# XiYe20/NPVP

Measured on AMD Instinct MI355X. Metric: predictor train frames/sec, higher is better.
Workload: dtype f32 (two-term fp16 split of amax-scaled operands, 3 MFMAs per product, fp32 accumulate: fp32-grade; small GEMMs: three-term bf16 split)

## Files before the change

### include/npvp_hip.h

```cpp
#ifndef NPVP_HIP_H
#define NPVP_HIP_H
#include <stddef.h>
#ifdef __cplusplus
extern "C" {
#endif

typedef struct ihipStream_t* npvp_stream_t;

int npvp_version(void);
const char* npvp_last_error(void);
long long npvp_launch_count(void);
void* npvp_stream_create_low_priority(int* least, int* greatest);
int npvp_stream_destroy(void* stream);
void* npvp_event_create(void);
int npvp_event_record(void* event, void* stream);
float npvp_event_elapsed_ms(void* event0, void* event1);
int npvp_event_destroy(void* event);

long long npvp_graph_node_counts(void* graph, long long* counts, long long* memset_bytes, int max_memsets);

long long npvp_gemm_workspace_bytes(int M, int N, int K);
int npvp_gemm_kernel_id(int a_kc, int b_kc, int M, int N, int K, int precision, int has_planes);
int npvp_gemm_route(int a_kc, int b_kc, int M, int N, int K, int precision, int has_planes, int plain_epilogue, int* out4);
int npvp_gemm_f32(int a_kc, int b_kc, int M, int N, int K, const float* A, long long lda, const float* B, long long ldb,
                  float* C, long long ldc, const float* bias, int act, const float* aux_in, float* aux_out,
                  const float* residual, long long ldr, float drop_p, int drop_mode, int drop_g1, int drop_g2,
                  const unsigned long long* seed, unsigned int salt, float alpha, int precision, float* colsum_a,
                  const void* b_pre, int accumulate, float* rowstats, const float* a_amax, const float* b_amax,
                  float* c_amax, unsigned int* range_flag, float adrop_p, int adrop_g1, int adrop_g2, unsigned int adrop_salt,
                  void* workspace, long long ws_bytes, npvp_stream_t stream);
int npvp_gemm_f32_skip(int a_kc, int b_kc, int M, int N, int K, const float* A, long long lda, const float* B, long long ldb,
                       float* C, long long ldc, const float* bias, int act, const float* aux_in, float* aux_out,
                       const float* residual, long long ldr, float drop_p, int drop_mode, int drop_g1, int drop_g2,
                       const unsigned long long* seed, unsigned int salt, float alpha, int precision, float* colsum_a,
                       const void* b_pre, int accumulate, float* rowstats, const float* a_amax, const float* b_amax,
                       float* c_amax, unsigned int* range_flag, float adrop_p, int adrop_g1, int adrop_g2, unsigned int adrop_salt,
                       float skip_p, int skip_g1, int skip_g2, unsigned int skip_salt, void* workspace, long long ws_bytes,
                       npvp_stream_t stream);
int npvp_frame_stats_finalize(const float* part, int parts_per_frame, float values_per_part, float* mean, float* rstd,
                              int frames, float eps, npvp_stream_t stream);
int npvp_split_weight(const float* w, long long ld, int N, int K, void* F, void* D, npvp_stream_t stream);
int npvp_split_weights_batched(const void* desc, int count, npvp_stream_t stream);
int npvp_amax(const float* x, long long rows, long long cols, long long ld, float* slot, npvp_stream_t stream);

typedef struct npvp_reduce_job {
  const float* ws; float* out; long long ldc; int M, N, splits, accum; float alpha; int blocks; const float* cs_part; float* cs_out;
} npvp_reduce_job_t;
int npvp_wgrad_f16_chainable(int M, int N, int K);
long long npvp_wgrad_f16_chain_workspace_bytes(int M, int N, int K);
int npvp_wgrad_f16_chained(int M, int N, int K, const float* dy, long long lda, const float* x, long long ldb, float* dw,
                           long long ldc, float* db, int accumulate, const float* a_amax, const float* b_amax,
                           unsigned int* range_flag, float adrop_p, int adrop_g1, int adrop_g2, unsigned int adrop_salt,
                           const unsigned long long* seed, const void* prev_job, void* my_job, void* workspace,
                           long long ws_bytes, npvp_stream_t stream);
int npvp_wgrad_f16_chained_skip(int M, int N, int K, const float* dy, long long lda, const float* x, long long ldb, float* dw,
                                long long ldc, float* db, int accumulate, const float* a_amax, const float* b_amax,
                                unsigned int* range_flag, float adrop_p, int adrop_g1, int adrop_g2, unsigned int adrop_salt,
                                float skip_p, int skip_g1, int skip_g2, unsigned int skip_salt,
                                const unsigned long long* seed, const void* prev_job, void* my_job, void* workspace,
                                long long ws_bytes, npvp_stream_t stream);
int npvp_splitk_reduce_job(const void* job, npvp_stream_t stream);
int npvp_splitk_reduce_multi(const void* jobs, int n, npvp_stream_t stream);
int npvp_linear_bwd_f16_takes(int R, int N, int K);
int npvp_linear_bwd_f16(int R, int N, int K, const float* dy, long long ldy, const float* dy_amax, const void* w_planes_d,
                        const float* w_amax, float* dx, long long ldx, int act, const float* aux_in, const float* residual,
                        long long ldr, float drop_p, int drop_mode, int drop_g1, int drop_g2, unsigned int drop_salt, float* dx_amax,
                        const float* x, long long ldxx, const float* x_amax, float* dw, long long ldw, float* db,
                        unsigned int* range_flag, float adrop_p, int adrop_g1, int adrop_g2, unsigned int adrop_salt,
                        const unsigned long long* seed, const void* prev_job, void* my_job, void* workspace, long long ws_bytes,
                        npvp_stream_t stream);
int npvp_linear_bwd_f16_skip(int R, int N, int K, const float* dy, long long ldy, const float* dy_amax, const void* w_planes_d,
                             const float* w_amax, float* dx, long long ldx, int act, const float* aux_in, const float* residual,
                             long long ldr, float drop_p, int drop_mode, int drop_g1, int drop_g2, unsigned int drop_salt,
                             float* dx_amax, const float* x, long long ldxx, const float* x_amax, float* dw, long long ldw, float* db,
                             unsigned int* range_flag, float adrop_p, int adrop_g1, int adrop_g2, unsigned int adrop_salt,
                             float skip_p, int skip_g1, int skip_g2, unsigned int skip_salt, const unsigned long long* seed,
                             const void* prev_job, void* my_job, void* workspace, long long ws_bytes, npvp_stream_t stream);
int npvp_split_weight_f16(const float* w, long long ld, int N, int K, void* F, void* D, float* amax_slot, npvp_stream_t stream);
int npvp_split_weights_f16(const void* desc, int count, void* amax_table, long long amax_bytes, npvp_stream_t stream);

int npvp_layernorm_fwd(const float* x, const float* w, const float* b, float* y, float* mean, float* rstd, long long rows,
                       int C, float eps, int relu, float* y_amax, npvp_stream_t stream);
long long npvp_layernorm_bwd_workspace_bytes(long long rows, int C);
int npvp_layernorm_bwd(const float* dy, const float* x, const float* w, const float* b, const float* mean,
                       const float* rstd, float* dx, float* dw, float* db, long long rows, int C, int relu,
                       const float* dres ,
                       int accumulate , float* dx_amax,
                       void* workspace, long long ws_bytes, npvp_stream_t stream);
int npvp_layernorm_bwd_reduce(const void* workspace, float* dw, float* db, long long rows, int C, int accumulate,
                              npvp_stream_t stream);

int npvp_layernorm_bwd_reduce_job(const void* workspace, float* dw, float* db, long long rows, int C, int accumulate, void* job);
int npvp_frameln_act_bwd_reduce_job(const void* workspace, float* dw, float* db, int frames, int per_frame, int accumulate, void* job);
int npvp_mlpdw_mid_bwd_reduce_job(const void* workspace, float* gw, float* gb, int frames, int Ch, void* job);
int npvp_sum_rows_multi(const void* jobs, int n, npvp_stream_t stream);

int npvp_layernorm_nchw_fwd(const float* x, const float* w, const float* b, float* out_nchw, float* mean, float* rstd, int frames,
                            int P, int C, float eps, int relu, npvp_stream_t stream);

int npvp_frame_stats(const float* x, const float* add, float* mean, float* rstd, int frames, int T, int per_frame,
                     float eps, npvp_stream_t stream);
int npvp_posfuse_fwd(const float* x, const float* add, const float* beta, const float* gamma, float* y, float* mean,
                     float* rstd, int N, int T, int per_frame, float eps, float* y_amax, npvp_stream_t stream);
int npvp_ln_posfuse_fwd(const float* x, const float* lw, const float* lb, float ln_eps, float* y1, float* ln_mean, float* ln_rstd,
                        const float* add, const float* beta, const float* gamma, float* fused, float* pf_mean, float* pf_rstd,
                        int N, int T, int P, int C, float pf_eps, float* y1_amax, float* fused_amax, npvp_stream_t stream);
int npvp_posfuse_bwd_fused(int N, int T, int per_frame);
int npvp_posfuse_bwd(const float* dy, const float* x, const float* add, const float* gamma, const float* mean,
                     const float* rstd, float* du, float* dyxh, float* dbeta, float* dgamma, int N, int T, int per_frame,
                     int accumulate, void* workspace, long long ws_bytes , npvp_stream_t stream);

int npvp_posfuse_instance_fwd(const float* x, const float* add, const float* beta, const float* gamma, float* y, float* mean,
                              float* rstd, int N, int T, int P, int C, float eps, float* y_amax, npvp_stream_t stream);
int npvp_posfuse_instance_bwd(const float* dy, const float* x, const float* add, const float* gamma, const float* mean,
                              const float* rstd, float* du, float* dyxh, int N, int T, int P, int C, npvp_stream_t stream);

int npvp_frameln_act_fwd(const float* h, const float* mean, const float* rstd, const float* w, const float* b,
                         const float* res, float* out, int frames, int per_frame, float drop_p, unsigned int salt,
                         float dp_p, unsigned int dp_salt, int frames_per_sample, const unsigned long long* seed,
                         float* out_amax, npvp_stream_t stream);
long long npvp_frameln_act_bwd_workspace_bytes(int frames, int per_frame);
int npvp_frameln_act_bwd(const float* dout, const float* h, const float* mean, const float* rstd, const float* w,
                         const float* b, float* dh, float* dw, float* db, int frames, int per_frame, float drop_p,
                         unsigned int salt, float dp_p, unsigned int dp_salt, int frames_per_sample,
                         const unsigned long long* seed, int accumulate ,
                         float* dh_amax, void* workspace, long long ws_bytes, npvp_stream_t stream);
int npvp_frameln_act_bwd_reduce(const void* workspace, float* dw, float* db, int frames, int per_frame, int accumulate,
                                npvp_stream_t stream);
int npvp_dwconv3x3(const float* a, const float* wt, const float* bias, float* out, int frames, int H, int W, int Ch,
                   int flip, npvp_stream_t stream);
int npvp_dwconv3x3_stats(const float* a, const float* wt, const float* bias, float* out, float* mean, float* rstd, int frames,
                         int H, int W, int Ch, float eps, void* workspace, long long ws_bytes, npvp_stream_t stream);
int npvp_mlpdw_mid_fwd(const float* h1, const float* mean1, const float* rstd1, const float* w1n, const float* b1n,
                       const float* wt, const float* bias, float* h2, float* mean2, float* rstd2, int frames, int H, int W,
                       int Ch, float eps, void* workspace, long long ws_bytes, npvp_stream_t stream);
int npvp_mlpdw_mid_fwd_parts(const float* h1, const float* part1, int J1, float nb1, float* mean1, float* rstd1, const float* w1n,
                             const float* b1n, const float* wt, const float* bias, float* h2, float* part2, int frames, int H,
                             int W, int Ch, float eps, npvp_stream_t stream);
int npvp_frameln_act_fwd_parts(const float* h, const float* part, int J, float nb, float eps, float* mean, float* rstd,
                               const float* w, const float* b, const float* res, float* out, int frames, int per_frame,
                               float drop_p, unsigned int salt, float dp_p, unsigned int dp_salt, int frames_per_sample,
                               const unsigned long long* seed, float* out_amax, npvp_stream_t stream);
long long npvp_mlpdw_mid_bwd_workspace_bytes(int frames, int Ch);
int npvp_mlpdw_mid_bwd(const float* dh2, const float* h1, const float* mean1, const float* rstd1, const float* w1n,
                       const float* b1n, const float* wt, float* da1, float* dwt_db, float* psum, int frames, int H, int W,
                       int Ch, int accumulate, void* workspace, long long ws_bytes, npvp_stream_t stream);
int npvp_mlpdw_mid_bwd_reduce(const void* workspace, float* dwt_db, int frames, int Ch, int accumulate, npvp_stream_t stream);
int npvp_mlpdw_mid_bwd_reduce_into(const void* workspace, float* gw, float* gb, int frames, int Ch, npvp_stream_t stream);
int npvp_mlpdw_mid_bwd_n2(const float* da2, const float* h2, const float* mean2, const float* rstd2, const float* w2n,
                          const float* b2n, const float* psum2, int nparts2, float drop_p, unsigned int salt,
                          const unsigned long long* seed, const float* h1, const float* mean1, const float* rstd1,
                          const float* w1n, const float* b1n, const float* wt, float* da1, float* dwt_db, float* psum, int frames,
                          int H, int W, int Ch, int accumulate, void* workspace, long long ws_bytes, npvp_stream_t stream);
int npvp_frameln_act_bwd_pgrad(const float* dout, const float* h, const float* mean, const float* rstd, const float* w,
                               const float* b, float* psum, float* dw, float* db, int frames, int per_frame, float drop_p,
                               unsigned int salt, float dp_p, unsigned int dp_salt, int frames_per_sample,
                               const unsigned long long* seed, int accumulate, void* workspace, long long ws_bytes,
                               npvp_stream_t stream);
int npvp_frameln_act_bwd_apply(const float* dout, const float* h, const float* mean, const float* rstd, const float* w,
                               const float* b, const float* psum, int nparts, float* dh, float* dw, float* db, int frames,
                               int per_frame, int accumulate, float* dh_amax, void* workspace, long long ws_bytes,
                               npvp_stream_t stream);
int npvp_mlpdw_mid_fwd_parts_skip(const float* h1, const float* part1, int J1, float nb1, float* mean1, float* rstd1,
                                  const float* w1n, const float* b1n, const float* wt, const float* bias, float* h2, float* part2,
                                  int frames, int H, int W, int Ch, float eps, float skip_p, unsigned int skip_salt, int skip_fps,
                                  const unsigned long long* seed, npvp_stream_t stream);
int npvp_frameln_act_fwd_parts_skip(const float* h, const float* part, int J, float nb, float eps, float* mean, float* rstd,
                                    const float* w, const float* b, const float* res, float* out, int frames, int per_frame,
                                    float drop_p, unsigned int salt, float dp_p, unsigned int dp_salt, int frames_per_sample,
                                    const unsigned long long* seed, float* out_amax, float skip_p, unsigned int skip_salt,
                                    int skip_fps, npvp_stream_t stream);
int npvp_frameln_act_bwd_apply_skip(const float* dout, const float* h, const float* mean, const float* rstd, const float* w,
                                    const float* b, const float* psum, int nparts, float* dh, float* dw, float* db, int frames,
                                    int per_frame, int accumulate, float* dh_amax, void* workspace, long long ws_bytes,
                                    float skip_p, unsigned int skip_salt, int skip_fps, const unsigned long long* seed,
                                    npvp_stream_t stream);

int npvp_im2col3x3(const float* in, float* out, int frames, int H, int W, int C, int col2im, npvp_stream_t stream);
long long npvp_dwconv3x3_wgrad_workspace_bytes(int frames, int Ch);
int npvp_dwconv3x3_wgrad(const float* a, const float* dout, float* dwt_db, int frames, int H, int W, int Ch,
                         void* workspace, long long ws_bytes, npvp_stream_t stream);

int npvp_attn_fwd(const float* q, long long ld_q, const float* k, long long ld_k, const float* v, long long ld_v, float* o,
                  long long ld_o, int mode, int dim0, int P, int W, int ws, int Tq, int Tk, int heads, int head_dim,
                  int mask_mode, float drop_p, const unsigned long long* seed, unsigned int salt, float* o_amax,
                  npvp_stream_t stream);
int npvp_attn_bwd(const float* q, long long ld_q, const float* k, long long ld_k, const float* v, long long ld_v,
                  const float* go, long long ld_o, float* dq, long long ld_dq, float* dk, long long ld_dk, float* dv,
                  long long ld_dv, int mode, int dim0, int P, int W, int ws, int Tq, int Tk, int heads, int head_dim,
                  int mask_mode, float drop_p, const unsigned long long* seed, unsigned int salt, float* dq_amax,
                  float* dk_amax , float* dv_amax,
                  npvp_stream_t stream);
int npvp_attn_long_fwd(const float* q, long long ld_q, const float* k, long long ld_k, const float* v, long long ld_v, float* o,
                       long long ld_o, int mode, int dim0, int P, int W, int ws, int Tq, int Tk, int heads, int head_dim,
                       int mask_mode, float drop_p, const unsigned long long* seed, unsigned int salt, float* o_amax,
                       npvp_stream_t stream);
long long npvp_attn_long_bwd_workspace_bytes(int mode, int dim0, int P, int W, int ws, int Tq, int Tk, int heads);
int npvp_attn_long_bwd(const float* q, long long ld_q, const float* k, long long ld_k, const float* v, long long ld_v,
                       const float* go, long long ld_o, float* dq, long long ld_dq, float* dk, long long ld_dk, float* dv,
                       long long ld_dv, int mode, int dim0, int P, int W, int ws, int Tq, int Tk, int heads, int head_dim,
                       int mask_mode, float drop_p, const unsigned long long* seed, unsigned int salt, float* dq_amax,
                       float* dk_amax , float* dv_amax, void* workspace, long long ws_bytes,
                       npvp_stream_t stream);

int npvp_reparam_samples(const float* mu, const float* logvar, float* z, float* eps_out, long long numel, int S,
                         long long sample_base, const unsigned long long* seed, unsigned int salt, npvp_stream_t stream);
int npvp_attn_samples_fwd(const float* q, long long ld_q, const float* k, long long ld_k, const float* v, long long ld_v, float* o,
                          long long ld_o, int S, int N, int P, int Tq, int Tk, int heads, int head_dim, int sample_chunk,
                          float* o_amax, npvp_stream_t stream);

int npvp_drop_apply(const float* x, float* out, long long rows, int ncols, float p, int mode, int g1, int g2,
                    const unsigned long long* seed, unsigned int salt, float* out_amax, npvp_stream_t stream);
int npvp_transpose(const float* in, float* out, int batch, int R, int C, npvp_stream_t stream);
int npvp_dwtb_accumulate(const float* dwtb, float* gw, float* gb, int C, npvp_stream_t stream);
int npvp_dwtb_build(const float* w, const float* b, float* wtb, int C, npvp_stream_t stream);
int npvp_reduce_mid(const float* in, float* out, int A, int B, long long Cc, float scale, int accumulate, npvp_stream_t stream);
int npvp_broadcast_mid(const float* in, float* out, int A, int B, long long Cc, float scale, npvp_stream_t stream);
int npvp_grid_center_pad(const float* src, long long ld_src, float* dst, long long ld_dst, int F, int H, int W, int Hp, int Wp, int top,
                         int left, int C, long long rows_out, float* dst_amax, npvp_stream_t stream);
int npvp_grid_center_cut(const float* src, long long ld_src, const float* addend, long long ld_add, float* dst, long long ld_dst, int F,
                         int H, int W, int Hp, int Wp, int top, int left, int C, float* dst_amax, npvp_stream_t stream);
int npvp_evt_token_join(const float* x, long long ld_x, const float* token, long long ld_token, long long token_clip_stride, float* y,
                        long long ld_y, int N, int T, int P, int C, float* y_amax, npvp_stream_t stream);
int npvp_evt_token_split(const float* y, long long ld_y, float* x, long long ld_x, float* last, long long ld_last, int N, int T, int P,
                         int C, float* x_amax, float* last_amax, npvp_stream_t stream);

long long npvp_colsum_workspace_bytes(long long rows, int N);
int npvp_colsum(const float* x, long long rows, int N, long long ld, float* out, int accumulate ,
                void* workspace, long long ws_bytes, npvp_stream_t stream);

int npvp_l1_mean(const float* a, const float* b, long long n, float lam, float* out, void* workspace, long long ws_bytes,
                 npvp_stream_t stream);
int npvp_l1_mean_bwd(const float* a, const float* b, long long n, const float* gout, float lam, float* da, npvp_stream_t stream);
int npvp_sum_all(const float* x, long long n, float* out, void* workspace, long long ws_bytes, npvp_stream_t stream);

int npvp_grad_norm_clip(const float* g, long long n, float max_norm, float* out2, void* workspace, long long ws_bytes,
                        npvp_stream_t stream);
int npvp_adamw_step(float* p, float* g, float* m, float* v, long long n, const float* hyper, float beta1, float beta2,
                    float eps, float weight_decay, const float* clip, long long clip_begin, long long clip_end,
                    int write_back_grad, npvp_stream_t stream);

long long npvp_sqdiff_workspace_bytes(int N, long long per_image);
int npvp_sqdiff_per_image(const float* x, const float* y, int N, long long per_image, float data_range, float scale, float* out,
                          void* workspace, long long ws_bytes, npvp_stream_t stream);
long long npvp_ssim_workspace_bytes(int N, int C, int H, int W);
int npvp_ssim_per_image(const float* img1, const float* img2, int N, int C, int H, int W, const float* taps ,
                        int window_size, float* out, void* workspace, long long ws_bytes, npvp_stream_t stream);

int npvp_u8hwc_to_f32chw(const void* src_u8, float* dst, long long frames, int H, int W, int C, const float* mean,
                         const float* std, npvp_stream_t stream);

int npvp_bias_act(const float* x, const float* bias, const float* residual, float* out, long long outer, long long inner, int C,
                  int layout, int act, npvp_stream_t stream);
int npvp_act_bwd(const float* g, const float* y, float* dx, long long n, int act, npvp_stream_t stream);

int npvp_bn_workspace_bytes(int C);
int npvp_bn_stats(const float* x, long long outer, long long inner, int C, int layout, double* sums, void* workspace, long long ws_bytes,
                  npvp_stream_t stream);
int npvp_bn_act_apply(const float* x, const float* w, const float* b, const float* residual, const double* sums, long long count,
                      float eps, float momentum, float* running_mean, float* running_var, long long outer, long long inner, int C,
                      int layout, int act, float* y, float* mean, float* rstd, npvp_stream_t stream);
int npvp_bn_act_bwd(const float* g, const float* x, const float* mean, const float* rstd, const float* w, const float* b, long long outer,
                    long long inner, int C, int layout, int act, int train, float* dx, float* dw, float* db, void* workspace,
                    long long ws_bytes, npvp_stream_t stream);
int npvp_bn_act_apply_sync(const float* x, const float* w, const float* b, const float* residual, const double* stat, float eps,
                           float momentum, float* running_mean, float* running_var, long long outer, long long inner, int C, int layout,
                           int act, float* y, float* mean, float* rstd, npvp_stream_t stream);
int npvp_bn_bwd_sums(const float* g, const float* x, const float* mean, const float* rstd, const float* w, const float* b, long long outer,
                     long long inner, int C, int layout, int act, double* sums, float* dw, float* db, void* workspace, long long ws_bytes,
                     npvp_stream_t stream);
int npvp_bn_act_bwd_apply(const float* g, const float* x, const float* mean, const float* rstd, const float* w, const float* b,
                          const double* sums, const double* count, long long outer, long long inner, int C, int layout, int act, float* dx,
                          npvp_stream_t stream);
int npvp_reflect_pad(const float* x, float* y, int planes, int H, int W, int C, int P, int layout, int backward, npvp_stream_t stream);
int npvp_nonlocal_attn_fwd(const float* q, long long ldq, const float* k, long long ldk, const float* v, long long ldv, float* o,
                           long long ldo, float* lse, int F, int H, int W, int A, int V, npvp_stream_t stream);
int npvp_nonlocal_attn_bwd(const float* q, long long ldq, const float* k, long long ldk, const float* v, long long ldv, const float* go,
                           long long ldgo, const float* lse, float* D, float* dq, long long lddq,
                           float* dk, long long lddk, float* dv, long long lddv, int F, int H, int W, int A, int V, npvp_stream_t stream);
int npvp_nonlocal_attn_grid_fwd(const float* q, long long ldq, const float* k, long long ldk, const float* v, long long ldv, float* o,
                                long long ldo, float* lse, int F, int H, int W, int A, int V, npvp_stream_t stream);
int npvp_nonlocal_attn_grid_bwd(const float* q, long long ldq, const float* k, long long ldk, const float* v, long long ldv,
                                const float* go, long long ldgo, const float* lse, float* D, float* dq, long long lddq,
                                float* dk, long long lddk, float* dv, long long lddv, int F, int H, int W, int A, int V,
                                npvp_stream_t stream);
int npvp_temporal_attn_fwd(const float* q, long long ldq, const float* k, long long ldk, const float* v, long long ldv, float* o,
                           long long ldo, float* lse, int N, int T, int HW, int A, int V, npvp_stream_t stream);
int npvp_temporal_attn_bwd(const float* q, long long ldq, const float* k, long long ldk, const float* v, long long ldv, const float* go,
                           long long ldgo, const float* lse, float* dq, long long lddq, float* dk, long long lddk, float* dv,
                           long long lddv, int N, int T, int HW, int A, int V, npvp_stream_t stream);
int npvp_temporal_attn_long_fwd(const float* q, long long ldq, const float* k, long long ldk, const float* v, long long ldv, float* o,
                                long long ldo, float* lse, int N, int T, int HW, int A, int V, npvp_stream_t stream);
int npvp_temporal_attn_long_bwd(const float* q, long long ldq, const float* k, long long ldk, const float* v, long long ldv,
                                const float* go, long long ldgo, const float* lse, float* D, float* dq, long long lddq, float* dk,
                                long long lddk, float* dv, long long lddv, int N, int T, int HW, int A, int V, npvp_stream_t stream);

int npvp_dp_unique_id(void* id_out_128_bytes);
int npvp_dp_init(int rank, int world, const void* unique_id_128_bytes);
int npvp_dp_world(void);
int npvp_dp_rank(void);
int npvp_dp_allreduce_async(float* bucket, size_t n, npvp_stream_t side);
int npvp_dp_wait(npvp_stream_t compute);
int npvp_dp_finalize(void);

#ifdef __cplusplus
}
#endif
#endif
```

### npvp_amd/csrc/common.h

```cpp
#pragma once
#include <hip/hip_runtime.h>
#include <stdint.h>
#include "npvp_hip.h"

#define NPVP_OK 0
#define NPVP_ERR_ARG (-1)
#define NPVP_ERR_LAUNCH (-2)
#define NPVP_ERR_WORKSPACE (-3)

void npvp_set_error(const char* msg);

namespace npvp { extern long long g_launches; }
#define NPVP_LAUNCH(...)                                                    \
  do {                                                                      \
    __atomic_fetch_add(&npvp::g_launches, 1ll, __ATOMIC_RELAXED);           \
    hipLaunchKernelGGL(__VA_ARGS__);                                        \
  } while (0)

#define NPVP_CHECK_ARG(cond, msg)                    \
  do {                                               \
    if (!(cond)) {                                   \
      npvp_set_error(msg);                           \
      return NPVP_ERR_ARG;                           \
    }                                                \
  } while (0)

#define NPVP_CHECK_LAUNCH()                          \
  do {                                               \
    hipError_t e__ = hipGetLastError();              \
    if (e__ != hipSuccess) {                         \
      npvp_set_error(hipGetErrorString(e__));        \
      return NPVP_ERR_LAUNCH;                        \
    }                                                \
  } while (0)

namespace npvp {

constexpr int WAVE = 64;

__device__ __forceinline__ float wave_sum(float v) {
#pragma unroll
  for (int o = 32; o > 0; o >>= 1) v += __shfl_xor(v, o, 64);
  return v;
}
__device__ __forceinline__ float wave_max(float v) {
#pragma unroll
  for (int o = 32; o > 0; o >>= 1) v = fmaxf(v, __shfl_xor(v, o, 64));
  return v;
}

constexpr int AMAX_WORDS = 32, AMAX_STRIDE = 16;
__device__ __forceinline__ float amax_slot_read(const float* slot) {
  const float v = wave_max(slot[(threadIdx.x & (AMAX_WORDS - 1)) * AMAX_STRIDE]);
  return __builtin_bit_cast(float, __builtin_amdgcn_readfirstlane(__builtin_bit_cast(int, v)));
}
__device__ __forceinline__ unsigned int amax_peek(const float* slot, unsigned int idx) {
  if (!slot) return 0xffffffffu;
  return __hip_atomic_load(reinterpret_cast<const unsigned int*>(slot) + (idx & (AMAX_WORDS - 1)) * AMAX_STRIDE, __ATOMIC_RELAXED,
                           __HIP_MEMORY_SCOPE_AGENT);
}
__device__ __forceinline__ unsigned int amax_peek_wave(const float* slot) { return amax_peek(slot, blockIdx.x * 4u + (threadIdx.x >> 6)); }
__device__ __forceinline__ unsigned int amax_peek_block(const float* slot) { return amax_peek(slot, blockIdx.x); }
__device__ __forceinline__ void amax_word_raise(float* slot, unsigned int idx, float m, unsigned int peeked) {
  const unsigned int bits = __float_as_uint(m);
  if (bits > peeked) atomicMax(reinterpret_cast<unsigned int*>(slot) + (idx & (AMAX_WORDS - 1)) * AMAX_STRIDE, bits);
}
__device__ __forceinline__ void amax_slot_commit(float* slot, float m, unsigned int peeked) {
  if (!slot) return;
  m = wave_max(m);
  if ((threadIdx.x & 63) == 0) amax_word_raise(slot, blockIdx.x * 4u + (threadIdx.x >> 6), m, peeked);
}
__device__ __forceinline__ void amax_slot_commit_block(float* slot, float m, float* red, unsigned int peeked) {
  if (!slot) return;
  m = wave_max(m);
  if ((threadIdx.x & 63) == 0) red[threadIdx.x >> 6] = m;
  __syncthreads();
  if (threadIdx.x == 0) {
    for (unsigned int i = 1; i < (blockDim.x >> 6); ++i) m = fmaxf(m, red[i]);
    amax_word_raise(slot, blockIdx.x, m, peeked);
  }
}
__host__ __device__ __forceinline__ float amax_scale(float amax) {
  unsigned int u;
  __builtin_memcpy(&u, &amax, 4);
  const unsigned int E = (u >> 23) & 0xffu;
  if (E < 16u || E == 255u) return 1.f;
  u = (268u - E) << 23;
  float s;
  __builtin_memcpy(&s, &u, 4);
  return s;
}

__host__ __device__ __forceinline__ float pow2_recip(float s) {
  unsigned int u;
  __builtin_memcpy(&u, &s, 4);
  u = 0x7f000000u - u;
  float r;
  __builtin_memcpy(&r, &u, 4);
  return r;
}

__device__ __forceinline__ float amax4(float m, const float4& v) {
  return fmaxf(fmaxf(fmaxf(m, fabsf(v.x)), fabsf(v.y)), fmaxf(fabsf(v.z), fabsf(v.w)));
}

__device__ __forceinline__ void fmac_scalar(float& acc, float a, float b) {
#if defined(__HIP_DEVICE_COMPILE__)
  asm volatile("v_fmac_f32 %0, %1, %2" : "+v"(acc) : "v"(a), "v"(b));
#else
  acc = fmaf(a, b, acc);
#endif
}

template <int NW>
__device__ __forceinline__ float block_sum(float v, float* red) {
  v = wave_sum(v);
  const int w = threadIdx.x >> 6;
  __syncthreads();
  if ((threadIdx.x & 63) == 0) red[w] = v;
  __syncthreads();
  float t = 0.f;
#pragma unroll
  for (int i = 0; i < NW; ++i) t += red[i];
  return t;
}

__device__ __forceinline__ void frame_stats_merge(const float* __restrict__ part, long long f, int J, float nb, float eps, float& mu,
                                                  float& rs) {
  float m = 0.f;
  for (int j = 0; j < J; ++j) m += part[(f * J + j) * 2];
  m /= J;
  float m2 = 0.f;
  for (int j = 0; j < J; ++j) { const float d = part[(f * J + j) * 2] - m; m2 += part[(f * J + j) * 2 + 1] + nb * d * d; }
  mu = m;
  rs = rsqrtf(m2 / (nb * J) + eps);
}

__device__ __forceinline__ float gelu_phi(float x, float& E) {
  const float au = fabsf(x) * 0.70710678118654752440f;
  const float t = __builtin_amdgcn_rcpf(fmaf(0.3275911f, au, 1.0f));
  E = __expf(-0.5f * x * x);
  float p = fmaf(1.061405429f, t, -1.453152027f);
  p = fmaf(p, t, 1.421413741f);
  p = fmaf(p, t, -0.284496736f);
  p = fmaf(p, t, 0.254829592f);
  const float hq = 0.5f * p * t * E;
  return x >= 0.f ? 1.0f - hq : hq;
}
__device__ __forceinline__ float gelu_f(float x) {
  float E;
  return x * gelu_phi(x, E);
}
__device__ __forceinline__ float gelu_grad_f(float x) {
  float E;
  const float phi = gelu_phi(x, E);
  return fmaf(x * 0.39894228040143267794f, E, phi);
}

__host__ __device__ __forceinline__ uint32_t mix32(uint32_t h) {
  h ^= h >> 16; h *= 0x85ebca6bu;
  h ^= h >> 13; h *= 0xc2b2ae35u;
  h ^= h >> 16;
  return h;
}
__host__ __device__ __forceinline__ uint32_t rng_u32(uint64_t seed, uint32_t salt, uint64_t idx) {
  const uint32_t k0 = mix32((uint32_t)seed ^ mix32(salt * 0x9e3779b9u + 0x7f4a7c15u));
  const uint32_t k1 = mix32((uint32_t)(seed >> 32) + mix32(salt ^ 0x85ebca6bu));
  const uint32_t h = mix32((uint32_t)idx ^ k0);
  return mix32(h + k1 + (uint32_t)(idx >> 32) * 0x9e3779b9u);
}
__device__ __forceinline__ float drop_scale(uint64_t seed, uint32_t salt, uint64_t idx, uint32_t thresh, float inv_keep) {
  return rng_u32(seed, salt, idx) >= thresh ? inv_keep : 0.f;
}
__host__ __device__ __forceinline__ uint32_t drop_threshold(float p) {
  double t = (double)p * 4294967296.0;
  if (t < 0) t = 0;
  if (t > 4294967295.0) t = 4294967295.0;
  return (uint32_t)t;
}

struct DropSpec {
  unsigned int thresh; float inv_keep; unsigned int salt; int mode; int g1; int g2;
  unsigned int m1, m2; int s1, s2;
};
__host__ __device__ __forceinline__ void div_magic(unsigned int d, unsigned int& m, int& s) {
  int l = 0;
  while (l < 31 && (1u << l) < d) ++l;
  s = 31 + l;
  m = (unsigned int)(((1ull << s) + d - 1ull) / d);
}
__device__ __forceinline__ unsigned int div_by_magic(unsigned int n, unsigned int m, int s) {
  return (unsigned int)(((unsigned long long)n * m) >> s);
}
__device__ __forceinline__ unsigned int drop_group(const DropSpec& d, long long row) {
  const unsigned int q1 = div_by_magic((unsigned int)row, d.m1, d.s1);
  return q1 - div_by_magic(q1, d.m2, d.s2) * (unsigned int)d.g2;
}
__device__ __forceinline__ float drop_spec_scale(const DropSpec& d, uint64_t seed, long long row, int col, int ncols) {
  const uint64_t key = d.mode == 0 ? (uint64_t)row * (uint64_t)ncols + (uint64_t)col : (uint64_t)drop_group(d, row);
  return rng_u32(seed, d.salt, key) >= d.thresh ? d.inv_keep : 0.f;
}
inline DropSpec make_drop_spec(float p, unsigned int salt, int mode, int g1, int g2) {
  DropSpec d;
  d.thresh = p > 0.f ? drop_threshold(p) : 0u;
  d.inv_keep = p > 0.f ? 1.f / (1.f - p) : 1.f;
  d.salt = salt; d.mode = mode; d.g1 = g1 > 0 ? g1 : 1; d.g2 = g2 > 0 ? g2 : 1;
  div_magic((unsigned int)d.g1, d.m1, d.s1);
  div_magic((unsigned int)d.g2, d.m2, d.s2);
  return d;
}

struct FrameSkip {
  const unsigned long long* seed; unsigned int thresh; unsigned int salt; int fps;
};
__device__ __forceinline__ unsigned long long frame_skip_seed(const FrameSkip& s) { return (s.thresh && s.seed) ? *s.seed : 0ull; }
__device__ __forceinline__ bool frame_skipped(const FrameSkip& s, unsigned long long seed, long long f) {
  return s.thresh && rng_u32(seed, s.salt, (uint64_t)((unsigned int)f / (unsigned int)s.fps)) < s.thresh;
}
__device__ __forceinline__ unsigned long long frame_skip_mask(const FrameSkip& s, long long f0, long long f1) {
  if (!s.thresh) return 0ull;
  const unsigned long long seed = frame_skip_seed(s);
  const long long f = f0 + (long long)(threadIdx.x & 63);
  return __builtin_amdgcn_ballot_w64(f < f1 && frame_skipped(s, seed, f));
}
inline FrameSkip make_frame_skip(float p, unsigned int salt, int frames_per_sample, const unsigned long long* seed) {
  FrameSkip s;
  s.seed = seed; s.thresh = (p > 0.f && seed) ? drop_threshold(p) : 0u; s.salt = salt; s.fps = frames_per_sample > 0 ? frames_per_sample : 1;
  return s;
}

__device__ __forceinline__ float4 ld4(const float* p) { return *reinterpret_cast<const float4*>(p); }
__device__ __forceinline__ void st4(float* p, float4 v) { *reinterpret_cast<float4*>(p) = v; }

}
```

### npvp_amd/csrc/mlpdw.hip

```cpp
#include "partials.h"
#include <cstring>
#include <cstdlib>

namespace npvp {

__global__ void dwconv3x3_kernel(const float* __restrict__ a, const float* __restrict__ wt, const float* __restrict__ bias,
                                 float* __restrict__ out, int H, int W, int Ch, long long total4, int flip) {
  const int c4n = Ch / 4, P = H * W;
  for (long long i = (long long)blockIdx.x * blockDim.x + threadIdx.x; i < total4; i += (long long)gridDim.x * blockDim.x) {
    const int c = (int)(i % c4n) * 4;
    const long long fp = i / c4n;
    const int p = (int)(fp % P);
    const long long f = fp / P;
    const int h = p / W, w = p - h * W;
    float4 acc = bias ? ld4(bias + c) : make_float4(0.f, 0.f, 0.f, 0.f);
    const float* af = a + f * P * Ch + c;
#pragma unroll
    for (int ky = -1; ky <= 1; ++ky) {
      const int hh = h + ky;
      if (hh < 0 || hh >= H) continue;
#pragma unroll
      for (int kx = -1; kx <= 1; ++kx) {
        const int ww = w + kx;
        if (ww < 0 || ww >= W) continue;
// ... 20 lines not shown
  const int c = (int)(i % c4n) * 4;
  const long long f = i / c4n;
  float4 wv[9];
#pragma unroll
  for (int t = 0; t < 9; ++t) wv[t] = ld4(wt + (flip ? 8 - t : t) * Ch + c);
  const float4 bv = bias ? ld4(bias + c) : make_float4(0.f, 0.f, 0.f, 0.f);
  const float* af = a + f * (HH * WW) * Ch + c;
  float* of = out + f * (HH * WW) * Ch + c;
  const float4 z = make_float4(0.f, 0.f, 0.f, 0.f);
  float4 r0[WW], r1[WW], r2[WW];
#pragma unroll
  for (int w = 0; w < WW; ++w) { r0[w] = z; r1[w] = ld4(af + (long long)w * Ch); }
#pragma unroll
  for (int h = 0; h < HH; ++h) {
#pragma unroll
    for (int w = 0; w < WW; ++w) r2[w] = (h + 1 < HH) ? ld4(af + (long long)((h + 1) * WW + w) * Ch) : z;
#pragma unroll
    for (int w = 0; w < WW; ++w) {
      float4 acc = bv;
#pragma unroll
      for (int kx = -1; kx <= 1; ++kx) {
        const int ww = w + kx;
        if (ww < 0 || ww >= WW) continue;
        const float4 w0 = wv[kx + 1], w1 = wv[3 + kx + 1], w2 = wv[6 + kx + 1];
        const float4 x0 = r0[ww], x1 = r1[ww], x2 = r2[ww];
        acc.x += w0.x * x0.x + w1.x * x1.x + w2.x * x2.x; acc.y += w0.y * x0.y + w1.y * x1.y + w2.y * x2.y;
        acc.z += w0.z * x0.z + w1.z * x1.z + w2.z * x2.z; acc.w += w0.w * x0.w + w1.w * x1.w + w2.w * x2.w;
      }
      st4(of + (long long)(h * WW + w) * Ch, acc);
      if constexpr (STATS) {
        if (h == 0 && w == 0) shift = acc.x;
        const float a0 = acc.x - shift, a1 = acc.y - shift, a2 = acc.z - shift, a3 = acc.w - shift;
        s1 += (a0 + a1) + (a2 + a3);
        s2 += (a0 * a0 + a1 * a1) + (a2 * a2 + a3 * a3);
      }
    }
#pragma unroll
    for (int w = 0; w < WW; ++w) { r0[w] = r1[w]; r1[w] = r2[w]; }
  }
  if constexpr (STATS) {
    const float n = (float)(HH * WW * 4), m1 = s1 / n, mean_t = shift + m1, m2_t = s2 - s1 * m1;
    const float mean_b = block_sum<4>(mean_t, red) / 256.f;
    const float d = mean_t - mean_b;
    const float m2_b = block_sum<4>(m2_t + n * d * d, red);
    if (threadIdx.x == 0) { part[blockIdx.x * 2] = mean_b; part[blockIdx.x * 2 + 1] = m2_b; }
  }
}

template <int VEC> struct Vec { float v[VEC]; };
template <int VEC> __device__ __forceinline__ Vec<VEC> ldv(const float* p) {
  Vec<VEC> r;
  if constexpr (VEC == 4) { const float4 t = ld4(p); r.v[0] = t.x; r.v[1] = t.y; r.v[2] = t.z; r.v[3] = t.w; }
  else if constexpr (VEC == 2) { const float2 t = *reinterpret_cast<const float2*>(p); r.v[0] = t.x; r.v[1] = t.y; }
  else r.v[0] = *p;
  return r;
}
template <int VEC> __device__ __forceinline__ void stv(float* p, const Vec<VEC>& r) {
  if constexpr (VEC == 4) st4(p, make_float4(r.v[0], r.v[1], r.v[2], r.v[3]));
  else if constexpr (VEC == 2) *reinterpret_cast<float2*>(p) = make_float2(r.v[0], r.v[1]);
  else *p = r.v[0];
}

template <int VEC>
__global__ __launch_bounds__(256, 4) void mlpdw_mid_fwd_kernel(const float* __restrict__ h1, const float* __restrict__ mean1,
                                                            const float* __restrict__ rstd1, const float* __restrict__ w1n,
                                                            const float* __restrict__ b1n, const float* __restrict__ wt,
                                                            const float* __restrict__ bias, float* __restrict__ h2,
                                                            float* __restrict__ part, int Ch, const float* __restrict__ part1,
                                                            int J1, float nb1, float eps1, float* __restrict__ mean1_out,
                                                            float* __restrict__ rstd1_out, FrameSkip skip) {
  constexpr int HH = 8, WW = 8;
  __shared__ float red[4];
  const int bpf = Ch / VEC / 256;
  const long long f = blockIdx.x / bpf;
  const int c = ((blockIdx.x - (int)f * bpf) * 256 + threadIdx.x) * VEC;
  float mu, rs;
  if (part1) {
    frame_stats_merge(part1, f, J1, nb1, eps1, mu, rs);
    if (blockIdx.x == f * bpf && threadIdx.x == 0) { mean1_out[f] = mu; rstd1_out[f] = rs; }
  } else { mu = mean1[f]; rs = rstd1[f]; }
  const float* hf = h1 + f * (HH * WW) * Ch;
  float* of = h2 + f * (HH * WW) * Ch;
  if (frame_skipped(skip, frame_skip_seed(skip), f)) {
    Vec<VEC> z;
#pragma unroll
    for (int e = 0; e < VEC; ++e) z.v[e] = 0.f;
#pragma unroll
    for (int pix = 0; pix < HH * WW; ++pix) stv<VEC>(of + pix * Ch + c, z);
    if (threadIdx.x == 0) { part[blockIdx.x * 2] = 0.f; part[blockIdx.x * 2 + 1] = 0.f; }
    return;
  }
  Vec<VEC> wv[9];
#pragma unroll
  for (int t = 0; t < 9; ++t) wv[t] = ldv<VEC>(wt + t * Ch + c);
  const Vec<VEC> bv = ldv<VEC>(bias + c);
  Vec<VEC> r0[WW], r1[WW], r2[WW];
  auto load_row = [&](Vec<VEC>* row, int hh) {
#pragma unroll
    for (int w = 0; w < WW; ++w) {
      const int pix = hh * WW + w, off = pix * Ch + c;
      const Vec<VEC> x = ldv<VEC>(hf + off), ww = ldv<VEC>(w1n + off), bb = ldv<VEC>(b1n + off);
#pragma unroll
      for (int e = 0; e < VEC; ++e) row[w].v[e] = gelu_f((x.v[e] - mu) * rs * ww.v[e] + bb.v[e]);
    }
  };
#pragma unroll
  for (int w = 0; w < WW; ++w)
#pragma unroll
    for (int e = 0; e < VEC; ++e) r0[w].v[e] = 0.f;
  load_row(r1, 0);
  float shift = 0.f, s1 = 0.f, s2 = 0.f;
#pragma unroll 1
  for (int h = 0; h < HH; ++h) {
    if (h + 1 < HH) load_row(r2, h + 1);
    else {
#pragma unroll
      for (int w = 0; w < WW; ++w)
#pragma unroll
        for (int e = 0; e < VEC; ++e) r2[w].v[e] = 0.f;
    }
#pragma unroll
    for (int w = 0; w < WW; ++w) {
      Vec<VEC> acc = bv;
#pragma unroll
      for (int kx = -1; kx <= 1; ++kx) {
        const int ww = w + kx;
        if (ww < 0 || ww >= WW) continue;
#pragma unroll
        for (int e = 0; e < VEC; ++e)
          acc.v[e] += wv[kx + 1].v[e] * r0[ww].v[e] + wv[3 + kx + 1].v[e] * r1[ww].v[e] + wv[6 + kx + 1].v[e] * r2[ww].v[e];
      }
      stv<VEC>(of + (h * WW + w) * Ch + c, acc);
      if (h == 0 && w == 0) shift = acc.v[0];
#pragma unroll
      for (int e = 0; e < VEC; ++e) { const float a = acc.v[e] - shift; s1 += a; s2 += a * a; }
    }
#pragma unroll
    for (int w = 0; w < WW; ++w) { r0[w] = r1[w]; r1[w] = r2[w]; }
  }
  const float n = (float)(HH * WW * VEC), m1 = s1 / n, mean_t = shift + m1, m2_t = s2 - s1 * m1;
  const float mean_b = block_sum<4>(mean_t, red) / 256.f;
  const float d = mean_t - mean_b;
  const float m2_b = block_sum<4>(m2_t + n * d * d, red);
  if (threadIdx.x == 0) { part[blockIdx.x * 2] = mean_b; part[blockIdx.x * 2 + 1] = m2_b; }
}

#ifndef NPVP_MID_BWD_WAVES
#define NPVP_MID_BWD_WAVES 2
#endif
struct MidN2 {
  const float* h2; const float* mean2; const float* rstd2; const float* w2n; const float* b2n;
  const float* psum2; int nparts2;
  const unsigned long long* seed; unsigned int drop_thresh; float drop_inv_keep; unsigned int salt;
};

template <int VEC, bool FUSE2>
__global__ __launch_bounds__(256, NPVP_MID_BWD_WAVES) void mlpdw_mid_bwd_kernel(const float* __restrict__ dh2, const float* __restrict__ h1,
                                                            const float* __restrict__ mean1, const float* __restrict__ rstd1,
                                                            const float* __restrict__ w1n, const float* __restrict__ b1n,
                                                            const float* __restrict__ wt, float* __restrict__ da1,
                                                            float* __restrict__ part, float* __restrict__ psum, int Ch,
                                                            int frames, int frames_per_chunk, MidN2 n2) {
  constexpr int HH = 8, WW = 8;
  __shared__ float red[4];
  const unsigned long long seed2 = (FUSE2 && n2.seed && n2.drop_thresh) ? *n2.seed : 0ull;
  const int c = (blockIdx.x * blockDim.x + threadIdx.x) * VEC;
  const int nblk = gridDim.x;
  Vec<VEC> wv[9], aw[9], ab;
#pragma unroll
  for (int t = 0; t < 9; ++t) {
    wv[t] = ldv<VEC>(wt + t * Ch + c);
#pragma unroll
    for (int e = 0; e < VEC; ++e) aw[t].v[e] = 0.f;
  }
#pragma unroll
  for (int e = 0; e < VEC; ++e) ab.v[e] = 0.f;
  const int f0 = blockIdx.y * frames_per_chunk, f1 = min(frames, f0 + frames_per_chunk);
  for (long long f = f0; f < f1; ++f) {
    const float mu = mean1[f], rs = rstd1[f];
    const float* hf = h1 + f * (HH * WW) * Ch;
    const float* gf = dh2 + f * (HH * WW) * Ch;
    float* of = da1 + f * (HH * WW) * Ch;
    float mu2 = 0.f, rs2 = 0.f, c1 = 0.f, c2 = 0.f;
    const float* h2f = nullptr;
    if constexpr (FUSE2) {
      mu2 = n2.mean2[f]; rs2 = n2.rstd2[f];
      h2f = n2.h2 + f * (HH * WW) * Ch;
      const int j = threadIdx.x;
      const float p1 = j < n2.nparts2 ? n2.psum2[(f * n2.nparts2 + j) * 2] : 0.f;
      const float p2 = j < n2.nparts2 ? n2.psum2[(f * n2.nparts2 + j) * 2 + 1] : 0.f;
      const float inv = 1.f / (float)(HH * WW * Ch);
      c1 = block_sum<4>(p1, red) * inv;
      c2 = block_sum<4>(p2, red) * inv;
    }
    Vec<VEC> a0[WW], a1r[WW], a2[WW], g0[WW], g1[WW], g2[WW], gp1[WW], xh1[WW], gp2[WW], xh2[WW];
    auto load_row = [&](Vec<VEC>* arow, Vec<VEC>* grow, Vec<VEC>* gprow, Vec<VEC>* xhrow, int hh) {
      if constexpr (FUSE2) {
#pragma unroll
        for (int w0 = 0; w0 < WW; w0 += 4) {
#pragma unroll
          for (int w = w0; w < w0 + 4; ++w) {
            const int off = (hh * WW + w) * Ch + c;
            const Vec<VEC> d2 = ldv<VEC>(gf + off), x2 = ldv<VEC>(h2f + off), w2 = ldv<VEC>(n2.w2n + off), b2 = ldv<VEC>(n2.b2n + off);
#pragma unroll
            for (int e = 0; e < VEC; ++e) {
              const float xh2 = (x2.v[e] - mu2) * rs2;
              float m = 1.f;
              if (n2.drop_thresh)
                m = drop_scale(seed2, n2.salt, (unsigned long long)(f * (HH * WW) * Ch + off + e), n2.drop_thresh, n2.drop_inv_keep);
              const float dyln = d2.v[e] * m * gelu_grad_f(xh2 * w2.v[e] + b2.v[e]);
              grow[w].v[e] = rs2 * (dyln * w2.v[e] - c1 - xh2 * c2);
            }
          }
          __builtin_amdgcn_sched_barrier(0);
        }
      }
#pragma unroll
      for (int w = 0; w < WW; ++w) {
        const int pix = hh * WW + w, off = pix * Ch + c;
        const Vec<VEC> x = ldv<VEC>(hf + off), ww = ldv<VEC>(w1n + off), bb = ldv<VEC>(b1n + off);
        if constexpr (!FUSE2) grow[w] = ldv<VEC>(gf + off);
#pragma unroll
        for (int e = 0; e < VEC; ++e) {
          const float xh = (x.v[e] - mu) * rs, y = xh * ww.v[e] + bb.v[e];
          float E;
          const float phi = gelu_phi(y, E);
          arow[w].v[e] = y * phi;
          gprow[w].v[e] = fmaf(y * 0.39894228040143267794f, E, phi) * ww.v[e];
          xhrow[w].v[e] = xh;
        }
      }
    };
#pragma unroll
    for (int w = 0; w < WW; ++w)
#pragma unroll
      for (int e = 0; e < VEC; ++e) { a0[w].v[e] = 0.f; g0[w].v[e] = 0.f; }
    load_row(a1r, g1, gp1, xh1, 0);
    float s1 = 0.f, s2 = 0.f;
#pragma unroll 1
    for (int h = 0; h < HH; ++h) {
      if (h + 1 < HH) load_row(a2, g2, gp2, xh2, h + 1);
      else {
#pragma unroll
        for (int w = 0; w < WW; ++w)
#pragma unroll
          for (int e = 0; e < VEC; ++e) { a2[w].v[e] = 0.f; g2[w].v[e] = 0.f; }
      }
#pragma unroll
      for (int w = 0; w < WW; ++w) {
        Vec<VEC> acc;
#pragma unroll
        for (int e = 0; e < VEC; ++e) { acc.v[e] = 0.f; ab.v[e] += g1[w].v[e]; }
#pragma unroll
        for (int kx = -1; kx <= 1; ++kx) {
          const int ww = w + kx;
          if (ww < 0 || ww >= WW) continue;
#pragma unroll
          for (int e = 0; e < VEC; ++e) {
            acc.v[e] += wv[8 - (kx + 1)].v[e] * g0[ww].v[e] + wv[8 - (3 + kx + 1)].v[e] * g1[ww].v[e] + wv[8 - (6 + kx + 1)].v[e] * g2[ww].v[e];
            const float d = g1[w].v[e];
            fmac_scalar(aw[kx + 1].v[e], d, a0[ww].v[e]);
            fmac_scalar(aw[3 + kx + 1].v[e], d, a1r[ww].v[e]);
            fmac_scalar(aw[6 + kx + 1].v[e], d, a2[ww].v[e]);
          }
        }
        stv<VEC>(of + (h * WW + w) * Ch + c, acc);
#pragma unroll
        for (int e = 0; e < VEC; ++e) { const float g = acc.v[e] * gp1[w].v[e]; s1 += g; s2 += g * xh1[w].v[e]; }
      }
#pragma unroll
      for (int w = 0; w < WW; ++w) { a0[w] = a1r[w]; a1r[w] = a2[w]; g0[w] = g1[w]; g1[w] = g2[w]; gp1[w] = gp2[w]; xh1[w] = xh2[w]; }
    }
    s1 = block_sum<4>(s1, red);
    s2 = block_sum<4>(s2, red);
    if (threadIdx.x == 0) { psum[(f * nblk + blockIdx.x) * 2] = s1; psum[(f * nblk + blockIdx.x) * 2 + 1] = s2; }
  }
  float* o = part + (long long)blockIdx.y * 10 * Ch;
#pragma unroll
  for (int t = 0; t < 9; ++t) stv<VEC>(o + t * Ch + c, aw[t]);
  stv<VEC>(o + 9 * Ch + c, ab);
}

__global__ void frame_stats_finalize_kernel(const float* __restrict__ part, int J, float nb, float* __restrict__ mean,
                                            float* __restrict__ rstd, int frames, float eps) {
  const int f = blockIdx.x * blockDim.x + threadIdx.x;
  if (f >= frames) return;
  float m = 0.f;
  for (int j = 0; j < J; ++j) m += part[(f * J + j) * 2];
  m /= J;
  float m2 = 0.f;
  for (int j = 0; j < J; ++j) { const float d = part[(f * J + j) * 2] - m; m2 += part[(f * J + j) * 2 + 1] + nb * d * d; }
  mean[f] = m;
  rstd[f] = rsqrtf(m2 / (nb * J) + eps);
}

template <int HH, int WW>
__global__ __launch_bounds__(256) void dwconv3x3_wgrad_win_kernel(const float* __restrict__ a, const float* __restrict__ dout,
                                                                  float* __restrict__ part, int Ch, int frames,
                                                                  int frames_per_chunk) {
  const int c = (blockIdx.x * blockDim.x + threadIdx.x) * 4;
  if (c >= Ch) return;
  const float4 z = make_float4(0.f, 0.f, 0.f, 0.f);
  float4 aw[9], ab = z;
#pragma unroll
  for (int t = 0; t < 9; ++t) aw[t] = z;
  const int f0 = blockIdx.y * frames_per_chunk, f1 = min(frames, f0 + frames_per_chunk);
  for (long long f = f0; f < f1; ++f) {
    const float* af = a + f * (HH * WW) * Ch + c;
    const float* df = dout + f * (HH * WW) * Ch + c;
    float4 r0[WW], r1[WW], r2[WW];
#pragma unroll
    for (int w = 0; w < WW; ++w) { r0[w] = z; r1[w] = ld4(af + (long long)w * Ch); }
#pragma unroll
    for (int h = 0; h < HH; ++h) {
#pragma unroll
      for (int w = 0; w < WW; ++w) r2[w] = (h + 1 < HH) ? ld4(af + (long long)((h + 1) * WW + w) * Ch) : z;
#pragma unroll
      for (int w = 0; w < WW; ++w) {
        const float4 d = ld4(df + (long long)(h * WW + w) * Ch);
        ab.x += d.x; ab.y += d.y; ab.z += d.z; ab.w += d.w;
#pragma unroll
        for (int kx = -1; kx <= 1; ++kx) {
          const int ww = w + kx;
          if (ww < 0 || ww >= WW) continue;
          const float4 x0 = r0[ww], x1 = r1[ww], x2 = r2[ww];
          float4& t0 = aw[kx + 1]; float4& t1 = aw[3 + kx + 1]; float4& t2 = aw[6 + kx + 1];
          t0.x += d.x * x0.x; t0.y += d.y * x0.y; t0.z += d.z * x0.z; t0.w += d.w * x0.w;
          t1.x += d.x * x1.x; t1.y += d.y * x1.y; t1.z += d.z * x1.z; t1.w += d.w * x1.w;
          t2.x += d.x * x2.x; t2.y += d.y * x2.y; t2.z += d.z * x2.z; t2.w += d.w * x2.w;
        }
      }
#pragma unroll
      for (int w = 0; w < WW; ++w) { r0[w] = r1[w]; r1[w] = r2[w]; }
    }
  }
  float* o = part + (long long)blockIdx.y * 10 * Ch;
#pragma unroll
  for (int t = 0; t < 9; ++t) st4(o + t * Ch + c, aw[t]);
  st4(o + 9 * Ch + c, ab);
}

__global__ __launch_bounds__(256) void dwconv3x3_wgrad_kernel(const float* __restrict__ a, const float* __restrict__ dout,
                                                              float* __restrict__ part, int H, int W, int Ch, int frames,
                                                              int frames_per_chunk) {
  __shared__ float4 red[3][10][64];
  const int cx = threadIdx.x & 63, pg = threadIdx.x >> 6;
  const int c = (blockIdx.x * 64 + cx) * 4;
  const bool live = c < Ch;
  const int P = H * W;
  float4 aw[9], ab = make_float4(0.f, 0.f, 0.f, 0.f);
#pragma unroll
  for (int t = 0; t < 9; ++t) aw[t] = make_float4(0.f, 0.f, 0.f, 0.f);
  const int f0 = blockIdx.y * frames_per_chunk, f1 = min(frames, f0 + frames_per_chunk);
  if (live) {
    for (long long f = f0; f < f1; ++f) {
      const float* af = a + f * P * Ch + c;
      const float* df = dout + f * P * Ch + c;
      for (int p = pg; p < P; p += 4) {
        const int h = p / W, w = p - h * W;
        const float4 d = ld4(df + (long long)p * Ch);
        ab.x += d.x; ab.y += d.y; ab.z += d.z; ab.w += d.w;
#pragma unroll
// ... 14 lines not shown
  }
  if (pg > 0) {
#pragma unroll
    for (int t = 0; t < 9; ++t) red[pg - 1][t][cx] = aw[t];
    red[pg - 1][9][cx] = ab;
  }
  __syncthreads();
  if (pg == 0 && live) {
    float* o = part + (long long)blockIdx.y * 10 * Ch;
#pragma unroll
    for (int t = 0; t < 10; ++t) {
      float4 s = t < 9 ? aw[t] : ab;
#pragma unroll
      for (int g = 0; g < 3; ++g) { const float4 q = red[g][t][cx]; s.x += q.x; s.y += q.y; s.z += q.z; s.w += q.w; }
      st4(o + t * Ch + c, s);
    }
  }
}

__global__ void im2col3x3_kernel(const float* __restrict__ in, float* __restrict__ out, int H, int W, int C, long long total4,
                                 int col2im) {
  const int c4n = C / 4, P = H * W;
  for (long long i = (long long)blockIdx.x * blockDim.x + threadIdx.x; i < total4; i += (long long)gridDim.x * blockDim.x) {
    if (!col2im) {
      const int c = (int)(i % c4n) * 4;
      long long r = i / c4n;
      const int tap = (int)(r % 9); r /= 9;
      const int p = (int)(r % P);
      const long long f = r / P;
      const int h = p / W + tap / 3 - 1, w = p % W + tap % 3 - 1;
      float4 v = make_float4(0.f, 0.f, 0.f, 0.f);
      if (h >= 0 && h < H && w >= 0 && w < W) v = ld4(in + (f * P + h * W + w) * C + c);
      st4(out + r * 9 * C + (long long)tap * C + c, v);
    } else {
      const int c = (int)(i % c4n) * 4;
      const long long r = i / c4n;
      const int q = (int)(r % P);
      const long long f = r / P;
      float4 s = make_float4(0.f, 0.f, 0.f, 0.f);
#pragma unroll
      for (int tap = 0; tap < 9; ++tap) {
        const int h = q / W - (tap / 3 - 1), w = q % W - (tap % 3 - 1);
        if (h < 0 || h >= H || w < 0 || w >= W) continue;
        const float4 v = ld4(in + (f * P + h * W + w) * 9 * C + (long long)tap * C + c);
        s.x += v.x; s.y += v.y; s.z += v.z; s.w += v.w;
      }
      st4(out + r * C + c, s);
    }
  }
}

static int dw_chunks(int frames) { return frames < 256 ? frames : 256; }

}

using namespace npvp;

extern "C" int npvp_dwconv3x3(const float* a, const float* wt, const float* bias, float* out, int frames, int H, int W,
                              int Ch, int flip, hipStream_t stream) {
  NPVP_CHECK_ARG(frames > 0 && H > 0 && W > 0 && Ch % 4 == 0, "dwconv: bad shape");
  if (H == 8 && W == 8) {
    const long long nthreads = (long long)frames * (Ch / 4);
    NPVP_LAUNCH((dwconv3x3_win_kernel<8, 8, false>), dim3((unsigned)((nthreads + 255) / 256)), dim3(256), 0, stream, a,
                       wt, bias, out, Ch, nthreads, flip, (float*)nullptr);
    NPVP_CHECK_LAUNCH();
    return NPVP_OK;
  }
  const long long total4 = (long long)frames * H * W * Ch / 4;
  long long blocks = (total4 + 255) / 256; if (blocks > 8192) blocks = 8192;
  NPVP_LAUNCH(dwconv3x3_kernel, dim3((unsigned)blocks), dim3(256), 0, stream, a, wt, bias, out, H, W, Ch, total4, flip);
  NPVP_CHECK_LAUNCH();
  return NPVP_OK;
}

extern "C" int npvp_frame_stats_finalize(const float* part, int parts_per_frame, float values_per_part, float* mean,
                                         float* rstd, int frames, float eps, hipStream_t stream) {
  NPVP_CHECK_ARG(part && mean && rstd && frames > 0 && parts_per_frame > 0, "frame_stats_finalize: bad arguments");
  NPVP_LAUNCH(frame_stats_finalize_kernel, dim3((frames + 255) / 256), dim3(256), 0, stream, part, parts_per_frame,
                     values_per_part, mean, rstd, frames, eps);
  NPVP_CHECK_LAUNCH();
  return NPVP_OK;
}

extern "C" int npvp_dwconv3x3_stats(const float* a, const float* wt, const float* bias, float* out, float* mean, float* rstd,
                                    int frames, int H, int W, int Ch, float eps, void* workspace, long long ws_bytes,
                                    hipStream_t stream) {
  NPVP_CHECK_ARG(frames > 0 && H == 8 && W == 8 && Ch > 0 && Ch % 1024 == 0, "dwconv_stats: needs an 8x8 grid and Ch % 1024 == 0");
  const int J = Ch / 1024;
  NPVP_CHECK_ARG(workspace && ws_bytes >= (long long)frames * J * 8, "dwconv_stats: workspace too small");
  const long long nthreads = (long long)frames * (Ch / 4);
  NPVP_LAUNCH((dwconv3x3_win_kernel<8, 8, true>), dim3((unsigned)(nthreads / 256)), dim3(256), 0, stream, a, wt, bias, out,
                     Ch, nthreads, 0, (float*)workspace);
  NPVP_CHECK_LAUNCH();
  NPVP_LAUNCH(frame_stats_finalize_kernel, dim3((frames + 255) / 256), dim3(256), 0, stream, (const float*)workspace, J,
                     65536.f, mean, rstd, frames, eps);
  NPVP_CHECK_LAUNCH();
  return NPVP_OK;
}

extern "C" int npvp_mlpdw_mid_fwd(const float* h1, const float* mean1, const float* rstd1, const float* w1n, const float* b1n,
                                  const float* wt, const float* bias, float* h2, float* mean2, float* rstd2, int frames,
                                  int H, int W, int Ch, float eps, void* workspace, long long ws_bytes, hipStream_t stream) {
  NPVP_CHECK_ARG(frames > 0 && H == 8 && W == 8 && Ch > 0 && Ch % 512 == 0, "mlpdw_mid_fwd: needs an 8x8 grid and Ch % 512 == 0");
  const int J = Ch / 512;
  NPVP_CHECK_ARG(workspace && ws_bytes >= (long long)frames * J * 8, "mlpdw_mid_fwd: workspace too small");
  const long long nthreads = (long long)frames * (Ch / 2);
  NPVP_LAUNCH((mlpdw_mid_fwd_kernel<2>), dim3((unsigned)(nthreads / 256)), dim3(256), 0, stream, h1, mean1, rstd1, w1n, b1n,
                     wt, bias, h2, (float*)workspace, Ch, (const float*)nullptr, 0, 0.f, 0.f, (float*)nullptr, (float*)nullptr, FrameSkip{});
  NPVP_CHECK_LAUNCH();
  NPVP_LAUNCH(frame_stats_finalize_kernel, dim3((frames + 255) / 256), dim3(256), 0, stream, (const float*)workspace, J,
                     32768.f, mean2, rstd2, frames, eps);
  NPVP_CHECK_LAUNCH();
  return NPVP_OK;
}

extern "C" int npvp_mlpdw_mid_fwd_parts_skip(const float* h1, const float* part1, int J1, float nb1, float* mean1, float* rstd1,
                                             const float* w1n, const float* b1n, const float* wt, const float* bias, float* h2,
                                             float* part2, int frames, int H, int W, int Ch, float eps, float skip_p,
                                             unsigned int skip_salt, int skip_fps, const unsigned long long* seed, hipStream_t stream) {
  NPVP_CHECK_ARG(frames > 0 && H == 8 && W == 8 && Ch > 0 && Ch % 512 == 0, "mlpdw_mid_fwd_parts: needs an 8x8 grid and Ch % 512 == 0");
  NPVP_CHECK_ARG(part1 && J1 > 0 && nb1 > 0.f && mean1 && rstd1 && part2, "mlpdw_mid_fwd_parts: bad arguments");
  NPVP_CHECK_ARG(skip_p >= 0.f && skip_p < 1.f && (skip_p == 0.f || (seed && skip_fps > 0)), "mlpdw_mid_fwd_parts: bad frame-skip arguments");
  const long long nthreads = (long long)frames * (Ch / 2);
  NPVP_LAUNCH((mlpdw_mid_fwd_kernel<2>), dim3((unsigned)(nthreads / 256)), dim3(256), 0, stream, h1, (const float*)nullptr,
                     (const float*)nullptr, w1n, b1n, wt, bias, h2, part2, Ch, part1, J1, nb1, eps, mean1, rstd1,
                     make_frame_skip(skip_p, skip_salt, skip_fps, seed));
  NPVP_CHECK_LAUNCH();
  return NPVP_OK;
}

extern "C" int npvp_mlpdw_mid_fwd_parts(const float* h1, const float* part1, int J1, float nb1, float* mean1, float* rstd1,
                                        const float* w1n, const float* b1n, const float* wt, const float* bias, float* h2,
                                        float* part2, int frames, int H, int W, int Ch, float eps, hipStream_t stream) {
  return npvp_mlpdw_mid_fwd_parts_skip(h1, part1, J1, nb1, mean1, rstd1, w1n, b1n, wt, bias, h2, part2, frames, H, W, Ch, eps, 0.f, 0u, 1,
                                       nullptr, stream);
}

static int mid_chunks(int frames) { return frames < 128 ? frames : 128; }

static Partials mid_partials(const void* ws, float* out, float* out_b, int frames, int Ch, int accumulate) {
  return make_partials(ws, 0, frames, mid_chunks(frames), 10 * Ch, out, accumulate, out_b, out_b ? Ch : 0, out_b ? 1 : 0);
}

extern "C" long long npvp_mlpdw_mid_bwd_workspace_bytes(int frames, int Ch) {
  return mid_partials(nullptr, nullptr, nullptr, frames, Ch, 0).bytes;
}

static int mid_bwd_launch(const float* dh2, const float* h1, const float* mean1, const float* rstd1, const float* w1n,
                          const float* b1n, const float* wt, float* da1, float* dwt_db, float* psum, int frames, int H, int W,
                          int Ch, int accumulate, void* workspace, long long ws_bytes, hipStream_t stream, const MidN2* n2) {
  NPVP_CHECK_ARG(frames > 0 && H == 8 && W == 8 && Ch > 0 && Ch % 512 == 0, "mlpdw_mid_bwd: needs an 8x8 grid and Ch % 512 == 0");
  NPVP_CHECK_ARG(workspace && ws_bytes >= npvp_mlpdw_mid_bwd_workspace_bytes(frames, Ch), "mlpdw_mid_bwd: workspace too small");
  const Partials P = mid_partials(workspace, dwt_db, nullptr, frames, Ch, accumulate);
  if (n2)
    NPVP_LAUNCH((mlpdw_mid_bwd_kernel<1, true>), dim3(Ch / 256, P.job.nb), dim3(256), 0, stream, dh2, h1, mean1, rstd1, w1n,
                       b1n, wt, da1, P.part(), psum, Ch, frames, P.per, *n2);
  else
    NPVP_LAUNCH((mlpdw_mid_bwd_kernel<1, false>), dim3(Ch / 256, P.job.nb), dim3(256), 0, stream, dh2, h1, mean1, rstd1, w1n,
                       b1n, wt, da1, P.part(), psum, Ch, frames, P.per, MidN2{});
  NPVP_CHECK_LAUNCH();
  return finish_partials(P.job, accumulate, stream, "mlpdw_mid_bwd: reduce launch failed");
}

extern "C" int npvp_mlpdw_mid_bwd(const float* dh2, const float* h1, const float* mean1, const float* rstd1, const float* w1n,
                                  const float* b1n, const float* wt, float* da1, float* dwt_db, float* psum, int frames, int H,
                                  int W, int Ch, int accumulate, void* workspace, long long ws_bytes, hipStream_t stream) {
  return mid_bwd_launch(dh2, h1, mean1, rstd1, w1n, b1n, wt, da1, dwt_db, psum, frames, H, W, Ch, accumulate, workspace, ws_bytes,
                        stream, nullptr);
}

extern "C" int npvp_mlpdw_mid_bwd_n2(const float* da2, const float* h2, const float* mean2, const float* rstd2, const float* w2n,
                                     const float* b2n, const float* psum2, int nparts2, float drop_p, unsigned int salt,
                                     const unsigned long long* seed, const float* h1, const float* mean1, const float* rstd1,
                                     const float* w1n, const float* b1n, const float* wt, float* da1, float* dwt_db, float* psum,
                                     int frames, int H, int W, int Ch, int accumulate, void* workspace, long long ws_bytes,
                                     hipStream_t stream) {
  NPVP_CHECK_ARG(h2 && mean2 && rstd2 && w2n && b2n && psum2 && nparts2 > 0 && nparts2 <= 256, "mlpdw_mid_bwd_n2: bad norm2 arguments");
  NPVP_CHECK_ARG(drop_p >= 0.f && drop_p < 1.f && (drop_p == 0.f || seed), "mlpdw_mid_bwd_n2: bad dropout arguments");
  MidN2 n2;
  n2.h2 = h2; n2.mean2 = mean2; n2.rstd2 = rstd2; n2.w2n = w2n; n2.b2n = b2n; n2.psum2 = psum2; n2.nparts2 = nparts2;
  n2.seed = seed; n2.drop_thresh = drop_p > 0.f ? drop_threshold(drop_p) : 0u;
  n2.drop_inv_keep = drop_p > 0.f ? 1.f / (1.f - drop_p) : 1.f; n2.salt = salt;
  return mid_bwd_launch(da2, h1, mean1, rstd1, w1n, b1n, wt, da1, dwt_db, psum, frames, H, W, Ch, accumulate, workspace, ws_bytes,
                        stream, &n2);
}

__global__ void mid_bwd_reduce_into_kernel(const float* __restrict__ part, float* __restrict__ gw, float* __restrict__ gb, int Ch,
                                           int nchunks) {
  const int i = blockIdx.x * blockDim.x + threadIdx.x;
  if (i >= 10 * Ch) return;
  float s = 0.f;
  for (int k = 0; k < nchunks; ++k) s += part[(long long)k * 10 * Ch + i];
  const int tap = i / Ch, c = i - tap * Ch;
  if (tap < 9) gw[c * 9 + tap] += s; else gb[c] += s;
}

extern "C" int npvp_mlpdw_mid_bwd_reduce_into(const void* workspace, float* gw, float* gb, int frames, int Ch,
                                              hipStream_t stream) {
  NPVP_CHECK_ARG(workspace && gw && gb && frames > 0 && Ch > 0, "mlpdw_mid_bwd_reduce_into: bad arguments");
  const SumRowsJob j = mid_partials(workspace, gw, gb, frames, Ch, 1).job;
  NPVP_LAUNCH(mid_bwd_reduce_into_kernel, dim3((10 * Ch + 255) / 256), dim3(256), 0, stream, j.in, gw, gb, Ch, j.nb);
  NPVP_CHECK_LAUNCH();
  return NPVP_OK;
}

extern "C" int npvp_mlpdw_mid_bwd_reduce_job(const void* workspace, float* gw, float* gb, int frames, int Ch, void* job) {
  NPVP_CHECK_ARG(workspace && gw && gb && frames > 0 && Ch > 0 && job, "mlpdw_mid_bwd_reduce_job: bad arguments");
  return put_job(job, mid_partials(workspace, gw, gb, frames, Ch, 1).job);
}

extern "C" int npvp_mlpdw_mid_bwd_reduce(const void* workspace, float* dwt_db, int frames, int Ch, int accumulate,
                                         hipStream_t stream) {
  return finish_partials(mid_partials(workspace, dwt_db, nullptr, frames, Ch, accumulate).job, 0, stream, "mlpdw_mid_bwd_reduce: launch failed");
}

extern "C" int npvp_im2col3x3(const float* in, float* out, int frames, int H, int W, int C, int col2im, hipStream_t stream) {
  NPVP_CHECK_ARG(frames > 0 && H > 0 && W > 0 && C % 4 == 0, "im2col: bad shape");
  const long long total4 = (long long)frames * H * W * (col2im ? 1 : 9) * C / 4;
  long long blocks = (total4 + 255) / 256; if (blocks > 8192) blocks = 8192;
  NPVP_LAUNCH(im2col3x3_kernel, dim3((unsigned)blocks), dim3(256), 0, stream, in, out, H, W, C, total4, col2im);
  NPVP_CHECK_LAUNCH();
  return NPVP_OK;
}

static Partials dw_partials(const void* ws, float* dwt_db, int frames, int Ch) {
  return make_partials(ws, 0, frames, dw_chunks(frames), 10 * Ch, dwt_db, 0);
}

extern "C" long long npvp_dwconv3x3_wgrad_workspace_bytes(int frames, int Ch) { return dw_partials(nullptr, nullptr, frames, Ch).bytes; }

extern "C" int npvp_dwconv3x3_wgrad(const float* a, const float* dout, float* dwt_db, int frames, int H, int W, int Ch,
                                    void* workspace, long long ws_bytes, hipStream_t stream) {
  NPVP_CHECK_ARG(frames > 0 && H > 0 && W > 0 && Ch % 4 == 0, "dwconv_wgrad: bad shape");
  NPVP_CHECK_ARG(workspace && ws_bytes >= npvp_dwconv3x3_wgrad_workspace_bytes(frames, Ch), "dwconv_wgrad: workspace too small");
  const Partials P = dw_partials(workspace, dwt_db, frames, Ch);
  if (H == 8 && W == 8)
    NPVP_LAUNCH((dwconv3x3_wgrad_win_kernel<8, 8>), dim3((Ch / 4 + 255) / 256, P.job.nb), dim3(256), 0, stream, a, dout,
                       P.part(), Ch, frames, P.per);
  else
    NPVP_LAUNCH(dwconv3x3_wgrad_kernel, dim3((Ch / 4 + 63) / 64, P.job.nb), dim3(256), 0, stream, a, dout,
                       P.part(), H, W, Ch, frames, P.per);
  NPVP_CHECK_LAUNCH();
  return finish_partials(P.job, 0, stream, "dwconv_wgrad: reduce launch failed");
}
```

### npvp_amd/csrc/norm.hip

```cpp
#include "partials.h"
#include <cstring>
#include <cstdlib>

namespace npvp {

template <int NV>
__global__ __launch_bounds__(256) void ln_fwd_kernel(const float* __restrict__ x, const float* __restrict__ w,
                                                     const float* __restrict__ b, float* __restrict__ y,
                                                     float* __restrict__ mean, float* __restrict__ rstd, long long rows,
                                                     float eps, int relu, float* __restrict__ amax) {
  constexpr int C = NV * 256;
  __shared__ float ared[4];
  const unsigned int peek = amax_peek_block(amax);
  const int lane = threadIdx.x & 63;
  float4 ww[NV], bb[NV];
#pragma unroll
  for (int i = 0; i < NV; ++i) { ww[i] = ld4(w + (i * 64 + lane) * 4); bb[i] = ld4(b + (i * 64 + lane) * 4); }
  float am = 0.f;
  for (long long row = (long long)blockIdx.x * 4 + (threadIdx.x >> 6); row < rows; row += (long long)gridDim.x * 4) {
    float4 v[NV];
    float s = 0.f;
#pragma unroll
    for (int i = 0; i < NV; ++i) {
      v[i] = ld4(x + row * C + (i * 64 + lane) * 4);
// ... 378 lines not shown
    float4 g = ld4(dy + (long long)f * per_frame + e);
    if (gamma) {
      const float4 gm = ld4(gamma + (long long)t * per_frame + e);
      g.x *= 1.f + gm.x; g.y *= 1.f + gm.y; g.z *= 1.f + gm.z; g.w *= 1.f + gm.w;
    }
    s1 += g.x + g.y + g.z + g.w;
    s2 += g.x * (v.x - mu) * rs + g.y * (v.y - mu) * rs + g.z * (v.z - mu) * rs + g.w * (v.w - mu) * rs;
  }
  s1 = block_sum<8>(s1, red) / per_frame;
  s2 = block_sum<8>(s2, red) / per_frame;
  if (threadIdx.x == 0) { s1o[f] = s1; s2o[f] = s2; }
}

__global__ void posfuse_bwd_apply_kernel(const float* __restrict__ dy, const float* __restrict__ x,
                                         const float* __restrict__ add, const float* __restrict__ gamma,
                                         const float* __restrict__ mean, const float* __restrict__ rstd,
                                         const float* __restrict__ s1, const float* __restrict__ s2,
                                         float* __restrict__ du, float* __restrict__ dyxh, int T, int per_frame,
                                         long long total4) {
  const int pf4 = per_frame / 4;
  for (long long i = (long long)blockIdx.x * blockDim.x + threadIdx.x; i < total4; i += (long long)gridDim.x * blockDim.x) {
    const long long f = i / pf4;
    const int e = (int)(i - f * pf4) * 4;
    const int n = (int)(f / T), t = (int)(f - (long long)n * T);
    float4 v = ld4(x + f * per_frame + e);
    if (add) { const float4 a = ld4(add + (long long)n * per_frame + e); v.x += a.x; v.y += a.y; v.z += a.z; v.w += a.w; }
    const float mu = mean[f], rs = rstd[f], a1 = s1[f], a2 = s2[f];
    float4 uh;
    uh.x = (v.x - mu) * rs; uh.y = (v.y - mu) * rs; uh.z = (v.z - mu) * rs; uh.w = (v.w - mu) * rs;
    const float4 d = ld4(dy + f * per_frame + e);
    float4 g = d;
    if (gamma) {
      const float4 gm = ld4(gamma + (long long)t * per_frame + e);
      g.x *= 1.f + gm.x; g.y *= 1.f + gm.y; g.z *= 1.f + gm.z; g.w *= 1.f + gm.w;
    }
    float4 o;
    o.x = rs * (g.x - a1 - uh.x * a2); o.y = rs * (g.y - a1 - uh.y * a2);
    o.z = rs * (g.z - a1 - uh.z * a2); o.w = rs * (g.w - a1 - uh.w * a2);
    st4(du + f * per_frame + e, o);
    if (dyxh) st4(dyxh + f * per_frame + e, make_float4(d.x * uh.x, d.y * uh.y, d.z * uh.z, d.w * uh.w));
  }
}

__global__ __launch_bounds__(256) void posfuse_bwd_apply_nsum_kernel(const float* __restrict__ dy, const float* __restrict__ x,
                                                                     const float* __restrict__ add, const float* __restrict__ gamma,
                                                                     const float* __restrict__ mean, const float* __restrict__ rstd,
                                                                     const float* __restrict__ s1, const float* __restrict__ s2,
                                                                     float* __restrict__ du, float* __restrict__ dbeta,
                                                                     float* __restrict__ dgamma, int N, int T, int per_frame, int accum) {
  const int pf4 = per_frame / 4;
  const int t = blockIdx.x / (pf4 / 256), e = ((blockIdx.x % (pf4 / 256)) * 256 + threadIdx.x) * 4;
  float4 gm = make_float4(1.f, 1.f, 1.f, 1.f);
  if (gamma) { const float4 g0 = ld4(gamma + (long long)t * per_frame + e); gm.x += g0.x; gm.y += g0.y; gm.z += g0.z; gm.w += g0.w; }
  float4 sb = make_float4(0.f, 0.f, 0.f, 0.f), sg = sb;
#pragma unroll 4
  for (int n = 0; n < N; ++n) {
    const long long f = (long long)n * T + t;
    float4 v = ld4(x + f * per_frame + e);
    if (add) { const float4 a = ld4(add + (long long)n * per_frame + e); v.x += a.x; v.y += a.y; v.z += a.z; v.w += a.w; }
    const float mu = mean[f], rs = rstd[f], a1 = s1[f], a2 = s2[f];
    float4 uh;
    uh.x = (v.x - mu) * rs; uh.y = (v.y - mu) * rs; uh.z = (v.z - mu) * rs; uh.w = (v.w - mu) * rs;
    const float4 d = ld4(dy + f * per_frame + e);
    float4 o;
    o.x = rs * (d.x * gm.x - a1 - uh.x * a2); o.y = rs * (d.y * gm.y - a1 - uh.y * a2);
    o.z = rs * (d.z * gm.z - a1 - uh.z * a2); o.w = rs * (d.w * gm.w - a1 - uh.w * a2);
    st4(du + f * per_frame + e, o);
    sb.x += d.x; sb.y += d.y; sb.z += d.z; sb.w += d.w;
    sg.x += d.x * uh.x; sg.y += d.y * uh.y; sg.z += d.z * uh.z; sg.w += d.w * uh.w;
  }
  if (dbeta) {
    if (accum) { const float4 o = ld4(dbeta + (long long)t * per_frame + e); sb.x += o.x; sb.y += o.y; sb.z += o.z; sb.w += o.w; }
    st4(dbeta + (long long)t * per_frame + e, sb);
  }
  if (dgamma) {
    if (accum) { const float4 o = ld4(dgamma + (long long)t * per_frame + e); sg.x += o.x; sg.y += o.y; sg.z += o.z; sg.w += o.w; }
    st4(dgamma + (long long)t * per_frame + e, sg);
  }
}

constexpr int PFI_MAXP = 64;
__global__ __launch_bounds__(256) void posfuse_inst_fwd_kernel(const float* __restrict__ x, const float* __restrict__ add,
                                                               const float* __restrict__ beta, const float* __restrict__ gamma,
                                                               float* __restrict__ y, float* __restrict__ mean,
                                                               float* __restrict__ rstd, int T, int P, int C, float eps,
                                                               float* __restrict__ amax) {
  __shared__ float ared[4];
  const unsigned int peek = amax_peek_block(amax);
  const int c = blockIdx.x * blockDim.x + threadIdx.x;
  const long long f = blockIdx.y;
  float am = 0.f;
  if (c < C) {
    const int n = (int)(f / T), t = (int)(f - (long long)n * T);
    const float* xp = x + f * P * C + c;
    const float* ap = add ? add + (long long)n * P * C + c : nullptr;
    float u[PFI_MAXP], s = 0.f;
#pragma unroll
    for (int p = 0; p < PFI_MAXP; ++p) if (p < P) { u[p] = xp[(long long)p * C] + (ap ? ap[(long long)p * C] : 0.f); s += u[p]; }
    const float mu = s / P;
    float q = 0.f;
#pragma unroll
    for (int p = 0; p < PFI_MAXP; ++p) if (p < P) { const float d = u[p] - mu; q += d * d; }
    const float rs = rsqrtf(q / P + eps);
    mean[f * C + c] = mu; rstd[f * C + c] = rs;
    const float* bp = beta + (long long)t * P * C + c;
    const float* gp = gamma ? gamma + (long long)t * P * C + c : nullptr;
#pragma unroll
    for (int p = 0; p < PFI_MAXP; ++p) if (p < P) {
      float o = (u[p] - mu) * rs;
      if (gp) o *= 1.f + gp[(long long)p * C];
      o += bp[(long long)p * C];
      y[f * P * C + (long long)p * C + c] = o;
      am = fmaxf(am, fabsf(o));
    }
  }
  amax_slot_commit_block(amax, am, ared, peek);
}

__global__ __launch_bounds__(256) void posfuse_inst_bwd_kernel(const float* __restrict__ dy, const float* __restrict__ x,
                                                               const float* __restrict__ add, const float* __restrict__ gamma,
                                                               const float* __restrict__ mean, const float* __restrict__ rstd,
                                                               float* __restrict__ du, float* __restrict__ dyxh, int T, int P,
                                                               int C) {
  const int c = blockIdx.x * blockDim.x + threadIdx.x;
  const long long f = blockIdx.y;
  if (c >= C) return;
  const int n = (int)(f / T), t = (int)(f - (long long)n * T);
  const long long base = f * P * C + c;
  const float* ap = add ? add + (long long)n * P * C + c : nullptr;
  const float* gp = gamma ? gamma + (long long)t * P * C + c : nullptr;
  const float mu = mean[f * C + c], rs = rstd[f * C + c];
  float g[PFI_MAXP], uh[PFI_MAXP], s1 = 0.f, s2 = 0.f;
#pragma unroll
  for (int p = 0; p < PFI_MAXP; ++p) if (p < P) {
    const float d = dy[base + (long long)p * C];
    uh[p] = (x[base + (long long)p * C] + (ap ? ap[(long long)p * C] : 0.f) - mu) * rs;
    if (dyxh) dyxh[base + (long long)p * C] = d * uh[p];
    g[p] = gp ? d * (1.f + gp[(long long)p * C]) : d;
    s1 += g[p]; s2 += g[p] * uh[p];
  }
  s1 /= P; s2 /= P;
#pragma unroll
  for (int p = 0; p < PFI_MAXP; ++p) if (p < P) du[base + (long long)p * C] = rs * (g[p] - s1 - uh[p] * s2);
}

struct FlnParams {
  const float* h; const float* mean; const float* rstd; const float* w; const float* b;
  const float* res;
  const unsigned long long* seed;
  unsigned int drop_thresh; float drop_inv_keep; unsigned int salt;
  unsigned int dp_thresh; float dp_inv_keep; unsigned int dp_salt; int frames_per_sample;
  int per_frame; long long total4;
  FrameSkip skip;
};

__device__ __forceinline__ float fln_frame_scale(const FlnParams& p, unsigned long long seed, long long f) {
  if (!p.dp_thresh) return 1.f;
  return drop_scale(seed, p.dp_salt, (unsigned long long)((unsigned int)f / (unsigned int)p.frames_per_sample), p.dp_thresh, p.dp_inv_keep);
}
__device__ __forceinline__ float fln_scale(const FlnParams& p, unsigned long long seed, float frame_scale, long long gidx) {
  if (!p.drop_thresh) return frame_scale;
  return drop_scale(seed, p.salt, (unsigned long long)gidx, p.drop_thresh, p.drop_inv_keep) * frame_scale;
}

__global__ void frameln_act_fwd_kernel(FlnParams p, float* __restrict__ out, float* __restrict__ amax) {
  const int pf4 = p.per_frame / 4;
  __shared__ float ared[16];
  const unsigned int peek = amax_peek_block(amax);
  float am = 0.f;
  const unsigned long long seed = (p.seed && (p.drop_thresh || p.dp_thresh)) ? *p.seed : 0ull;
  for (long long i = (long long)blockIdx.x * blockDim.x + threadIdx.x; i < p.total4; i += (long long)gridDim.x * blockDim.x) {
    const long long f = i / pf4;
    const int e = (int)(i - f * pf4) * 4;
    const float mu = p.mean[f], rs = p.rstd[f];
    const float fsc = fln_frame_scale(p, seed, f);
    const float4 v = ld4(p.h + f * p.per_frame + e), ww = ld4(p.w + e), bb = ld4(p.b + e);
    const long long g0 = f * p.per_frame + e;
    float4 o;
    o.x = gelu_f((v.x - mu) * rs * ww.x + bb.x) * fln_scale(p, seed, fsc, g0 + 0);
    o.y = gelu_f((v.y - mu) * rs * ww.y + bb.y) * fln_scale(p, seed, fsc, g0 + 1);
    o.z = gelu_f((v.z - mu) * rs * ww.z + bb.z) * fln_scale(p, seed, fsc, g0 + 2);
    o.w = gelu_f((v.w - mu) * rs * ww.w + bb.w) * fln_scale(p, seed, fsc, g0 + 3);
    if (p.res) { const float4 r = ld4(p.res + g0); o.x += r.x; o.y += r.y; o.z += r.z; o.w += r.w; }
    st4(out + g0, o);
    am = amax4(am, o);
  }
  amax_slot_commit_block(amax, am, ared, peek);
}

__global__ __launch_bounds__(256) void frameln_act_fwd_parts_kernel(FlnParams p, const float* __restrict__ part, int J, float nb,
                                                                    float eps, float* __restrict__ mean_out,
                                                                    float* __restrict__ rstd_out, float* __restrict__ out,
                                                                    float* __restrict__ amax) {
  __shared__ float ared[16];
  const unsigned int peek = amax_peek_block(amax);
  const int bpf = p.per_frame / 4096;
  const long long f = blockIdx.x / bpf;
  const int e0 = (blockIdx.x - (int)f * bpf) * 4096;
  const unsigned long long seed = (p.seed && (p.drop_thresh || p.dp_thresh)) ? *p.seed : 0ull;
  float mu, rs;
  frame_stats_merge(part, f, J, nb, eps, mu, rs);
  if (e0 == 0 && threadIdx.x == 0) { mean_out[f] = mu; rstd_out[f] = rs; }
  const float fsc = fln_frame_scale(p, seed, f);
  float am = 0.f;
  if (frame_skipped(p.skip, frame_skip_seed(p.skip), f)) {
#pragma unroll
    for (int k = 0; k < 4; ++k) {
      const long long g0 = f * p.per_frame + e0 + (k * 256 + threadIdx.x) * 4;
      const float4 o = p.res ? ld4(p.res + g0) : make_float4(0.f, 0.f, 0.f, 0.f);
      st4(out + g0, o);
      am = amax4(am, o);
    }
    amax_slot_commit_block(amax, am, ared, peek);
    return;
  }
#pragma unroll
  for (int k = 0; k < 4; ++k) {
    const int e = e0 + (k * 256 + threadIdx.x) * 4;
    const long long g0 = f * p.per_frame + e;
    const float4 v = ld4(p.h + g0), ww = ld4(p.w + e), bb = ld4(p.b + e);
    float4 o;
    o.x = gelu_f((v.x - mu) * rs * ww.x + bb.x) * fln_scale(p, seed, fsc, g0 + 0);
    o.y = gelu_f((v.y - mu) * rs * ww.y + bb.y) * fln_scale(p, seed, fsc, g0 + 1);
    o.z = gelu_f((v.z - mu) * rs * ww.z + bb.z) * fln_scale(p, seed, fsc, g0 + 2);
    o.w = gelu_f((v.w - mu) * rs * ww.w + bb.w) * fln_scale(p, seed, fsc, g0 + 3);
    if (p.res) { const float4 r = ld4(p.res + g0); o.x += r.x; o.y += r.y; o.z += r.z; o.w += r.w; }
    st4(out + g0, o);
    am = amax4(am, o);
  }
  amax_slot_commit_block(amax, am, ared, peek);
}

constexpr int FLN_PARTS = 4;
__global__ __launch_bounds__(512) void frameln_act_bwd_stats_kernel(FlnParams p, const float* __restrict__ dout,
                                                                    float* __restrict__ psum) {
  __shared__ float red[8];
  const long long f = blockIdx.x;
  const unsigned long long seed = (p.seed && (p.drop_thresh || p.dp_thresh)) ? *p.seed : 0ull;
  const float mu = p.mean[f], rs = p.rstd[f];
  const float fsc = fln_frame_scale(p, seed, f);
  float s1 = 0.f, s2 = 0.f;
  const int span = p.per_frame / FLN_PARTS, e0 = blockIdx.y * span, e1 = blockIdx.y == FLN_PARTS - 1 ? p.per_frame : e0 + span;
  for (int e = e0 + threadIdx.x * 4; e < e1; e += 512 * 4) {
    const long long g0 = f * p.per_frame + e;
    const float4 v = ld4(p.h + g0), ww = ld4(p.w + e), bb = ld4(p.b + e), d = ld4(dout + g0);
    const float hx = (v.x - mu) * rs, hy = (v.y - mu) * rs, hz = (v.z - mu) * rs, hw = (v.w - mu) * rs;
    const float gx = d.x * fln_scale(p, seed, fsc, g0 + 0) * gelu_grad_f(hx * ww.x + bb.x) * ww.x;
    const float gy = d.y * fln_scale(p, seed, fsc, g0 + 1) * gelu_grad_f(hy * ww.y + bb.y) * ww.y;
    const float gz = d.z * fln_scale(p, seed, fsc, g0 + 2) * gelu_grad_f(hz * ww.z + bb.z) * ww.z;
    const float gw = d.w * fln_scale(p, seed, fsc, g0 + 3) * gelu_grad_f(hw * ww.w + bb.w) * ww.w;
    s1 += gx + gy + gz + gw;
    s2 += gx * hx + gy * hy + gz * hz + gw * hw;
  }
  s1 = block_sum<8>(s1, red);
  s2 = block_sum<8>(s2, red);
  if (threadIdx.x == 0) { psum[(f * FLN_PARTS + blockIdx.y) * 2] = s1; psum[(f * FLN_PARTS + blockIdx.y) * 2 + 1] = s2; }
}

__global__ void frameln_act_bwd_fused_kernel(FlnParams p, const float* __restrict__ dout, const float* __restrict__ psum,
                                             float* __restrict__ dh, float* __restrict__ part, int frames,
                                             int frames_per_chunk, int nparts, float* __restrict__ amax) {
  const int e = (blockIdx.x * blockDim.x + threadIdx.x) * 4;
  __shared__ float ared[16];
  const unsigned int peek = amax_peek_block(amax);
  float am = 0.f;
  const bool live = e < p.per_frame;
  const unsigned long long seed = (p.seed && (p.drop_thresh || p.dp_thresh)) ? *p.seed : 0ull;
  const float4 zero4 = make_float4(0.f, 0.f, 0.f, 0.f);
  const float4 ww = live ? ld4(p.w + e) : zero4, bb = live ? ld4(p.b + e) : zero4;
  float4 aw = zero4, ab = zero4;
  const int f0 = blockIdx.y * frames_per_chunk;
  const int f1 = live ? min(frames, f0 + frames_per_chunk) : f0;
  const unsigned long long skipped = frame_skip_mask(p.skip, f0, min(frames, f0 + frames_per_chunk));
  for (long long f = f0; f < f1; ++f) {
    const long long g0 = f * p.per_frame + e;
    if (f - f0 < 64 && ((skipped >> (int)(f - f0)) & 1ull)) { st4(dh + g0, zero4); continue; }
    const float mu = p.mean[f], rs = p.rstd[f];
    const float fsc = fln_frame_scale(p, seed, f);
    float a1 = 0.f, a2 = 0.f;
    for (int j = 0; j < nparts; ++j) { a1 += psum[(f * nparts + j) * 2]; a2 += psum[(f * nparts + j) * 2 + 1]; }
    a1 /= p.per_frame; a2 /= p.per_frame;
    const float4 v = ld4(p.h + g0), d = ld4(dout + g0);
    const float hx = (v.x - mu) * rs, hy = (v.y - mu) * rs, hz = (v.z - mu) * rs, hw = (v.w - mu) * rs;
    const float dx_ = d.x * fln_scale(p, seed, fsc, g0 + 0) * gelu_grad_f(hx * ww.x + bb.x);
    const float dy_ = d.y * fln_scale(p, seed, fsc, g0 + 1) * gelu_grad_f(hy * ww.y + bb.y);
    const float dz_ = d.z * fln_scale(p, seed, fsc, g0 + 2) * gelu_grad_f(hz * ww.z + bb.z);
    const float dw_ = d.w * fln_scale(p, seed, fsc, g0 + 3) * gelu_grad_f(hw * ww.w + bb.w);
    aw.x += dx_ * hx; aw.y += dy_ * hy; aw.z += dz_ * hz; aw.w += dw_ * hw;
    ab.x += dx_; ab.y += dy_; ab.z += dz_; ab.w += dw_;
    float4 o;
    o.x = rs * (dx_ * ww.x - a1 - hx * a2); o.y = rs * (dy_ * ww.y - a1 - hy * a2);
    o.z = rs * (dz_ * ww.z - a1 - hz * a2); o.w = rs * (dw_ * ww.w - a1 - hw * a2);
    st4(dh + g0, o);
    am = amax4(am, o);
  }
  amax_slot_commit_block(amax, am, ared, peek);
  if (!live) return;
  float* o = part + (long long)blockIdx.y * 2 * p.per_frame;
  st4(o + e, aw);
  st4(o + p.per_frame + e, ab);
}

__global__ __launch_bounds__(256) void frameln_act_bwd_pgrad_kernel(FlnParams p, const float* __restrict__ dout,
                                                                    float* __restrict__ psum, float* __restrict__ part, int frames,
                                                                    int frames_per_chunk) {
  __shared__ float red[4];
  const int e = (blockIdx.x * blockDim.x + threadIdx.x) * 4;
  const int nblk = gridDim.x;
  const unsigned long long seed = (p.seed && (p.drop_thresh || p.dp_thresh)) ? *p.seed : 0ull;
  const float4 ww = ld4(p.w + e), bb = ld4(p.b + e);
  float4 aw = make_float4(0.f, 0.f, 0.f, 0.f), ab = make_float4(0.f, 0.f, 0.f, 0.f);
  const int f0 = blockIdx.y * frames_per_chunk;
  const int f1 = min(frames, f0 + frames_per_chunk);
  for (long long f = f0; f < f1; ++f) {
    const long long g0 = f * p.per_frame + e;
    const float mu = p.mean[f], rs = p.rstd[f];
    const float fsc = fln_frame_scale(p, seed, f);
    const float4 v = ld4(p.h + g0), d = ld4(dout + g0);
    const float hx = (v.x - mu) * rs, hy = (v.y - mu) * rs, hz = (v.z - mu) * rs, hw = (v.w - mu) * rs;
    const float dx_ = d.x * fln_scale(p, seed, fsc, g0 + 0) * gelu_grad_f(hx * ww.x + bb.x);
    const float dy_ = d.y * fln_scale(p, seed, fsc, g0 + 1) * gelu_grad_f(hy * ww.y + bb.y);
    const float dz_ = d.z * fln_scale(p, seed, fsc, g0 + 2) * gelu_grad_f(hz * ww.z + bb.z);
    const float dw_ = d.w * fln_scale(p, seed, fsc, g0 + 3) * gelu_grad_f(hw * ww.w + bb.w);
    aw.x += dx_ * hx; aw.y += dy_ * hy; aw.z += dz_ * hz; aw.w += dw_ * hw;
    ab.x += dx_; ab.y += dy_; ab.z += dz_; ab.w += dw_;
    const float gx = dx_ * ww.x, gy = dy_ * ww.y, gz = dz_ * ww.z, gw = dw_ * ww.w;
    const float s1 = block_sum<4>((gx + gy) + (gz + gw), red);
    const float s2 = block_sum<4>((gx * hx + gy * hy) + (gz * hz + gw * hw), red);
    if (threadIdx.x == 0) { psum[(f * nblk + blockIdx.x) * 2] = s1; psum[(f * nblk + blockIdx.x) * 2 + 1] = s2; }
  }
  float* o = part + (long long)blockIdx.y * 2 * p.per_frame;
  st4(o + e, aw);
  st4(o + p.per_frame + e, ab);
}

struct SumRowsPlan { int cw, threads; };
static SumRowsPlan plan_sum_rows(const SumRowsJob& q) {
  if (q.mode == 0 && q.nb < 64 && q.ncols >= 4096 && q.ncols % 4 == 0 && q.stride % 4 == 0 && (!q.out_b || q.split % 4 == 0)
      && ((uintptr_t)q.in & 15) == 0)
    return {sum_rows_wide_cols(), 1024};
  if (q.nb >= 64 && q.ncols <= 8192) return {16, 1024};
  return {64, q.nb >= 64 ? 1024 : 256};
}

int launch_sum_rows(const SumRowsJob& q, hipStream_t stream) {
  if (q.mode != 0) return NPVP_ERR_ARG;
  const SumRowsPlan pl = plan_sum_rows(q);
  const auto kernel = pl.cw == sum_rows_wide_cols() ? sum_rows_wide_kernel : pl.cw == 16 ? sum_rows_kernel<16> : sum_rows_kernel<64>;
  NPVP_LAUNCH(kernel, dim3((q.ncols + pl.cw - 1) / pl.cw), dim3(pl.threads), 0, stream, q.in, q.out, q.nb, q.stride, q.ncols, q.accum,
              q.out_b, q.out_b ? q.split : 0);
  return hipGetLastError() == hipSuccess ? NPVP_OK : NPVP_ERR_LAUNCH;
}

struct SumRowsBatch { SumRowsJob j[SRJ_MAX]; int first[SRJ_MAX + 1]; int cw[SRJ_MAX]; int n; };

__global__ __launch_bounds__(1024) void sum_rows_multi_kernel(SumRowsBatch b) {
  __shared__ float red[1024];
  int lo = 0, hi = b.n - 1;
  while (lo < hi) { const int mid = (lo + hi + 1) >> 1; if (b.first[mid] <= (int)blockIdx.x) lo = mid; else hi = mid - 1; }
  const SumRowsJob& J = b.j[lo];
  const int CW = b.cw[lo], sh = CW == 16 ? 4 : 6;
  if (CW == sum_rows_wide_cols()) {
    sum_rows_wide(J.in, J.out, J.out_b, J.nb, J.stride, J.ncols, J.out_b ? J.split : 0, J.accum,
                  (((int)blockIdx.x - b.first[lo]) * 1024 + (int)threadIdx.x) * 4);
    return;
  }
  const int cx = threadIdx.x & (CW - 1), rl = threadIdx.x >> sh, nrl = 1024 >> sh;
  const int c = ((int)blockIdx.x - b.first[lo]) * CW + cx;
  float s = 0.f;
  if (c < J.ncols)
    for (int r = rl; r < J.nb; r += nrl) s += J.in[(long long)r * J.stride + c];
  red[rl * CW + cx] = s;
  __syncthreads();
  if (rl == 0 && c < J.ncols) {
    float t = 0.f;
    for (int i = 0; i < nrl; ++i) t += red[i * CW + cx];
    float* o;
    if (J.mode == 1) { const int tap = c / J.split, ch = c - tap * J.split; o = tap < 9 ? J.out + ch * 9 + tap : J.out_b + ch; }
    else o = (J.out_b && c >= J.split) ? J.out_b + (c - J.split) : J.out + c;
    *o = J.accum ? *o + t : t;
  }
}

static inline int ew_blocks(long long total, int threads) {
  long long b = (total + threads - 1) / threads;
  if (b > 4096) b = 4096;
  if (b < 1) b = 1;
  return (int)b;
}

static void fill_fln(FlnParams& p, const float* h, const float* mean, const float* rstd, const float* w, const float* b,
                     const float* res, int frames, int per_frame, float drop_p, unsigned int salt, float dp_p,
                     unsigned int dp_salt, int frames_per_sample, const unsigned long long* seed) {
  p.h = h; p.mean = mean; p.rstd = rstd; p.w = w; p.b = b; p.res = res; p.seed = seed;
  p.drop_thresh = drop_p > 0.f ? drop_threshold(drop_p) : 0u;
  p.drop_inv_keep = drop_p > 0.f ? 1.f / (1.f - drop_p) : 1.f;
  p.salt = salt;
  p.dp_thresh = dp_p > 0.f ? drop_threshold(dp_p) : 0u;
  p.dp_inv_keep = dp_p > 0.f ? 1.f / (1.f - dp_p) : 1.f;
  p.dp_salt = dp_salt; p.frames_per_sample = frames_per_sample > 0 ? frames_per_sample : 1;
  p.per_frame = per_frame; p.total4 = (long long)frames * per_frame / 4;
  p.skip = FrameSkip{};
}
#define NPVP_CHECK_FRAME_SKIP(who) \
  NPVP_CHECK_ARG(skip_p >= 0.f && skip_p < 1.f && (skip_p == 0.f || (seed && skip_fps > 0)), who ": bad frame-skip arguments")

}

using namespace npvp;

#define LN_LAUNCH(kernel, C, ...)                                                                         \
  switch ((C) / 256) {                                                                                    \
    case 1: NPVP_LAUNCH(kernel<1>, __VA_ARGS__); break;  case 2: NPVP_LAUNCH(kernel<2>, __VA_ARGS__); break;   \
    case 3: NPVP_LAUNCH(kernel<3>, __VA_ARGS__); break;  default: NPVP_LAUNCH(kernel<4>, __VA_ARGS__); break;  \
  }

extern "C" int npvp_layernorm_fwd(const float* x, const float* w, const float* b, float* y, float* mean, float* rstd,
                                  long long rows, int C, float eps, int relu, float* amax, hipStream_t stream) {
  NPVP_CHECK_ARG(rows > 0, "layernorm: no rows");
  NPVP_CHECK_ARG(C % 256 == 0 && C >= 256 && C <= 1024, "layernorm: C must be 256, 512, 768 or 1024");
  const long long nb = (rows + 3) / 4;
  LN_LAUNCH(ln_fwd_kernel, C, dim3((unsigned)(nb > 4096 ? 4096 : nb)), dim3(256), 0, stream, x, w, b, y, mean, rstd, rows, eps, relu, amax);
  NPVP_CHECK_LAUNCH();
  return NPVP_OK;
}

static int ln_bwd_blocks(long long rows) {
  long long b = (rows + 3) / 4;
  return (int)(b > 512 ? 512 : b);
}

static Partials ln_partials(const void* ws, float* dw, float* db, long long rows, int C, int accumulate) {
  const int nb = ln_bwd_blocks(rows);
  return make_partials(ws, 0, nb, nb, 2 * C, dw, accumulate, db, C);
}

extern "C" long long npvp_layernorm_bwd_workspace_bytes(long long rows, int C) {
  return ln_partials(nullptr, nullptr, nullptr, rows, C, 0).bytes;
}

extern "C" int npvp_layernorm_bwd(const float* dy, const float* x, const float* w, const float* b, const float* mean,
                                  const float* rstd, float* dx, float* dw, float* db, long long rows, int C, int relu,
                                  const float* dres, int accumulate, float* amax, void* workspace, long long ws_bytes,
                                  hipStream_t stream) {
  NPVP_CHECK_ARG(rows > 0, "layernorm_bwd: no rows");
  NPVP_CHECK_ARG(C % 256 == 0 && C >= 256 && C <= 1024, "layernorm_bwd: C must be 256, 512, 768 or 1024");
  const Partials P = ln_partials(workspace, dw, db, rows, C, accumulate);
  NPVP_CHECK_ARG(workspace && ws_bytes >= P.bytes, "layernorm_bwd: workspace too small");
  LN_LAUNCH(ln_bwd_kernel, C, dim3(P.job.nb), dim3(256), 0, stream, dy, x, w, b, mean, rstd, dx, P.part(), rows, relu, dres, amax);
  NPVP_CHECK_LAUNCH();
  return finish_partials(P.job, accumulate, stream, "layernorm_bwd: reduce launch failed");
}

extern "C" int npvp_layernorm_bwd_reduce(const void* workspace, float* dw, float* db, long long rows, int C, int accumulate,
                                         hipStream_t stream) {
  NPVP_CHECK_ARG(workspace && dw && db && rows > 0, "layernorm_bwd_reduce: bad arguments");
  return finish_partials(ln_partials(workspace, dw, db, rows, C, accumulate).job, 0, stream, "layernorm_bwd_reduce: launch failed");
}

extern "C" int npvp_layernorm_bwd_reduce_job(const void* workspace, float* dw, float* db, long long rows, int C, int accumulate, void* job) {
  NPVP_CHECK_ARG(workspace && dw && db && rows > 0 && job, "layernorm_bwd_reduce_job: bad arguments");
  return put_job(job, ln_partials(workspace, dw, db, rows, C, accumulate).job);
}

extern "C" int npvp_sum_rows_multi(const void* jobs, int n, hipStream_t stream) {
  NPVP_CHECK_ARG(jobs && n > 0, "sum_rows_multi: no jobs");
  const SumRowsJob* J = (const SumRowsJob*)jobs;
  for (int at = 0; at < n; at += SRJ_MAX) {
    SumRowsBatch b;
    b.n = n - at < SRJ_MAX ? n - at : SRJ_MAX;
    int blocks = 0;
    for (int i = 0; i < b.n; ++i) {
      b.j[i] = J[at + i];
      NPVP_CHECK_ARG(b.j[i].in && b.j[i].out && b.j[i].nb > 0 && b.j[i].ncols > 0, "sum_rows_multi: bad job");
      b.cw[i] = plan_sum_rows(b.j[i]).cw;
      b.first[i] = blocks;
      blocks += (b.j[i].ncols + b.cw[i] - 1) / b.cw[i];
    }
    b.first[b.n] = blocks;
    NPVP_LAUNCH(sum_rows_multi_kernel, dim3(blocks), dim3(1024), 0, stream, b);
    NPVP_CHECK_LAUNCH();
  }
  return NPVP_OK;
}

extern "C" int npvp_layernorm_nchw_fwd(const float* x, const float* w, const float* b, float* out, float* mean, float* rstd,
                                       int frames, int P, int C, float eps, int relu, hipStream_t stream) {
  NPVP_CHECK_ARG(x && w && b && out && mean && rstd && frames > 0, "layernorm_nchw_fwd: bad arguments");
  NPVP_CHECK_ARG(P == 64 && (C == 256 || C == 512), "layernorm_nchw_fwd: 64-pixel frames, C = 256 or 512");
  if (C == 512) NPVP_LAUNCH(ln_nchw_fwd_kernel<512>, dim3(frames), dim3(256), 0, stream, x, w, b, out, mean, rstd, eps, relu);
  else NPVP_LAUNCH(ln_nchw_fwd_kernel<256>, dim3(frames), dim3(256), 0, stream, x, w, b, out, mean, rstd, eps, relu);
  NPVP_CHECK_LAUNCH();
  return NPVP_OK;
}

extern "C" int npvp_frame_stats(const float* x, const float* add, float* mean, float* rstd, int frames, int T,
                                int per_frame, float eps, hipStream_t stream) {
  NPVP_CHECK_ARG(frames > 0 && T > 0 && frames % T == 0, "frame_stats: frames must be a multiple of T");
  NPVP_CHECK_ARG(per_frame % 4 == 0, "frame_stats: per_frame must be a multiple of 4");
  NPVP_LAUNCH(frame_stats_kernel, dim3(frames), dim3(512), 0, stream, x, add, mean, rstd, T, per_frame, eps);
  NPVP_CHECK_LAUNCH();
  return NPVP_OK;
}

extern "C" int npvp_posfuse_fwd(const float* x, const float* add, const float* beta, const float* gamma, float* y,
                                float* mean, float* rstd, int N, int T, int per_frame, float eps, float* amax, hipStream_t stream) {
  NPVP_CHECK_ARG(N > 0 && T > 0 && per_frame % 4 == 0, "posfuse: bad shape");
  const int frames = N * T;
  if (per_frame == 32768) {
    NPVP_LAUNCH((posfuse_fwd_frame_kernel<8>), dim3(frames), dim3(1024), 0, stream, x, add, beta, gamma, y, mean, rstd, T,
                       eps, amax);
    NPVP_CHECK_LAUNCH();
    return NPVP_OK;
  }
  NPVP_LAUNCH(frame_stats_kernel, dim3(frames), dim3(512), 0, stream, x, add, mean, rstd, T, per_frame, eps);
  NPVP_CHECK_LAUNCH();
  const long long total4 = (long long)frames * per_frame / 4;
  NPVP_LAUNCH(posfuse_apply_kernel, dim3(ew_blocks(total4, 256)), dim3(256), 0, stream, x, add, beta, gamma,
                     (const float*)mean, (const float*)rstd, y, T, per_frame, total4, amax);
  NPVP_CHECK_LAUNCH();
  return NPVP_OK;
}

extern "C" int npvp_ln_posfuse_fwd(const float* x, const float* lw, const float* lb, float ln_eps, float* y1, float* ln_mean,
                                   float* ln_rstd, const float* add, const float* beta, const float* gamma, float* fused,
                                   float* pf_mean, float* pf_rstd, int N, int T, int P, int C, float pf_eps, float* y1_amax,
                                   float* fused_amax, hipStream_t stream) {
  NPVP_CHECK_ARG(N > 0 && T > 0 && P == 64 && C == 512, "ln_posfuse_fwd: frames of 64 token rows x 512 channels only");
  NPVP_CHECK_ARG(x && lw && lb && y1 && ln_mean && ln_rstd && beta && fused && pf_mean && pf_rstd, "ln_posfuse_fwd: null argument");
  NPVP_LAUNCH(ln_posfuse_fwd_frame_kernel, dim3(N * T), dim3(1024), 0, stream, x, lw, lb, ln_eps, y1, ln_mean, ln_rstd, add,
                     beta, gamma, fused, pf_mean, pf_rstd, T, pf_eps, y1_amax, fused_amax);
  NPVP_CHECK_LAUNCH();
  return NPVP_OK;
}

extern "C" int npvp_posfuse_bwd_fused(int N, int T, int per_frame) {
  if (per_frame % 1024 != 0) return 0;
  const long long blocks = (long long)T * (per_frame / 1024);
  return (blocks >= 128 || N <= 16) ? 1 : 0;
}

extern "C" int npvp_posfuse_bwd(const float* dy, const float* x, const float* add, const float* gamma, const float* mean,
                                const float* rstd, float* du, float* dyxh, float* dbeta, float* dgamma, int N, int T,
                                int per_frame, int accumulate, void* workspace, long long ws_bytes, hipStream_t stream) {
  const int frames = N * T;
  NPVP_CHECK_ARG(N > 0 && T > 0 && per_frame % 4 == 0, "posfuse_bwd: bad shape");
  NPVP_CHECK_ARG(workspace && ws_bytes >= (long long)frames * 2 * 4, "posfuse_bwd: workspace too small");
  NPVP_CHECK_ARG(!dgamma || gamma, "posfuse_bwd: dgamma without gamma");
  float* s1 = (float*)workspace; float* s2 = s1 + frames;
  NPVP_LAUNCH(posfuse_bwd_stats_kernel, dim3(frames), dim3(512), 0, stream, dy, x, add, gamma, mean, rstd, s1, s2, T,
                     per_frame);
  NPVP_CHECK_LAUNCH();
  if (npvp_posfuse_bwd_fused(N, T, per_frame)) {
    NPVP_LAUNCH(posfuse_bwd_apply_nsum_kernel, dim3(T * (per_frame / 1024)), dim3(256), 0, stream, dy, x, add, gamma, mean,
                       rstd, (const float*)s1, (const float*)s2, du, dbeta, dgamma, N, T, per_frame, accumulate ? 1 : 0);
    NPVP_CHECK_LAUNCH();
    return NPVP_OK;
  }
  NPVP_CHECK_ARG(!dgamma || dyxh, "posfuse_bwd: this shape needs the dy*uhat scratch (dyxh) for dgamma");
  const long long total4 = (long long)frames * per_frame / 4;
  NPVP_LAUNCH(posfuse_bwd_apply_kernel, dim3(ew_blocks(total4, 256)), dim3(256), 0, stream, dy, x, add, gamma, mean,
                     rstd, (const float*)s1, (const float*)s2, du, dgamma ? dyxh : nullptr, T, per_frame, total4);
  NPVP_CHECK_LAUNCH();
  if (dbeta) { const int rc = npvp_reduce_mid_launch(dy, dbeta, 1, N, (long long)T * per_frame, 1.f, stream, accumulate); if (rc) return rc; }
  if (dgamma) { const int rc = npvp_reduce_mid_launch(dyxh, dgamma, 1, N, (long long)T * per_frame, 1.f, stream, accumulate); if (rc) return rc; }
  return NPVP_OK;
}

extern "C" int npvp_posfuse_instance_fwd(const float* x, const float* add, const float* beta, const float* gamma, float* y,
                                         float* mean, float* rstd, int N, int T, int P, int C, float eps, float* y_amax,
                                         hipStream_t stream) {
  NPVP_CHECK_ARG(N > 0 && T > 0 && P > 0 && P <= PFI_MAXP && C > 0, "posfuse_instance: bad shape (P <= 64)");
  NPVP_LAUNCH(posfuse_inst_fwd_kernel, dim3((C + 255) / 256, N * T), dim3(256), 0, stream, x, add, beta, gamma, y, mean,
                     rstd, T, P, C, eps, y_amax);
  NPVP_CHECK_LAUNCH();
  return NPVP_OK;
}

extern "C" int npvp_posfuse_instance_bwd(const float* dy, const float* x, const float* add, const float* gamma, const float* mean,
                                         const float* rstd, float* du, float* dyxh, int N, int T, int P, int C,
                                         hipStream_t stream) {
  NPVP_CHECK_ARG(N > 0 && T > 0 && P > 0 && P <= PFI_MAXP && C > 0, "posfuse_instance_bwd: bad shape (P <= 64)");
  NPVP_LAUNCH(posfuse_inst_bwd_kernel, dim3((C + 255) / 256, N * T), dim3(256), 0, stream, dy, x, add, gamma, mean, rstd,
                     du, dyxh, T, P, C);
  NPVP_CHECK_LAUNCH();
  return NPVP_OK;
}

extern "C" int npvp_frameln_act_fwd(const float* h, const float* mean, const float* rstd, const float* w, const float* b,
                                    const float* res, float* out, int frames, int per_frame, float drop_p,
                                    unsigned int salt, float dp_p, unsigned int dp_salt, int frames_per_sample,
                                    const unsigned long long* seed, float* amax, hipStream_t stream) {
  NPVP_CHECK_ARG(frames > 0 && per_frame % 4 == 0, "frameln_act: bad shape");
  NPVP_CHECK_ARG((drop_p == 0.f && dp_p == 0.f) || seed, "frameln_act: dropout needs a device seed");
  FlnParams p;
  fill_fln(p, h, mean, rstd, w, b, res, frames, per_frame, drop_p, salt, dp_p, dp_salt, frames_per_sample, seed);
  NPVP_LAUNCH(frameln_act_fwd_kernel, dim3(ew_blocks(p.total4, 256)), dim3(256), 0, stream, p, out, amax);
  NPVP_CHECK_LAUNCH();
  return NPVP_OK;
}

extern "C" int npvp_frameln_act_fwd_parts_skip(const float* h, const float* part, int J, float nb, float eps, float* mean, float* rstd,
                                               const float* w, const float* b, const float* res, float* out, int frames,
                                               int per_frame, float drop_p, unsigned int salt, float dp_p, unsigned int dp_salt,
                                               int frames_per_sample, const unsigned long long* seed, float* amax, float skip_p,
                                               unsigned int skip_salt, int skip_fps, hipStream_t stream) {
  NPVP_CHECK_FRAME_SKIP("frameln_act_fwd_parts");
  NPVP_CHECK_ARG(frames > 0 && per_frame % 4096 == 0 && part && J > 0 && nb > 0.f && mean && rstd, "frameln_act_fwd_parts: bad arguments");
  NPVP_CHECK_ARG((drop_p == 0.f && dp_p == 0.f) || seed, "frameln_act: dropout needs a device seed");
  NPVP_CHECK_ARG((long long)frames * (per_frame / 4096) < (1ll << 31), "frameln_act_fwd_parts: too many blocks");
  FlnParams p;
  fill_fln(p, h, nullptr, nullptr, w, b, res, frames, per_frame, drop_p, salt, dp_p, dp_salt, frames_per_sample, seed);
  p.skip = make_frame_skip(skip_p, skip_salt, skip_fps, seed);
  NPVP_LAUNCH(frameln_act_fwd_parts_kernel, dim3((unsigned)((long long)frames * (per_frame / 4096))), dim3(256), 0, stream, p,
                     part, J, nb, eps, mean, rstd, out, amax);
  NPVP_CHECK_LAUNCH();
  return NPVP_OK;
}

extern "C" int npvp_frameln_act_fwd_parts(const float* h, const float* part, int J, float nb, float eps, float* mean, float* rstd,
                                          const float* w, const float* b, const float* res, float* out, int frames,
                                          int per_frame, float drop_p, unsigned int salt, float dp_p, unsigned int dp_salt,
                                          int frames_per_sample, const unsigned long long* seed, float* amax, hipStream_t stream) {
  return npvp_frameln_act_fwd_parts_skip(h, part, J, nb, eps, mean, rstd, w, b, res, out, frames, per_frame, drop_p, salt, dp_p, dp_salt,
                                         frames_per_sample, seed, amax, 0.f, 0u, 1, stream);
}

static int fln_chunks(int frames) {
  if (frames >= 512) return 32;
  const int c = frames / 2 < 16 ? frames / 2 : 16;
  return c < 1 ? 1 : c;
}

static Partials fln_partials(const void* ws, float* dw, float* db, int frames, int per_frame, int accumulate) {
  return make_partials(ws, (long long)frames * 2 * FLN_PARTS, frames, fln_chunks(frames), 2 * per_frame, dw, accumulate, db, per_frame);
}

extern "C" long long npvp_frameln_act_bwd_workspace_bytes(int frames, int per_frame) {
  return fln_partials(nullptr, nullptr, nullptr, frames, per_frame, 0).bytes;
}

static int fln_bwd_fused(const FlnParams& p, const float* dout, const float* psum, int nparts, float* dh, const Partials& P, int frames,
                         int accumulate, float* amax, hipStream_t stream, const char* error) {
  NPVP_LAUNCH(frameln_act_bwd_fused_kernel, dim3((p.per_frame / 4 + 255) / 256, P.job.nb), dim3(256), 0, stream, p,
                     dout, psum, dh, P.part(), frames, P.per, nparts, amax);
  NPVP_CHECK_LAUNCH();
  return finish_partials(P.job, accumulate, stream, error);
}

extern "C" int npvp_frameln_act_bwd(const float* dout, const float* h, const float* mean, const float* rstd, const float* w,
                                    const float* b, float* dh, float* dw, float* db, int frames, int per_frame,
                                    float drop_p, unsigned int salt, float dp_p, unsigned int dp_salt,
                                    int frames_per_sample, const unsigned long long* seed, int accumulate, float* amax,
                                    void* workspace, long long ws_bytes, hipStream_t stream) {
  NPVP_CHECK_ARG(frames > 0 && per_frame % 4 == 0, "frameln_act_bwd: bad shape");
  const Partials P = fln_partials(workspace, dw, db, frames, per_frame, accumulate);
  NPVP_CHECK_ARG(workspace && ws_bytes >= P.bytes, "frameln_act_bwd: workspace too small");
  FlnParams p;
  fill_fln(p, h, mean, rstd, w, b, nullptr, frames, per_frame, drop_p, salt, dp_p, dp_salt, frames_per_sample, seed);
  NPVP_CHECK_ARG(per_frame % (4 * FLN_PARTS) == 0, "frameln_act_bwd: per_frame must be a multiple of 16");
  NPVP_LAUNCH(frameln_act_bwd_stats_kernel, dim3(frames, FLN_PARTS), dim3(512), 0, stream, p, dout, (float*)workspace);
  NPVP_CHECK_LAUNCH();
  return fln_bwd_fused(p, dout, (const float*)workspace, FLN_PARTS, dh, P, frames, accumulate, amax, stream, "frameln_act_bwd: reduce launch failed");
}

extern "C" int npvp_frameln_act_bwd_apply_skip(const float* dout, const float* h, const float* mean, const float* rstd, const float* w,
                                               const float* b, const float* psum, int nparts, float* dh, float* dw, float* db,
                                               int frames, int per_frame, int accumulate, float* amax, void* workspace,
                                               long long ws_bytes, float skip_p, unsigned int skip_salt, int skip_fps,
                                               const unsigned long long* seed, hipStream_t stream) {
  NPVP_CHECK_FRAME_SKIP("frameln_act_bwd_apply");
  NPVP_CHECK_ARG(frames > 0 && per_frame % 4 == 0 && psum && nparts > 0, "frameln_act_bwd_apply: bad arguments");
  const Partials P = fln_partials(workspace, dw, db, frames, per_frame, accumulate);
  NPVP_CHECK_ARG(workspace && ws_bytes >= P.bytes, "frameln_act_bwd_apply: workspace too small");
  FlnParams p;
  fill_fln(p, h, mean, rstd, w, b, nullptr, frames, per_frame, 0.f, 0u, 0.f, 0u, 1, nullptr);
  p.skip = make_frame_skip(skip_p, skip_salt, skip_fps, seed);
  return fln_bwd_fused(p, dout, psum, nparts, dh, P, frames, accumulate, amax, stream, "frameln_act_bwd_apply: reduce launch failed");
}

extern "C" int npvp_frameln_act_bwd_apply(const float* dout, const float* h, const float* mean, const float* rstd, const float* w,
                                          const float* b, const float* psum, int nparts, float* dh, float* dw, float* db,
                                          int frames, int per_frame, int accumulate, float* amax, void* workspace,
                                          long long ws_bytes, hipStream_t stream) {
  return npvp_frameln_act_bwd_apply_skip(dout, h, mean, rstd, w, b, psum, nparts, dh, dw, db, frames, per_frame, accumulate, amax, workspace,
                                         ws_bytes, 0.f, 0u, 1, nullptr, stream);
}

extern "C" int npvp_frameln_act_bwd_pgrad(const float* dout, const float* h, const float* mean, const float* rstd, const float* w,
                                          const float* b, float* psum, float* dw, float* db, int frames, int per_frame,
                                          float drop_p, unsigned int salt, float dp_p, unsigned int dp_salt, int frames_per_sample,
                                          const unsigned long long* seed, int accumulate, void* workspace, long long ws_bytes,
                                          hipStream_t stream) {
  NPVP_CHECK_ARG(frames > 0 && per_frame % 1024 == 0 && psum, "frameln_act_bwd_pgrad: per_frame must be a multiple of 1024");
  const Partials P = fln_partials(workspace, dw, db, frames, per_frame, accumulate);
  NPVP_CHECK_ARG(workspace && ws_bytes >= P.bytes, "frameln_act_bwd_pgrad: workspace too small");
  FlnParams p;
  fill_fln(p, h, mean, rstd, w, b, nullptr, frames, per_frame, drop_p, salt, dp_p, dp_salt, frames_per_sample, seed);
  NPVP_LAUNCH(frameln_act_bwd_pgrad_kernel, dim3(per_frame / 1024, P.job.nb), dim3(256), 0, stream, p, dout, psum,
                     P.part(), frames, P.per);
  NPVP_CHECK_LAUNCH();
  return finish_partials(P.job, accumulate, stream, "frameln_act_bwd_pgrad: reduce launch failed");
}

extern "C" int npvp_frameln_act_bwd_reduce_job(const void* workspace, float* dw, float* db, int frames, int per_frame, int accumulate,
                                               void* job) {
  NPVP_CHECK_ARG(workspace && dw && db && frames > 0 && job, "frameln_act_bwd_reduce_job: bad arguments");
  return put_job(job, fln_partials(workspace, dw, db, frames, per_frame, accumulate).job);
}

extern "C" int npvp_frameln_act_bwd_reduce(const void* workspace, float* dw, float* db, int frames, int per_frame,
                                           int accumulate, hipStream_t stream) {
  NPVP_CHECK_ARG(workspace && dw && db && frames > 0, "frameln_act_bwd_reduce: bad arguments");
  return finish_partials(fln_partials(workspace, dw, db, frames, per_frame, accumulate).job, 0, stream, "frameln_act_bwd_reduce: launch failed");
}
```

### npvp_amd/ops.py

```python
import contextlib
import functools
import os
from collections import namedtuple

import torch

from ._lib import lib, check
from . import sched as _S
from .sched import (_p, _ptr, _stream, _ws, AmaxSlot, GemmProbe, HbmProbe, ProbeEvent, AuxStream, StepContext, current, use, scoped,
                    remember, rng, GradSink, WgradStream, WgradChain, ReduceQueue, RangeGuard)


def amax_of(t, slot=None):
    if slot is not None:
        return slot
    for cand in (t, t._base):
        tag = getattr(cand, "_npvp_amax", None) if cand is not None else None
        if tag is not None and tag[1] == cand._version:
            return tag[0]
    s = AmaxSlot.new(t.device)
    t2 = t if t.dim() == 2 else t.reshape(-1, t.shape[-1])
    if t2.stride(1) != 1:
        t2 = t2.contiguous()
    check(lib().npvp_amax(_ptr(t2), t2.shape[0], t2.shape[1], t2.stride(0), _ptr(s), _stream()), "npvp_amax")
# ... 1042 lines not shown
        self.grid = grid

    @property
    def tiles(self):
        return self.grid is None

    @classmethod
    def spatial(cls, frames, H, W, ws, heads, p_drop):
        Hp, Wp, top, left = window_pad_geometry(H, W, ws)
        grid = None if (Hp, Wp) == (H, W) else (H, W, top, left)
        return cls(0, frames, Hp * Wp, Wp, ws, 0, 0, heads, 0, p_drop, grid)

    def pad_args(self):
        H, W, top, left = self.grid
        return self.dim0, H, W, self.P // self.W, self.W, top, left

    @property
    def padded_rows(self):
        return -(-self.dim0 * self.P // 32) * 32


ATTN_LONG_MIN = 129


def _attn_len(cfg):
    return (cfg.ws * cfg.ws, cfg.ws * cfg.ws) if cfg.mode == 0 else (cfg.Tq, cfg.Tk)


def _attn_groups(cfg):
    return cfg.dim0 * (cfg.P // (cfg.ws * cfg.ws)) if cfg.mode == 0 else cfg.dim0 * cfg.P


def _attn_long(cfg):
    return max(_attn_len(cfg)) >= ATTN_LONG_MIN


def _attn_fwd_entry(cfg):
    return (lib().npvp_attn_long_fwd, "npvp_attn_long_fwd") if _attn_long(cfg) else (lib().npvp_attn_fwd, "npvp_attn_fwd")


def _attn_fwd(q, k, v, o, cfg):
    hd = o.shape[1] // cfg.heads
    seed = _S._cur.rng.seed_for(q.device, cfg.drop)
    if DropRecorder.sites is not None and cfg.drop.on:
        L_, S_ = _attn_len(cfg)
        DropRecorder.note(cfg.drop, "elem", _attn_groups(cfg) * cfg.heads * L_ * S_)
    slot = _new_slot(q.device)
    fn, what = _attn_fwd_entry(cfg)
    check(fn(_ptr(q), q.stride(0), _ptr(k), k.stride(0), _ptr(v), v.stride(0), _ptr(o), o.stride(0),
             cfg.mode, cfg.dim0, cfg.P, cfg.W, cfg.ws, cfg.Tq, cfg.Tk, cfg.heads, hd, cfg.mask_mode,
             cfg.drop.p, _ptr(seed), cfg.drop.salt, _ptr(slot), _stream()), what)
    tag_amax(o, slot)


ATTN_SAMPLES_MAX = 32


def _attn_samples_fwd(q, k, v, o, cfg, S, sample_chunk=0):
    if cfg.mode != 1 or cfg.mask_mode != 0 or cfg.drop.on:
        raise ValueError("_attn_samples_fwd: temporal geometry without mask and dropout only")
    hd = o.shape[1] // cfg.heads
    slot = _new_slot(q.device)
    if max(cfg.Tq, cfg.Tk) <= ATTN_SAMPLES_MAX:
        check(lib().npvp_attn_samples_fwd(_ptr(q), q.stride(0), _ptr(k), k.stride(0), _ptr(v), v.stride(0), _ptr(o), o.stride(0),
                                          S, cfg.dim0, cfg.P, cfg.Tq, cfg.Tk, cfg.heads, hd, sample_chunk, _ptr(slot), _stream()),
              "npvp_attn_samples_fwd")
    else:
        fn, what = _attn_fwd_entry(cfg)
        rows = cfg.dim0 * cfg.Tq * cfg.P
        for s in range(S):
            check(fn(q.data_ptr() + 4 * s * rows * q.stride(0), q.stride(0), _ptr(k), k.stride(0), _ptr(v), v.stride(0),
                     o.data_ptr() + 4 * s * rows * o.stride(0), o.stride(0), 1, cfg.dim0, cfg.P, cfg.W, 0, cfg.Tq, cfg.Tk, cfg.heads,
                     hd, 0, 0.0, None, 0, _ptr(slot), _stream()), what)
    tag_amax(o, slot)


def _attn_bwd(q, k, v, go, dq, dk, dv, cfg, packed=None):
    hd = go.shape[1] // cfg.heads
    seed = _S._cur.rng.seed_for(q.device, cfg.drop)
    sq = _new_slot(q.device)
    sk = sq if packed is not None else _new_slot(q.device)
    sv = _new_slot(q.device)
    args = (_ptr(q), q.stride(0), _ptr(k), k.stride(0), _ptr(v), v.stride(0), _ptr(go), go.stride(0),
            _ptr(dq), dq.stride(0), _ptr(dk), dk.stride(0), _ptr(dv), dv.stride(0), cfg.mode, cfg.dim0,
            cfg.P, cfg.W, cfg.ws, cfg.Tq, cfg.Tk, cfg.heads, hd, cfg.mask_mode, cfg.drop.p, _ptr(seed),
            cfg.drop.salt, _ptr(sq), _ptr(sk), _ptr(sv))
    if _attn_long(cfg):
        ws, wsn = _ws(lib().npvp_attn_long_bwd_workspace_bytes(cfg.mode, cfg.dim0, cfg.P, cfg.W, cfg.ws, cfg.Tq, cfg.Tk, cfg.heads),
                      q.device)
        check(lib().npvp_attn_long_bwd(*args, _ptr(ws), wsn, _stream()), "npvp_attn_long_bwd")
    else:
        check(lib().npvp_attn_bwd(*args, _stream()), "npvp_attn_bwd")
    if packed is not None:
        tag_amax(packed, sq)
    else:
        tag_amax(dq, sq); tag_amax(dk, sk)
    tag_amax(dv, sv)


class _AttnPacked(_Function):

    @staticmethod
    def forward(ctx, qk, v, cfg):
        remember(ctx)
        _chk(qk, v)
        C = v.shape[1]
        o = torch.empty_like(v)
        _attn_fwd(qk[:, :C], qk[:, C:], v, o, cfg)
        ctx.save_for_backward(qk, v)
        ctx.cfg = cfg
        return o

    @scoped
    def backward(ctx, go):
        qk, v = ctx.saved_tensors
        C = v.shape[1]
        go = _c(go)
        dqk, dv = torch.empty_like(qk), torch.empty_like(v)
        _attn_bwd(qk[:, :C], qk[:, C:], v, go, dqk[:, :C], dqk[:, C:], dv, ctx.cfg, packed=dqk)
        if not ctx.cfg.tiles:
            _zero_tail(ctx.cfg, dqk, dv)
        return dqk, dv, None


class _Attn(_Function):

    @staticmethod
    def forward(ctx, q, k, v, cfg):
        remember(ctx)
        _chk(q, k, v)
        o = torch.empty_like(q)
        _attn_fwd(q, k, v, o, cfg)
        ctx.save_for_backward(q, k, v)
        ctx.cfg = cfg
        return o

    @scoped
    def backward(ctx, go):
        q, k, v = ctx.saved_tensors
        go = _c(go)
        dq, dk, dv = torch.empty_like(q), torch.empty_like(k), torch.empty_like(v)
        _attn_bwd(q, k, v, go, dq, dk, dv, ctx.cfg)
        return dq, dk, dv, None


def attn_packed(qk, v, cfg):
    return _AttnPacked.apply(qk, v, cfg)


def attn(q, k, v, cfg):
    return _Attn.apply(q, k, v, cfg)


def _fln_bwd(dout, h, mean, rstd, w, b, frames, PF, d, dp, T, sk, psum=None, nparts=0, want_amax=True, skip=NO_SKIP):
    L = lib()
    dev = h.device
    dh = torch.empty_like(h)
    slot = _new_slot(dev, want_amax)
    tag_amax(dh, slot)
    dw, db = (sk[0][0], sk[1][0]) if sk else (torch.empty_like(w), torch.empty_like(b))
    ws, wsn = _ws(L.npvp_frameln_act_bwd_workspace_bytes(frames, PF), dev)
    mode = _sink_mode(sk)
    if psum is None:
        seed = _S._cur.rng.seed_for(dev, d, dp)
        check(L.npvp_frameln_act_bwd(_ptr(dout), _ptr(h), _ptr(mean), _ptr(rstd), _ptr(w), _ptr(b), _ptr(dh), _ptr(dw), _ptr(db),
                                     frames, PF, d.p, d.salt, dp.p, dp.salt, T, _ptr(seed), mode, _ptr(slot), _ptr(ws), wsn,
                                     _stream()), "npvp_frameln_act_bwd")
    else:
        pe = HbmProbe.begin()
        check(L.npvp_frameln_act_bwd_apply_skip(_ptr(dout), _ptr(h), _ptr(mean), _ptr(rstd), _ptr(w), _ptr(b), _ptr(psum), nparts,
                                                _ptr(dh), _ptr(dw), _ptr(db), frames, PF, mode, _ptr(slot), _ptr(ws), wsn, *skip.frame,
                                                _ptr(_S._cur.rng.seed_for(dev, skip.frame)), _stream()), "npvp_frameln_act_bwd_apply_skip")
        HbmProbe.end(pe, "npvp::frameln_act_bwd_fused_kernel", 4.0 * 3 * frames * PF)
    if sk:
        _reduce_partials(sk, ws, dw, db, L.npvp_frameln_act_bwd_reduce, L.npvp_frameln_act_bwd_reduce_job, "npvp_frameln_act_bwd_reduce",
                         (frames, PF, 1), True)
        return dh, None, None
    return dh, dw, db


def _fln_pgrad(dout, h, mean, rstd, w, b, frames, PF, d, sk):
    L = lib()
    dev = h.device
    psum = torch.empty(frames * (PF // 1024) * 2, dtype=torch.float32, device=dev)
    dw, db = (sk[0][0], sk[1][0]) if sk else (torch.empty_like(w), torch.empty_like(b))
    ws, wsn = _ws(L.npvp_frameln_act_bwd_workspace_bytes(frames, PF), dev)
    seed = _S._cur.rng.seed_for(dev, d)
    check(L.npvp_frameln_act_bwd_pgrad(_ptr(dout), _ptr(h), mean, rstd, _ptr(w), _ptr(b), _ptr(psum), _ptr(dw), _ptr(db),
                                       frames, PF, d.p, d.salt, 0.0, 0, 1, _ptr(seed), _sink_mode(sk), _ptr(ws), wsn, _stream()),
          "npvp_frameln_act_bwd_pgrad")
    if sk:
        _reduce_partials(sk, ws, dw, db, L.npvp_frameln_act_bwd_reduce, L.npvp_frameln_act_bwd_reduce_job, "npvp_frameln_act_bwd_reduce",
                         (frames, PF, 1), True)
        return psum, None, None
    return psum, dw, db


class _FrameLnAct(_Function):

    @staticmethod
    def forward(ctx, h, w_cl, b_cl, res, frames, p_drop, p_dp, frames_per_sample, mean=None, rstd=None):
        remember(ctx)
        _chk(h, w_cl, b_cl, res)
        h = _c(h)
        PF = h.numel() // frames
        w_cl, b_cl = _c(w_cl), _c(b_cl)
        res_c = None if res is None else _c(res)
        L = lib()
        if mean is None:
            mean = torch.empty(frames, dtype=torch.float32, device=h.device)
            rstd = torch.empty_like(mean)
            check(L.npvp_frame_stats(_ptr(h), _p(0), _ptr(mean), _ptr(rstd), frames, 1, PF, 1e-5, _stream()), "npvp_frame_stats")
        d, dp = Drop(p_drop), Drop(p_dp, 1)
        DropRecorder.note(d, "elem", h.numel())
        DropRecorder.note(dp, "group", frames // max(1, frames_per_sample))
        out = torch.empty_like(h)
        seed = _S._cur.rng.seed_for(h.device, d, dp)
        slot = _new_slot(h.device)
        check(L.npvp_frameln_act_fwd(_ptr(h), _ptr(mean), _ptr(rstd), _ptr(w_cl), _ptr(b_cl), _ptr(res_c), _ptr(out), frames,
                                     PF, d.p, d.salt, dp.p, dp.salt, frames_per_sample, _ptr(seed), _ptr(slot), _stream()),
              "npvp_frameln_act_fwd")
        tag_amax(out, slot)
        ctx.save_for_backward(h, mean, rstd, w_cl, b_cl)
        ctx.cfg = (frames, PF, d, dp, frames_per_sample, res is not None)
        ctx.sink = _ln_sink(w_cl, b_cl)
        return out

    @scoped
    def backward(ctx, dout):
        h, mean, rstd, w_cl, b_cl = ctx.saved_tensors
        frames, PF, d, dp, fps, has_res = ctx.cfg
        dout = _c(dout)
        dh, dw, db = _fln_bwd(dout, h, mean, rstd, w_cl, b_cl, frames, PF, d, dp, fps, ctx.sink)
        return dh, dw, db, (dout if has_res else None), None, None, None, None, None, None


def frameln_act(h, w_cl, b_cl, res, frames, p_drop=0.0, p_dp=0.0, frames_per_sample=1, stats=None):
    mean, rstd = stats if stats is not None else (None, None)
    return _FrameLnAct.apply(h, w_cl, b_cl, res, frames, p_drop, p_dp, frames_per_sample, mean, rstd)


class _DwConv(_Function):

    @staticmethod
    def forward(ctx, a, wtb, frames, H, W, want_stats):
        remember(ctx)
        _chk(a, wtb)
        a, wtb = _c(a), _c(wtb)
        Ch = wtb.shape[1]
        out = torch.empty_like(a)
        ctx.save_for_backward(a, wtb)
        ctx.cfg = (frames, H, W, Ch)
        if want_stats:
            mean = torch.empty(frames, dtype=torch.float32, device=a.device)
            rstd = torch.empty_like(mean)
            ws, wsn = _ws(frames * (Ch // 1024) * 8, a.device)
            check(lib().npvp_dwconv3x3_stats(_ptr(a), _ptr(wtb), _row(wtb, 9), _ptr(out), _ptr(mean), _ptr(rstd), frames, H, W,
                                             Ch, 1e-5, _ptr(ws), wsn, _stream()), "npvp_dwconv3x3_stats")
            ctx.mark_non_differentiable(mean, rstd)
            ctx.set_materialize_grads(False)
            return out, mean, rstd
        check(lib().npvp_dwconv3x3(_ptr(a), _ptr(wtb), _row(wtb, 9), _ptr(out), frames, H, W, Ch, 0, _stream()),
              "npvp_dwconv3x3")
        return out

    @scoped
    def backward(ctx, dout, *_unused):
        a, wtb = ctx.saved_tensors
        frames, H, W, Ch = ctx.cfg
        dout = _c(dout)
        L = lib()
        da = torch.empty_like(a)
        check(L.npvp_dwconv3x3(_ptr(dout), _ptr(wtb), _p(0), _ptr(da), frames, H, W, Ch, 1, _stream()), "npvp_dwconv3x3(bwd)")
        dwtb = torch.empty_like(wtb)
        ws, wsn = _ws(L.npvp_dwconv3x3_wgrad_workspace_bytes(frames, Ch), a.device)
        check(L.npvp_dwconv3x3_wgrad(_ptr(a), _ptr(dout), _ptr(dwtb), frames, H, W, Ch, _ptr(ws), wsn, _stream()),
              "npvp_dwconv3x3_wgrad")
        return da, dwtb, None, None, None, None


def dwconv3x3(a, wtb, frames, H, W, want_stats=False):
    return _DwConv.apply(a, wtb, frames, H, W, bool(want_stats))


class _MlpDwbn(_Function):

    @staticmethod
    def forward(ctx, x, res, w1, b1, n1w, n1b, dww, dwb, n2w, n2b, w2, b2, n3w, n3b, frames, T, p_drop, p_dp):
        remember(ctx)
        _chk(x, res, w1, b1, w2, b2)
        L = lib()
        R, C = x.shape
        hid, Co = w1.shape[0], w2.shape[0]
        dev, f32 = x.device, torch.float32
        st = _stream()
        PFh, PFo = 64 * hid, 64 * Co
        d2, d3, dp = Drop(p_drop), Drop(p_drop), Drop(p_dp, 1)
        ctx.skip = skip = SampleSkip.of(skip_roles("mlpdwbn", DROP_PATH_SKIP, WGRAD_ROW_SKIP), dp, T * 64, frames // max(1, T), R)
        seed = _S._cur.rng.seed_for(dev, d2, dp)
        h1 = torch.empty(R, hid, dtype=f32, device=dev)
        part = torch.empty(frames * (hid // 64) * 2, dtype=f32, device=dev)
        gemm(1, 1, R, hid, C, x, x.stride(0), w1, w1.stride(0), h1, bias=b1, b_pre=_planes(w1, "F", R), rowstats=part, row_skip=skip.forward)
        stats = torch.empty(6, frames, dtype=f32, device=dev)
        key = (WeightPlanes.epoch, dww._version, dwb._version, dww.data_ptr(), dwb.data_ptr())
        hit = dww.__dict__.get("_npvp_wtb")
        if hit is not None and hit[0] == key:
            wtb = hit[1]
        else:
            wtb = torch.empty(10, hid, dtype=f32, device=dev)
            check(L.npvp_dwtb_build(_ptr(_c(dww)), _ptr(dwb), _ptr(wtb), hid, st), "npvp_dwtb_build")
            dww.__dict__["_npvp_wtb"] = (key, wtb)
        h2 = torch.empty(R, hid, dtype=f32, device=dev)
        part2 = torch.empty(frames * (hid // 512) * 2, dtype=f32, device=dev)
        check(L.npvp_mlpdw_mid_fwd_parts_skip(_ptr(h1), _ptr(part), hid // 64, 4096.0, _row(stats, 0), _row(stats, 1), _ptr(n1w),
                                              _ptr(n1b), _ptr(wtb), _row(wtb, 9), _ptr(h2), _ptr(part2), frames, 8, 8, hid, 1e-5,
                                              *skip.frame, _ptr(seed), st), "npvp_mlpdw_mid_fwd_parts_skip")
        DropRecorder.note(d2, "elem", R * hid)
        a2 = torch.empty(R, hid, dtype=f32, device=dev)
        a2_slot = _new_slot(dev)
        check(L.npvp_frameln_act_fwd_parts_skip(_ptr(h2), _ptr(part2), hid // 512, 32768.0, 1e-5, _row(stats, 2), _row(stats, 3),
                                                _ptr(n2w), _ptr(n2b), None, _ptr(a2), frames, PFh, d2.p, d2.salt, 0.0, 0, 1, _ptr(seed),
                                                _ptr(a2_slot), *skip.frame, st), "npvp_frameln_act_fwd_parts_skip")
        tag_amax(a2, a2_slot)
        h3 = torch.empty(R, Co, dtype=f32, device=dev)
        part3 = torch.empty(frames * (Co // 64) * 2, dtype=f32, device=dev)
        gemm(1, 1, R, Co, hid, a2, hid, w2, w2.stride(0), h3, bias=b2, b_pre=_planes(w2, "F", R), rowstats=part3, row_skip=skip.forward)
        DropRecorder.note(d3, "elem", R * Co)
        DropRecorder.note(dp, "group", frames // max(1, T))
        out = torch.empty(R, Co, dtype=f32, device=dev)
        check(L.npvp_frameln_act_fwd_parts_skip(_ptr(h3), _ptr(part3), Co // 64, 4096.0, 1e-5, _row(stats, 4), _row(stats, 5),
                                                _ptr(n3w), _ptr(n3b), _ptr(res), _ptr(out), frames, PFo, d3.p, d3.salt, dp.p, dp.salt, T,
                                                _ptr(seed), None, *skip.frame, st), "npvp_frameln_act_fwd_parts_skip")
        ctx.save_for_backward(x, h1, h2, a2, h3, stats, wtb, w1, w2, n1w, n1b, n2w, n2b, n3w, n3b)
        ctx.cfg = (frames, T, d2, d3, dp, res is not None, b1 is not None, b2 is not None)
        ctx.sinks = (_wb_sink(w1, b1), _wb_sink(w2, b2), _ln_sink(n1w, n1b), _ln_sink(n2w, n2b), _ln_sink(n3w, n3b))
        sd = _wb_sink(dww, dwb) if (dww.is_contiguous() and dwb is not None) else None
        ctx.sink_dw = sd if (sd and sd[1] is not None) else None
        return out

    @scoped
    def backward(ctx, dout):
        x, h1, h2, a2, h3, stats, wtb, w1, w2, n1w, n1b, n2w, n2b, n3w, n3b = ctx.saved_tensors
        frames, T, d2, d3, dp, has_res, has_b1, has_b2 = ctx.cfg
        s_fc1, s_fc2, s_n1, s_n2, s_n3 = ctx.sinks
        L = lib()
        R, hid = h1.shape
        Co = h3.shape[1]
        dev = x.device
        dout = _c(dout)
        dh3, gn3w, gn3b = _fln_bwd(dout, h3, stats[4], stats[5], n3w, n3b, frames, 64 * Co, d3, dp, T, s_n3)
        da2, gw2, gb2 = linear_bwd(dh3, a2, w2, True if has_b2 else None, s_fc2, skip=ctx.skip)
        fuse_n2 = MID_BWD_N2 and hid // 16 <= 256
        if fuse_n2:
            psum2, gn2w, gn2b = _fln_pgrad(da2, h2, _row(stats, 2), _row(stats, 3), n2w, n2b, frames, 64 * hid, d2, s_n2)
        else:
            dh2, gn2w, gn2b = _fln_bwd(da2, h2, stats[2], stats[3], n2w, n2b, frames, 64 * hid, d2, NO_DROP, 1, s_n2,
                                          want_amax=False)
            del da2
        da1 = torch.empty_like(h1)
        dwtb = torch.empty(10, hid, dtype=torch.float32, device=dev)
        nparts = hid // 256
        psum = torch.empty(frames * nparts * 2, dtype=torch.float32, device=dev)
        ws, wsn = _ws(L.npvp_mlpdw_mid_bwd_workspace_bytes(frames, hid), dev)
        sk_dw = ctx.sink_dw if ctx.needs_input_grad[6] and ctx.needs_input_grad[7] else None
        wmode = 2 if sk_dw else 0
        if fuse_n2:
            seed = _S._cur.rng.seed_for(dev, d2)
            pe = HbmProbe.begin()
            check(L.npvp_mlpdw_mid_bwd_n2(_ptr(da2), _ptr(h2), _row(stats, 2), _row(stats, 3), _ptr(n2w), _ptr(n2b), _ptr(psum2),
                                          hid // 16, d2.p, d2.salt, _ptr(seed), _ptr(h1), _row(stats, 0), _row(stats, 1), _ptr(n1w),
                                          _ptr(n1b), _ptr(wtb), _ptr(da1), _ptr(dwtb), _ptr(psum), frames, 8, 8, hid, wmode, _ptr(ws), wsn,
                                          _stream()), "npvp_mlpdw_mid_bwd_n2")
            HbmProbe.end(pe, "npvp::mlpdw_mid_bwd_kernel<1, true>", 4.0 * 4 * frames * 64 * hid)
            del da2, psum2
        else:
            check(L.npvp_mlpdw_mid_bwd(_ptr(dh2), _ptr(h1), _row(stats, 0), _row(stats, 1), _ptr(n1w), _ptr(n1b), _ptr(wtb), _ptr(da1),
                                       _ptr(dwtb), _ptr(psum), frames, 8, 8, hid, wmode, _ptr(ws), wsn, _stream()), "npvp_mlpdw_mid_bwd")
            del dh2
        if sk_dw:
            _reduce_partials(sk_dw, ws, sk_dw[0][0], sk_dw[1][0], L.npvp_mlpdw_mid_bwd_reduce_into, L.npvp_mlpdw_mid_bwd_reduce_job,
                             "npvp_mlpdw_mid_bwd_reduce_into", (frames, hid), False)
            gdww = gdwb = None
        else:
            gdww = torch.empty(hid, 1, 3, 3, dtype=torch.float32, device=dev)
            check(L.npvp_transpose(_ptr(dwtb), _ptr(gdww), 1, 9, hid, _stream()), "npvp_transpose")
            gdwb = dwtb[9]
        dh1, gn1w, gn1b = _fln_bwd(da1, h1, stats[0], stats[1], n1w, n1b, frames, 64 * hid, NO_DROP, NO_DROP, 1, s_n1,
                                      psum=psum, nparts=nparts, skip=ctx.skip)
        del da1
        dx, gw1, gb1 = linear_bwd(dh1, x, w1, True if has_b1 else None, s_fc1, skip=ctx.skip)
        return (dx, dout if has_res else None, gw1, gb1, gn1w, gn1b, gdww, gdwb, gn2w, gn2b, gw2, gb2, gn3w, gn3b,
                None, None, None, None)


MID_BWD_N2 = True
DROP_PATH_SKIP = True
WGRAD_ROW_SKIP = True


def mlpdwbn_fused_supported(R, C, hid, Co, H, W):
    return (GEMM_PRECISION in (4, 6) and H == 8 and W == 8 and R % 64 == 0 and hid % 512 == 0 and Co % 128 == 0 and hid % 128 == 0
            and C % 32 == 0)


def mlpdwbn(x, res, w1, b1, n1w, n1b, dww, dwb, n2w, n2b, w2, b2, n3w, n3b, frames, T, p_drop, p_dp):
    return _MlpDwbn.apply(x, res, w1, b1, n1w, n1b, dww, dwb, n2w, n2b, w2, b2, n3w, n3b, frames, T, p_drop, p_dp)


def _raw_ln_fwd(x2, w, b, eps, relu=0):
    rows, C = x2.shape
    y = torch.empty_like(x2)
    st = torch.empty(2, rows, dtype=torch.float32, device=x2.device)
    slot = _new_slot(x2.device)
    check(lib().npvp_layernorm_fwd(_ptr(x2), _ptr(w), _ptr(b), _ptr(y), _row(st, 0), _row(st, 1), rows, C, eps, relu, _ptr(slot),
                                   _stream()), "npvp_layernorm_fwd")
    return tag_amax(y, slot), st


def _raw_ln_bwd(dy2, x2, w, b, st, dres, sk, relu=0, probe=False):
    L = lib()
    rows, C = x2.shape
    dx = torch.empty_like(x2)
    dw, db = (sk[0][0], sk[1][0]) if sk else (torch.empty_like(w), torch.empty_like(b))
    ws, wsn = _ws(L.npvp_layernorm_bwd_workspace_bytes(rows, C), x2.device)
    slot = _new_slot(x2.device)
    pe = HbmProbe.begin() if probe else None
    check(L.npvp_layernorm_bwd(_ptr(dy2), _ptr(x2), _ptr(w), _ptr(b), _row(st, 0), _row(st, 1), _ptr(dx), _ptr(dw), _ptr(db), rows, C,
                               relu, _ptr(dres), _sink_mode(sk), _ptr(slot), _ptr(ws), wsn, _stream()), "npvp_layernorm_bwd")
    HbmProbe.end(pe, "npvp::ln_bwd_kernel<2>", 4.0 * (3 + (dres is not None)) * rows * C)
    tag_amax(dx, slot)
    if sk:
        _reduce_partials(sk, ws, dw, db, L.npvp_layernorm_bwd_reduce, L.npvp_layernorm_bwd_reduce_job, "npvp_layernorm_bwd_reduce",
                         (rows, C, 1), True)
        return dx, None, None
    return dx, dw, db


def _raw_posfuse_fwd(x, add, beta, gamma, N, T):
    PF = x.numel() // (N * T)
    y = torch.empty_like(x)
    st = torch.empty(2, N * T, dtype=torch.float32, device=x.device)
    slot = _new_slot(x.device)
    check(lib().npvp_posfuse_fwd(_ptr(x), _ptr(add), _ptr(beta), _ptr(gamma), _ptr(y), _row(st, 0), _row(st, 1), N, T, PF, 1e-5,
                                 _ptr(slot), _stream()), "npvp_posfuse_fwd")
    return tag_amax(y, slot), st


LN_POSFUSE_ONE_KERNEL = True


def _raw_ln_posfuse_fwd(x2, lw, lb, eps, add, beta, gamma, N, T):
    rows, C = x2.shape
    if not (LN_POSFUSE_ONE_KERNEL and C == 512 and rows == N * T * 64):
        x1, lst = _raw_ln_fwd(x2, lw, lb, eps)
        fused, pst = _raw_posfuse_fwd(x1, add, beta, gamma, N, T)
        return x1, lst, fused, pst
    x1, fused = torch.empty_like(x2), torch.empty_like(x2)
    lst = torch.empty(2, rows, dtype=torch.float32, device=x2.device)
    pst = torch.empty(2, N * T, dtype=torch.float32, device=x2.device)
    s1, s2 = _new_slot(x2.device), _new_slot(x2.device)
    check(lib().npvp_ln_posfuse_fwd(_ptr(x2), _ptr(lw), _ptr(lb), eps, _ptr(x1), _row(lst, 0), _row(lst, 1), _ptr(add), _ptr(beta),
                                    _ptr(gamma), _ptr(fused), _row(pst, 0), _row(pst, 1), N, T, 64, C, 1e-5, _ptr(s1), _ptr(s2),
                                    _stream()), "npvp_ln_posfuse_fwd")
    return tag_amax(x1, s1), lst, tag_amax(fused, s2), pst


def _raw_posfuse_bwd(dy, x, add, beta_shape, gamma, st, N, T, want_add, sinks=(None, None, None)):
    PF = x.numel() // (N * T)
    du, dbeta, dgamma = _posfuse_bwd_call(dy, x, add, gamma, st, N, T, PF, beta_shape, True, gamma is not None,
                                          sinks[0], sinks[1])
    dadd = None
    if add is not None and want_add:
        if sinks[2] is not None:
            buf, acc = sinks[2].target(add.shape, x.device)
            reduce_mid(du.view(N, T, PF), out=buf.view(N, PF), accumulate=acc)
        else:
            dadd = reduce_mid(du.view(N, T, PF)).view(add.shape)
    return du, dadd, dbeta, dgamma


def _raw_grid_pad(x2, cfg, want_amax=True, out=None):
    F_, H, W, Hp, Wp, top, left = cfg.pad_args()
    rows = cfg.padded_rows
    if out is None:
        out = torch.empty(rows, x2.shape[1], dtype=torch.float32, device=x2.device)
    C = out.shape[1]
    if (0 if x2 is None else x2.shape[0]) != F_ * H * W or (x2 is not None and x2.stride(1) != 1) or out.shape[0] != rows or out.stride(1) != 1:
        raise RuntimeError(f"grid pad: {None if x2 is None else tuple(x2.shape)} -> {tuple(out.shape)} is not {F_} frames of {H} x {W} "
                           f"unit-stride token rows -> {rows} rows")
    slot = _new_slot(out.device, want_amax)
    check(lib().npvp_grid_center_pad(_ptr(x2), C if x2 is None else x2.stride(0), _ptr(out), out.stride(0), F_, H, W, Hp, Wp, top, left, C,
                                     rows, _ptr(slot), _stream()), "npvp_grid_center_pad")
    return tag_amax(out, slot)


def _raw_grid_cut(xp, cfg, addend=None, want_amax=False):
    F_, H, W, Hp, Wp, top, left = cfg.pad_args()
    C = xp.shape[1]
    if xp.shape[0] < F_ * Hp * Wp or xp.stride(1) != 1 or (addend is not None and (addend.shape != (F_ * H * W, C) or addend.stride(1) != 1)):
        raise RuntimeError(f"grid cut: {tuple(xp.shape)} does not hold {F_} frames of {Hp} x {Wp} unit-stride token rows")
    out = torch.empty(F_ * H * W, C, dtype=torch.float32, device=xp.device)
    slot = _new_slot(xp.device, want_amax)
    check(lib().npvp_grid_center_cut(_ptr(xp), xp.stride(0), _ptr(addend), 0 if addend is None else addend.stride(0), _ptr(out),
                                     out.stride(0), F_, H, W, Hp, Wp, top, left, C, _ptr(slot), _stream()), "npvp_grid_center_cut")
    return tag_amax(out, slot)


class _ZeroRows:
    __slots__ = ("padded_rows",)

    def __init__(self, rows):
        self.padded_rows = rows

    def pad_args(self):
        return 0, 1, 1, 1, 1, 0, 0


def _zero_tail(cfg, *ts):
    body = cfg.dim0 * cfg.P
    for t in ts:
        if t.shape[0] > body:
            _raw_grid_pad(None, _ZeroRows(t.shape[0] - body), want_amax=False, out=t[body:])


class _GridPad(_Function):
    @staticmethod
    def forward(ctx, x2, cfg):
        remember(ctx)
        _chk(x2)
        ctx.cfg = cfg
        return _raw_grid_pad(_c(x2), cfg)

    @scoped
    def backward(ctx, g):
        return _raw_grid_cut(_c(g), ctx.cfg), None


class _GridCut(_Function):
    @staticmethod
    def forward(ctx, xp, cfg):
        remember(ctx)
        _chk(xp)
        ctx.cfg = cfg
        return _raw_grid_cut(_c(xp), cfg, want_amax=True)

    @scoped
    def backward(ctx, g):
        return _raw_grid_pad(_c(g), ctx.cfg), None
# ... 740 lines not shown
```

Before: 8657.

## Store dropout keep masks as bitmasks in forward and reuse them in backward

```diff
diff --git a/include/npvp_hip.h b/include/npvp_hip.h
--- a/include/npvp_hip.h
+++ b/include/npvp_hip.h
@@ -175,6 +175,27 @@
                                     int per_frame, int accumulate, float* dh_amax, void* workspace, long long ws_bytes,
                                     float skip_p, unsigned int skip_salt, int skip_fps, const unsigned long long* seed,
                                     npvp_stream_t stream);
+int npvp_frameln_act_fwd_parts_skip_bits(const float* h, const float* part, int J, float nb, float eps, float* mean, float* rstd,
+                                         const float* w, const float* b, const float* res, float* out, int frames, int per_frame,
+                                         float drop_p, unsigned int salt, float dp_p, unsigned int dp_salt, int frames_per_sample,
+                                         const unsigned long long* seed, float* out_amax, float skip_p, unsigned int skip_salt,
+                                         int skip_fps, unsigned int* drop_bits, npvp_stream_t stream);
+int npvp_frameln_act_bwd_bits(const float* dout, const float* h, const float* mean, const float* rstd, const float* w,
+                              const float* b, float* dh, float* dw, float* db, int frames, int per_frame, float drop_p,
+                              unsigned int salt, float dp_p, unsigned int dp_salt, int frames_per_sample,
+                              const unsigned long long* seed, int accumulate, float* dh_amax, void* workspace, long long ws_bytes,
+                              const unsigned int* drop_bits, npvp_stream_t stream);
+int npvp_frameln_act_bwd_pgrad_bits(const float* dout, const float* h, const float* mean, const float* rstd, const float* w,
+                                    const float* b, float* psum, float* dw, float* db, int frames, int per_frame, float drop_p,
+                                    unsigned int salt, float dp_p, unsigned int dp_salt, int frames_per_sample,
+                                    const unsigned long long* seed, int accumulate, void* workspace, long long ws_bytes,
+                                    const unsigned int* drop_bits, npvp_stream_t stream);
+int npvp_mlpdw_mid_bwd_n2_bits(const float* da2, const float* h2, const float* mean2, const float* rstd2, const float* w2n,
+                               const float* b2n, const float* psum2, int nparts2, float drop_p, unsigned int salt,
+                               const unsigned long long* seed, const float* h1, const float* mean1, const float* rstd1,
+                               const float* w1n, const float* b1n, const float* wt, float* da1, float* dwt_db, float* psum, int frames,
+                               int H, int W, int Ch, int accumulate, void* workspace, long long ws_bytes,
+                               const unsigned int* drop_bits, npvp_stream_t stream);
 
 int npvp_im2col3x3(const float* in, float* out, int frames, int H, int W, int C, int col2im, npvp_stream_t stream);
 long long npvp_dwconv3x3_wgrad_workspace_bytes(int frames, int Ch);
diff --git a/npvp_amd/csrc/common.h b/npvp_amd/csrc/common.h
--- a/npvp_amd/csrc/common.h
+++ b/npvp_amd/csrc/common.h
@@ -172,6 +172,9 @@
 __device__ __forceinline__ float drop_scale(uint64_t seed, uint32_t salt, uint64_t idx, uint32_t thresh, float inv_keep) {
   return rng_u32(seed, salt, idx) >= thresh ? inv_keep : 0.f;
 }
+__device__ __forceinline__ unsigned int drop_bits_nibble(const unsigned int* __restrict__ bits, long long g0) {
+  return (unsigned int)reinterpret_cast<const unsigned char*>(bits)[g0 >> 3] >> ((unsigned int)g0 & 4u);
+}
 __host__ __device__ __forceinline__ uint32_t drop_threshold(float p) {
   double t = (double)p * 4294967296.0;
   if (t < 0) t = 0;
diff --git a/npvp_amd/csrc/mlpdw.hip b/npvp_amd/csrc/mlpdw.hip
--- a/npvp_amd/csrc/mlpdw.hip
+++ b/npvp_amd/csrc/mlpdw.hip
@@ -196,9 +196,14 @@
   const float* h2; const float* mean2; const float* rstd2; const float* w2n; const float* b2n;
   const float* psum2; int nparts2;
   const unsigned long long* seed; unsigned int drop_thresh; float drop_inv_keep; unsigned int salt;
+  const unsigned int* drop_bits;
 };
 
-template <int VEC, bool FUSE2>
+__device__ __forceinline__ unsigned long long lane_u64(unsigned long long v, int lane) {
+  const unsigned int lo = __builtin_amdgcn_readlane((int)(unsigned int)v, lane), hi = __builtin_amdgcn_readlane((int)(unsigned int)(v >> 32), lane);
+  return ((unsigned long long)hi << 32) | lo;
+}
+template <int VEC, bool FUSE2, bool BITS>
 __global__ __launch_bounds__(256, NPVP_MID_BWD_WAVES) void mlpdw_mid_bwd_kernel(const float* __restrict__ dh2, const float* __restrict__ h1,
                                                             const float* __restrict__ mean1, const float* __restrict__ rstd1,
                                                             const float* __restrict__ w1n, const float* __restrict__ b1n,
@@ -209,6 +214,7 @@
   __shared__ float red[4];
   const unsigned long long seed2 = (FUSE2 && n2.seed && n2.drop_thresh) ? *n2.seed : 0ull;
   const int c = (blockIdx.x * blockDim.x + threadIdx.x) * VEC;
+  const int cw = __builtin_amdgcn_readfirstlane(c);
   const int nblk = gridDim.x;
   Vec<VEC> wv[9], aw[9], ab;
 #pragma unroll
@@ -227,6 +233,9 @@
     float* of = da1 + f * (HH * WW) * Ch;
     float mu2 = 0.f, rs2 = 0.f, c1 = 0.f, c2 = 0.f;
     const float* h2f = nullptr;
+    unsigned long long kept = 0ull;
+    if constexpr (BITS)
+      kept = reinterpret_cast<const unsigned long long*>(n2.drop_bits)[(f * (HH * WW) * Ch + (long long)(threadIdx.x & 63) * Ch + cw) >> 6];
     if constexpr (FUSE2) {
       mu2 = n2.mean2[f]; rs2 = n2.rstd2[f];
       h2f = n2.h2 + f * (HH * WW) * Ch;
@@ -250,8 +259,12 @@
             for (int e = 0; e < VEC; ++e) {
               const float xh2 = (x2.v[e] - mu2) * rs2;
               float m = 1.f;
-              if (n2.drop_thresh)
-                m = drop_scale(seed2, n2.salt, (unsigned long long)(f * (HH * WW) * Ch + off + e), n2.drop_thresh, n2.drop_inv_keep);
+              if (n2.drop_thresh) {
+                if constexpr (BITS)
+                  m = __builtin_amdgcn_inverse_ballot_w64(lane_u64(kept, hh * WW + w)) ? n2.drop_inv_keep : 0.f;
+                else
+                  m = drop_scale(seed2, n2.salt, (unsigned long long)(f * (HH * WW) * Ch + off + e), n2.drop_thresh, n2.drop_inv_keep);
+              }
               const float dyln = d2.v[e] * m * gelu_grad_f(xh2 * w2.v[e] + b2.v[e]);
               grow[w].v[e] = rs2 * (dyln * w2.v[e] - c1 - xh2 * c2);
             }
@@ -572,11 +585,14 @@
   NPVP_CHECK_ARG(frames > 0 && H == 8 && W == 8 && Ch > 0 && Ch % 512 == 0, "mlpdw_mid_bwd: needs an 8x8 grid and Ch % 512 == 0");
   NPVP_CHECK_ARG(workspace && ws_bytes >= npvp_mlpdw_mid_bwd_workspace_bytes(frames, Ch), "mlpdw_mid_bwd: workspace too small");
   const Partials P = mid_partials(workspace, dwt_db, nullptr, frames, Ch, accumulate);
-  if (n2)
-    NPVP_LAUNCH((mlpdw_mid_bwd_kernel<1, true>), dim3(Ch / 256, P.job.nb), dim3(256), 0, stream, dh2, h1, mean1, rstd1, w1n,
+  if (n2 && n2->drop_bits && n2->drop_thresh)
+    NPVP_LAUNCH((mlpdw_mid_bwd_kernel<1, true, true>), dim3(Ch / 256, P.job.nb), dim3(256), 0, stream, dh2, h1, mean1, rstd1, w1n,
+                       b1n, wt, da1, P.part(), psum, Ch, frames, P.per, *n2);
+  else if (n2)
+    NPVP_LAUNCH((mlpdw_mid_bwd_kernel<1, true, false>), dim3(Ch / 256, P.job.nb), dim3(256), 0, stream, dh2, h1, mean1, rstd1, w1n,
                        b1n, wt, da1, P.part(), psum, Ch, frames, P.per, *n2);
   else
-    NPVP_LAUNCH((mlpdw_mid_bwd_kernel<1, false>), dim3(Ch / 256, P.job.nb), dim3(256), 0, stream, dh2, h1, mean1, rstd1, w1n,
+    NPVP_LAUNCH((mlpdw_mid_bwd_kernel<1, false, false>), dim3(Ch / 256, P.job.nb), dim3(256), 0, stream, dh2, h1, mean1, rstd1, w1n,
                        b1n, wt, da1, P.part(), psum, Ch, frames, P.per, MidN2{});
   NPVP_CHECK_LAUNCH();
   return finish_partials(P.job, accumulate, stream, "mlpdw_mid_bwd: reduce launch failed");
@@ -587,6 +603,23 @@
                                   int W, int Ch, int accumulate, void* workspace, long long ws_bytes, hipStream_t stream) {
   return mid_bwd_launch(dh2, h1, mean1, rstd1, w1n, b1n, wt, da1, dwt_db, psum, frames, H, W, Ch, accumulate, workspace, ws_bytes,
                         stream, nullptr);
+}
+
+extern "C" int npvp_mlpdw_mid_bwd_n2_bits(const float* da2, const float* h2, const float* mean2, const float* rstd2, const float* w2n,
+                                          const float* b2n, const float* psum2, int nparts2, float drop_p, unsigned int salt,
+                                          const unsigned long long* seed, const float* h1, const float* mean1, const float* rstd1,
+                                          const float* w1n, const float* b1n, const float* wt, float* da1, float* dwt_db, float* psum,
+                                          int frames, int H, int W, int Ch, int accumulate, void* workspace, long long ws_bytes,
+                                          const unsigned int* drop_bits, hipStream_t stream) {
+  NPVP_CHECK_ARG(h2 && mean2 && rstd2 && w2n && b2n && psum2 && nparts2 > 0 && nparts2 <= 256, "mlpdw_mid_bwd_n2: bad norm2 arguments");
+  NPVP_CHECK_ARG(drop_p >= 0.f && drop_p < 1.f && (drop_p == 0.f || seed || drop_bits), "mlpdw_mid_bwd_n2: bad dropout arguments");
+  NPVP_CHECK_ARG(((uintptr_t)drop_bits & 7) == 0, "mlpdw_mid_bwd_n2: drop_bits must be 8-byte aligned");
+  MidN2 n2;
+  n2.h2 = h2; n2.mean2 = mean2; n2.rstd2 = rstd2; n2.w2n = w2n; n2.b2n = b2n; n2.psum2 = psum2; n2.nparts2 = nparts2;
+  n2.seed = seed; n2.drop_thresh = drop_p > 0.f ? drop_threshold(drop_p) : 0u;
+  n2.drop_inv_keep = drop_p > 0.f ? 1.f / (1.f - drop_p) : 1.f; n2.salt = salt; n2.drop_bits = drop_bits;
+  return mid_bwd_launch(da2, h1, mean1, rstd1, w1n, b1n, wt, da1, dwt_db, psum, frames, H, W, Ch, accumulate, workspace, ws_bytes,
+                        stream, &n2);
 }
 
 extern "C" int npvp_mlpdw_mid_bwd_n2(const float* da2, const float* h2, const float* mean2, const float* rstd2, const float* w2n,
@@ -595,14 +628,8 @@
                                      const float* w1n, const float* b1n, const float* wt, float* da1, float* dwt_db, float* psum,
                                      int frames, int H, int W, int Ch, int accumulate, void* workspace, long long ws_bytes,
                                      hipStream_t stream) {
-  NPVP_CHECK_ARG(h2 && mean2 && rstd2 && w2n && b2n && psum2 && nparts2 > 0 && nparts2 <= 256, "mlpdw_mid_bwd_n2: bad norm2 arguments");
-  NPVP_CHECK_ARG(drop_p >= 0.f && drop_p < 1.f && (drop_p == 0.f || seed), "mlpdw_mid_bwd_n2: bad dropout arguments");
-  MidN2 n2;
-  n2.h2 = h2; n2.mean2 = mean2; n2.rstd2 = rstd2; n2.w2n = w2n; n2.b2n = b2n; n2.psum2 = psum2; n2.nparts2 = nparts2;
-  n2.seed = seed; n2.drop_thresh = drop_p > 0.f ? drop_threshold(drop_p) : 0u;
-  n2.drop_inv_keep = drop_p > 0.f ? 1.f / (1.f - drop_p) : 1.f; n2.salt = salt;
-  return mid_bwd_launch(da2, h1, mean1, rstd1, w1n, b1n, wt, da1, dwt_db, psum, frames, H, W, Ch, accumulate, workspace, ws_bytes,
-                        stream, &n2);
+  return npvp_mlpdw_mid_bwd_n2_bits(da2, h2, mean2, rstd2, w2n, b2n, psum2, nparts2, drop_p, salt, seed, h1, mean1, rstd1, w1n, b1n, wt, da1,
+                                    dwt_db, psum, frames, H, W, Ch, accumulate, workspace, ws_bytes, nullptr, stream);
 }
 
 __global__ void mid_bwd_reduce_into_kernel(const float* __restrict__ part, float* __restrict__ gw, float* __restrict__ gb, int Ch,
diff --git a/npvp_amd/csrc/norm.hip b/npvp_amd/csrc/norm.hip
--- a/npvp_amd/csrc/norm.hip
+++ b/npvp_amd/csrc/norm.hip
@@ -554,15 +554,26 @@
   unsigned int dp_thresh; float dp_inv_keep; unsigned int dp_salt; int frames_per_sample;
   int per_frame; long long total4;
   FrameSkip skip;
+  const unsigned int* drop_bits;
 };
 
 __device__ __forceinline__ float fln_frame_scale(const FlnParams& p, unsigned long long seed, long long f) {
   if (!p.dp_thresh) return 1.f;
   return drop_scale(seed, p.dp_salt, (unsigned long long)((unsigned int)f / (unsigned int)p.frames_per_sample), p.dp_thresh, p.dp_inv_keep);
 }
-__device__ __forceinline__ float fln_scale(const FlnParams& p, unsigned long long seed, float frame_scale, long long gidx) {
+__device__ __forceinline__ float fln_scale(const FlnParams& p, unsigned long long seed, float frame_scale, long long gidx, unsigned int stored) {
   if (!p.drop_thresh) return frame_scale;
+  if (p.drop_bits) return ((stored & 1u) ? p.drop_inv_keep : 0.f) * frame_scale;
   return drop_scale(seed, p.salt, (unsigned long long)gidx, p.drop_thresh, p.drop_inv_keep) * frame_scale;
+}
+__device__ __forceinline__ unsigned int fln_stored4(const FlnParams& p, long long g0) {
+  return (p.drop_bits && p.drop_thresh) ? drop_bits_nibble(p.drop_bits, g0) : 0u;
+}
+__device__ __forceinline__ unsigned int fln_hash_keep4(const FlnParams& p, unsigned long long seed, long long g0) {
+  unsigned int k = 0u;
+#pragma unroll
+  for (int i = 0; i < 4; ++i) k |= (rng_u32(seed, p.salt, (unsigned long long)(g0 + i)) >= p.drop_thresh ? 1u : 0u) << i;
+  return k;
 }
 
 __global__ void frameln_act_fwd_kernel(FlnParams p, float* __restrict__ out, float* __restrict__ amax) {
@@ -579,10 +590,11 @@
     const float4 v = ld4(p.h + f * p.per_frame + e), ww = ld4(p.w + e), bb = ld4(p.b + e);
     const long long g0 = f * p.per_frame + e;
     float4 o;
-    o.x = gelu_f((v.x - mu) * rs * ww.x + bb.x) * fln_scale(p, seed, fsc, g0 + 0);
-    o.y = gelu_f((v.y - mu) * rs * ww.y + bb.y) * fln_scale(p, seed, fsc, g0 + 1);
-    o.z = gelu_f((v.z - mu) * rs * ww.z + bb.z) * fln_scale(p, seed, fsc, g0 + 2);
-    o.w = gelu_f((v.w - mu) * rs * ww.w + bb.w) * fln_scale(p, seed, fsc, g0 + 3);
+    const unsigned int st4b = 0u;
+    o.x = gelu_f((v.x - mu) * rs * ww.x + bb.x) * fln_scale(p, seed, fsc, g0 + 0, st4b >> 0);
+    o.y = gelu_f((v.y - mu) * rs * ww.y + bb.y) * fln_scale(p, seed, fsc, g0 + 1, st4b >> 1);
+    o.z = gelu_f((v.z - mu) * rs * ww.z + bb.z) * fln_scale(p, seed, fsc, g0 + 2, st4b >> 2);
+    o.w = gelu_f((v.w - mu) * rs * ww.w + bb.w) * fln_scale(p, seed, fsc, g0 + 3, st4b >> 3);
     if (p.res) { const float4 r = ld4(p.res + g0); o.x += r.x; o.y += r.y; o.z += r.z; o.w += r.w; }
     st4(out + g0, o);
     am = amax4(am, o);
@@ -590,10 +602,18 @@
   amax_slot_commit_block(amax, am, ared, peek);
 }
 
+__device__ __forceinline__ void fln_store_keep4(unsigned int* __restrict__ bits, long long g0, unsigned int keep) {
+  unsigned int w = keep << ((threadIdx.x & 7) * 4);
+  w |= (unsigned int)__builtin_amdgcn_update_dpp(0, (int)w, 0xB1, 0xF, 0xF, false);
+  w |= (unsigned int)__builtin_amdgcn_update_dpp(0, (int)w, 0x4E, 0xF, 0xF, false);
+  w |= (unsigned int)__builtin_amdgcn_update_dpp(0, (int)w, 0x141, 0xF, 0xF, false);
+  if ((threadIdx.x & 7) == 0) bits[g0 >> 5] = w;
+}
+
 __global__ __launch_bounds__(256) void frameln_act_fwd_parts_kernel(FlnParams p, const float* __restrict__ part, int J, float nb,
                                                                     float eps, float* __restrict__ mean_out,
                                                                     float* __restrict__ rstd_out, float* __restrict__ out,
-                                                                    float* __restrict__ amax) {
+                                                                    float* __restrict__ amax, unsigned int* __restrict__ bits_out) {
   __shared__ float ared[16];
   const unsigned int peek = amax_peek_block(amax);
   const int bpf = p.per_frame / 4096;
@@ -609,6 +629,7 @@
 #pragma unroll
     for (int k = 0; k < 4; ++k) {
       const long long g0 = f * p.per_frame + e0 + (k * 256 + threadIdx.x) * 4;
+      if (bits_out && p.drop_thresh) fln_store_keep4(bits_out, g0, fln_hash_keep4(p, seed, g0));
       const float4 o = p.res ? ld4(p.res + g0) : make_float4(0.f, 0.f, 0.f, 0.f);
       st4(out + g0, o);
       am = amax4(am, o);
@@ -622,10 +643,18 @@
     const long long g0 = f * p.per_frame + e;
     const float4 v = ld4(p.h + g0), ww = ld4(p.w + e), bb = ld4(p.b + e);
     float4 o;
-    o.x = gelu_f((v.x - mu) * rs * ww.x + bb.x) * fln_scale(p, seed, fsc, g0 + 0);
-    o.y = gelu_f((v.y - mu) * rs * ww.y + bb.y) * fln_scale(p, seed, fsc, g0 + 1);
-    o.z = gelu_f((v.z - mu) * rs * ww.z + bb.z) * fln_scale(p, seed, fsc, g0 + 2);
-    o.w = gelu_f((v.w - mu) * rs * ww.w + bb.w) * fln_scale(p, seed, fsc, g0 + 3);
+    const unsigned int st4b = 0u;
+    const float s0 = fln_scale(p, seed, fsc, g0 + 0, st4b >> 0), s1 = fln_scale(p, seed, fsc, g0 + 1, st4b >> 1);
+    const float s2 = fln_scale(p, seed, fsc, g0 + 2, st4b >> 2), s3 = fln_scale(p, seed, fsc, g0 + 3, st4b >> 3);
+    o.x = gelu_f((v.x - mu) * rs * ww.x + bb.x) * s0;
+    o.y = gelu_f((v.y - mu) * rs * ww.y + bb.y) * s1;
+    o.z = gelu_f((v.z - mu) * rs * ww.z + bb.z) * s2;
+    o.w = gelu_f((v.w - mu) * rs * ww.w + bb.w) * s3;
+    if (bits_out && p.drop_thresh) {
+      const unsigned int keep = fsc != 0.f ? ((s0 != 0.f ? 1u : 0u) | (s1 != 0.f ? 2u : 0u) | (s2 != 0.f ? 4u : 0u) | (s3 != 0.f ? 8u : 0u))
+                                           : fln_hash_keep4(p, seed, g0);
+      fln_store_keep4(bits_out, g0, keep);
+    }
     if (p.res) { const float4 r = ld4(p.res + g0); o.x += r.x; o.y += r.y; o.z += r.z; o.w += r.w; }
     st4(out + g0, o);
     am = amax4(am, o);
@@ -647,10 +676,11 @@
     const long long g0 = f * p.per_frame + e;
     const float4 v = ld4(p.h + g0), ww = ld4(p.w + e), bb = ld4(p.b + e), d = ld4(dout + g0);
     const float hx = (v.x - mu) * rs, hy = (v.y - mu) * rs, hz = (v.z - mu) * rs, hw = (v.w - mu) * rs;
-    const float gx = d.x * fln_scale(p, seed, fsc, g0 + 0) * gelu_grad_f(hx * ww.x + bb.x) * ww.x;
-    const float gy = d.y * fln_scale(p, seed, fsc, g0 + 1) * gelu_grad_f(hy * ww.y + bb.y) * ww.y;
-    const float gz = d.z * fln_scale(p, seed, fsc, g0 + 2) * gelu_grad_f(hz * ww.z + bb.z) * ww.z;
-    const float gw = d.w * fln_scale(p, seed, fsc, g0 + 3) * gelu_grad_f(hw * ww.w + bb.w) * ww.w;
+    const unsigned int st4b = fln_stored4(p, g0);
+    const float gx = d.x * fln_scale(p, seed, fsc, g0 + 0, st4b >> 0) * gelu_grad_f(hx * ww.x + bb.x) * ww.x;
+    const float gy = d.y * fln_scale(p, seed, fsc, g0 + 1, st4b >> 1) * gelu_grad_f(hy * ww.y + bb.y) * ww.y;
+    const float gz = d.z * fln_scale(p, seed, fsc, g0 + 2, st4b >> 2) * gelu_grad_f(hz * ww.z + bb.z) * ww.z;
+    const float gw = d.w * fln_scale(p, seed, fsc, g0 + 3, st4b >> 3) * gelu_grad_f(hw * ww.w + bb.w) * ww.w;
     s1 += gx + gy + gz + gw;
     s2 += gx * hx + gy * hy + gz * hz + gw * hw;
   }
@@ -684,10 +714,11 @@
     a1 /= p.per_frame; a2 /= p.per_frame;
     const float4 v = ld4(p.h + g0), d = ld4(dout + g0);
     const float hx = (v.x - mu) * rs, hy = (v.y - mu) * rs, hz = (v.z - mu) * rs, hw = (v.w - mu) * rs;
-    const float dx_ = d.x * fln_scale(p, seed, fsc, g0 + 0) * gelu_grad_f(hx * ww.x + bb.x);
-    const float dy_ = d.y * fln_scale(p, seed, fsc, g0 + 1) * gelu_grad_f(hy * ww.y + bb.y);
-    const float dz_ = d.z * fln_scale(p, seed, fsc, g0 + 2) * gelu_grad_f(hz * ww.z + bb.z);
-    const float dw_ = d.w * fln_scale(p, seed, fsc, g0 + 3) * gelu_grad_f(hw * ww.w + bb.w);
+    const unsigned int st4b = fln_stored4(p, g0);
+    const float dx_ = d.x * fln_scale(p, seed, fsc, g0 + 0, st4b >> 0) * gelu_grad_f(hx * ww.x + bb.x);
+    const float dy_ = d.y * fln_scale(p, seed, fsc, g0 + 1, st4b >> 1) * gelu_grad_f(hy * ww.y + bb.y);
+    const float dz_ = d.z * fln_scale(p, seed, fsc, g0 + 2, st4b >> 2) * gelu_grad_f(hz * ww.z + bb.z);
+    const float dw_ = d.w * fln_scale(p, seed, fsc, g0 + 3, st4b >> 3) * gelu_grad_f(hw * ww.w + bb.w);
     aw.x += dx_ * hx; aw.y += dy_ * hy; aw.z += dz_ * hz; aw.w += dw_ * hw;
     ab.x += dx_; ab.y += dy_; ab.z += dz_; ab.w += dw_;
     float4 o;
@@ -720,10 +751,11 @@
     const float fsc = fln_frame_scale(p, seed, f);
     const float4 v = ld4(p.h + g0), d = ld4(dout + g0);
     const float hx = (v.x - mu) * rs, hy = (v.y - mu) * rs, hz = (v.z - mu) * rs, hw = (v.w - mu) * rs;
-    const float dx_ = d.x * fln_scale(p, seed, fsc, g0 + 0) * gelu_grad_f(hx * ww.x + bb.x);
-    const float dy_ = d.y * fln_scale(p, seed, fsc, g0 + 1) * gelu_grad_f(hy * ww.y + bb.y);
-    const float dz_ = d.z * fln_scale(p, seed, fsc, g0 + 2) * gelu_grad_f(hz * ww.z + bb.z);
-    const float dw_ = d.w * fln_scale(p, seed, fsc, g0 + 3) * gelu_grad_f(hw * ww.w + bb.w);
+    const unsigned int st4b = fln_stored4(p, g0);
+    const float dx_ = d.x * fln_scale(p, seed, fsc, g0 + 0, st4b >> 0) * gelu_grad_f(hx * ww.x + bb.x);
+    const float dy_ = d.y * fln_scale(p, seed, fsc, g0 + 1, st4b >> 1) * gelu_grad_f(hy * ww.y + bb.y);
+    const float dz_ = d.z * fln_scale(p, seed, fsc, g0 + 2, st4b >> 2) * gelu_grad_f(hz * ww.z + bb.z);
+    const float dw_ = d.w * fln_scale(p, seed, fsc, g0 + 3, st4b >> 3) * gelu_grad_f(hw * ww.w + bb.w);
     aw.x += dx_ * hx; aw.y += dy_ * hy; aw.z += dz_ * hz; aw.w += dw_ * hw;
     ab.x += dx_; ab.y += dy_; ab.z += dz_; ab.w += dw_;
     const float gx = dx_ * ww.x, gy = dy_ * ww.y, gz = dz_ * ww.z, gw = dw_ * ww.w;
@@ -803,6 +835,7 @@
   p.dp_salt = dp_salt; p.frames_per_sample = frames_per_sample > 0 ? frames_per_sample : 1;
   p.per_frame = per_frame; p.total4 = (long long)frames * per_frame / 4;
   p.skip = FrameSkip{};
+  p.drop_bits = nullptr;
 }
 #define NPVP_CHECK_FRAME_SKIP(who) \
   NPVP_CHECK_ARG(skip_p >= 0.f && skip_p < 1.f && (skip_p == 0.f || (seed && skip_fps > 0)), who ": bad frame-skip arguments")
@@ -1002,11 +1035,11 @@
   return NPVP_OK;
 }
 
-extern "C" int npvp_frameln_act_fwd_parts_skip(const float* h, const float* part, int J, float nb, float eps, float* mean, float* rstd,
-                                               const float* w, const float* b, const float* res, float* out, int frames,
-                                               int per_frame, float drop_p, unsigned int salt, float dp_p, unsigned int dp_salt,
-                                               int frames_per_sample, const unsigned long long* seed, float* amax, float skip_p,
-                                               unsigned int skip_salt, int skip_fps, hipStream_t stream) {
+extern "C" int npvp_frameln_act_fwd_parts_skip_bits(const float* h, const float* part, int J, float nb, float eps, float* mean, float* rstd,
+                                                    const float* w, const float* b, const float* res, float* out, int frames,
+                                                    int per_frame, float drop_p, unsigned int salt, float dp_p, unsigned int dp_salt,
+                                                    int frames_per_sample, const unsigned long long* seed, float* amax, float skip_p,
+                                                    unsigned int skip_salt, int skip_fps, unsigned int* drop_bits, hipStream_t stream) {
   NPVP_CHECK_FRAME_SKIP("frameln_act_fwd_parts");
   NPVP_CHECK_ARG(frames > 0 && per_frame % 4096 == 0 && part && J > 0 && nb > 0.f && mean && rstd, "frameln_act_fwd_parts: bad arguments");
   NPVP_CHECK_ARG((drop_p == 0.f && dp_p == 0.f) || seed, "frameln_act: dropout needs a device seed");
@@ -1015,9 +1048,18 @@
   fill_fln(p, h, nullptr, nullptr, w, b, res, frames, per_frame, drop_p, salt, dp_p, dp_salt, frames_per_sample, seed);
   p.skip = make_frame_skip(skip_p, skip_salt, skip_fps, seed);
   NPVP_LAUNCH(frameln_act_fwd_parts_kernel, dim3((unsigned)((long long)frames * (per_frame / 4096))), dim3(256), 0, stream, p,
-                     part, J, nb, eps, mean, rstd, out, amax);
+                     part, J, nb, eps, mean, rstd, out, amax, drop_p > 0.f ? drop_bits : (unsigned int*)nullptr);
   NPVP_CHECK_LAUNCH();
   return NPVP_OK;
+}
+
+extern "C" int npvp_frameln_act_fwd_parts_skip(const float* h, const float* part, int J, float nb, float eps, float* mean, float* rstd,
+                                               const float* w, const float* b, const float* res, float* out, int frames,
+                                               int per_frame, float drop_p, unsigned int salt, float dp_p, unsigned int dp_salt,
+                                               int frames_per_sample, const unsigned long long* seed, float* amax, float skip_p,
+                                               unsigned int skip_salt, int skip_fps, hipStream_t stream) {
+  return npvp_frameln_act_fwd_parts_skip_bits(h, part, J, nb, eps, mean, rstd, w, b, res, out, frames, per_frame, drop_p, salt, dp_p, dp_salt,
+                                              frames_per_sample, seed, amax, skip_p, skip_salt, skip_fps, nullptr, stream);
 }
 
 extern "C" int npvp_frameln_act_fwd_parts(const float* h, const float* part, int J, float nb, float eps, float* mean, float* rstd,
@@ -1050,20 +1092,30 @@
   return finish_partials(P.job, accumulate, stream, error);
 }
 
+extern "C" int npvp_frameln_act_bwd_bits(const float* dout, const float* h, const float* mean, const float* rstd, const float* w,
+                                         const float* b, float* dh, float* dw, float* db, int frames, int per_frame,
+                                         float drop_p, unsigned int salt, float dp_p, unsigned int dp_salt,
+                                         int frames_per_sample, const unsigned long long* seed, int accumulate, float* amax,
+                                         void* workspace, long long ws_bytes, const unsigned int* drop_bits, hipStream_t stream) {
+  NPVP_CHECK_ARG(frames > 0 && per_frame % 4 == 0, "frameln_act_bwd: bad shape");
+  const Partials P = fln_partials(workspace, dw, db, frames, per_frame, accumulate);
+  NPVP_CHECK_ARG(workspace && ws_bytes >= P.bytes, "frameln_act_bwd: workspace too small");
+  FlnParams p;
+  fill_fln(p, h, mean, rstd, w, b, nullptr, frames, per_frame, drop_p, salt, dp_p, dp_salt, frames_per_sample, seed);
+  p.drop_bits = drop_bits;
+  NPVP_CHECK_ARG(per_frame % (4 * FLN_PARTS) == 0, "frameln_act_bwd: per_frame must be a multiple of 16");
+  NPVP_LAUNCH(frameln_act_bwd_stats_kernel, dim3(frames, FLN_PARTS), dim3(512), 0, stream, p, dout, (float*)workspace);
+  NPVP_CHECK_LAUNCH();
+  return fln_bwd_fused(p, dout, (const float*)workspace, FLN_PARTS, dh, P, frames, accumulate, amax, stream, "frameln_act_bwd: reduce launch failed");
+}
+
 extern "C" int npvp_frameln_act_bwd(const float* dout, const float* h, const float* mean, const float* rstd, const float* w,
                                     const float* b, float* dh, float* dw, float* db, int frames, int per_frame,
                                     float drop_p, unsigned int salt, float dp_p, unsigned int dp_salt,
                                     int frames_per_sample, const unsigned long long* seed, int accumulate, float* amax,
                                     void* workspace, long long ws_bytes, hipStream_t stream) {
-  NPVP_CHECK_ARG(frames > 0 && per_frame % 4 == 0, "frameln_act_bwd: bad shape");
-  const Partials P = fln_partials(workspace, dw, db, frames, per_frame, accumulate);
-  NPVP_CHECK_ARG(workspace && ws_bytes >= P.bytes, "frameln_act_bwd: workspace too small");
-  FlnParams p;
-  fill_fln(p, h, mean, rstd, w, b, nullptr, frames, per_frame, drop_p, salt, dp_p, dp_salt, frames_per_sample, seed);
-  NPVP_CHECK_ARG(per_frame % (4 * FLN_PARTS) == 0, "frameln_act_bwd: per_frame must be a multiple of 16");
-  NPVP_LAUNCH(frameln_act_bwd_stats_kernel, dim3(frames, FLN_PARTS), dim3(512), 0, stream, p, dout, (float*)workspace);
-  NPVP_CHECK_LAUNCH();
-  return fln_bwd_fused(p, dout, (const float*)workspace, FLN_PARTS, dh, P, frames, accumulate, amax, stream, "frameln_act_bwd: reduce launch failed");
+  return npvp_frameln_act_bwd_bits(dout, h, mean, rstd, w, b, dh, dw, db, frames, per_frame, drop_p, salt, dp_p, dp_salt, frames_per_sample,
+                                   seed, accumulate, amax, workspace, ws_bytes, nullptr, stream);
 }
 
 extern "C" int npvp_frameln_act_bwd_apply_skip(const float* dout, const float* h, const float* mean, const float* rstd, const float* w,
@@ -1089,20 +1141,30 @@
                                          ws_bytes, 0.f, 0u, 1, nullptr, stream);
 }
 
+extern "C" int npvp_frameln_act_bwd_pgrad_bits(const float* dout, const float* h, const float* mean, const float* rstd, const float* w,
+                                               const float* b, float* psum, float* dw, float* db, int frames, int per_frame,
+                                               float drop_p, unsigned int salt, float dp_p, unsigned int dp_salt, int frames_per_sample,
+                                               const unsigned long long* seed, int accumulate, void* workspace, long long ws_bytes,
+                                               const unsigned int* drop_bits, hipStream_t stream) {
+  NPVP_CHECK_ARG(frames > 0 && per_frame % 1024 == 0 && psum, "frameln_act_bwd_pgrad: per_frame must be a multiple of 1024");
+  const Partials P = fln_partials(workspace, dw, db, frames, per_frame, accumulate);
+  NPVP_CHECK_ARG(workspace && ws_bytes >= P.bytes, "frameln_act_bwd_pgrad: workspace too small");
+  FlnParams p;
+  fill_fln(p, h, mean, rstd, w, b, nullptr, frames, per_frame, drop_p, salt, dp_p, dp_salt, frames_per_sample, seed);
+  p.drop_bits = drop_bits;
+  NPVP_LAUNCH(frameln_act_bwd_pgrad_kernel, dim3(per_frame / 1024, P.job.nb), dim3(256), 0, stream, p, dout, psum,
+                     P.part(), frames, P.per);
+  NPVP_CHECK_LAUNCH();
+  return finish_partials(P.job, accumulate, stream, "frameln_act_bwd_pgrad: reduce launch failed");
+}
+
 extern "C" int npvp_frameln_act_bwd_pgrad(const float* dout, const float* h, const float* mean, const float* rstd, const float* w,
                                           const float* b, float* psum, float* dw, float* db, int frames, int per_frame,
                                           float drop_p, unsigned int salt, float dp_p, unsigned int dp_salt, int frames_per_sample,
                                           const unsigned long long* seed, int accumulate, void* workspace, long long ws_bytes,
                                           hipStream_t stream) {
-  NPVP_CHECK_ARG(frames > 0 && per_frame % 1024 == 0 && psum, "frameln_act_bwd_pgrad: per_frame must be a multiple of 1024");
-  const Partials P = fln_partials(workspace, dw, db, frames, per_frame, accumulate);
-  NPVP_CHECK_ARG(workspace && ws_bytes >= P.bytes, "frameln_act_bwd_pgrad: workspace too small");
-  FlnParams p;
-  fill_fln(p, h, mean, rstd, w, b, nullptr, frames, per_frame, drop_p, salt, dp_p, dp_salt, frames_per_sample, seed);
-  NPVP_LAUNCH(frameln_act_bwd_pgrad_kernel, dim3(per_frame / 1024, P.job.nb), dim3(256), 0, stream, p, dout, psum,
-                     P.part(), frames, P.per);
-  NPVP_CHECK_LAUNCH();
-  return finish_partials(P.job, accumulate, stream, "frameln_act_bwd_pgrad: reduce launch failed");
+  return npvp_frameln_act_bwd_pgrad_bits(dout, h, mean, rstd, w, b, psum, dw, db, frames, per_frame, drop_p, salt, dp_p, dp_salt,
+                                         frames_per_sample, seed, accumulate, workspace, ws_bytes, nullptr, stream);
 }
 
 extern "C" int npvp_frameln_act_bwd_reduce_job(const void* workspace, float* dw, float* db, int frames, int per_frame, int accumulate,
diff --git a/npvp_amd/ops.py b/npvp_amd/ops.py
--- a/npvp_amd/ops.py
+++ b/npvp_amd/ops.py
@@ -1218,7 +1218,7 @@
     return _Attn.apply(q, k, v, cfg)
 
 
-def _fln_bwd(dout, h, mean, rstd, w, b, frames, PF, d, dp, T, sk, psum=None, nparts=0, want_amax=True, skip=NO_SKIP):
+def _fln_bwd(dout, h, mean, rstd, w, b, frames, PF, d, dp, T, sk, psum=None, nparts=0, want_amax=True, skip=NO_SKIP, bits=None):
     L = lib()
     dev = h.device
     dh = torch.empty_like(h)
@@ -1229,9 +1229,9 @@
     mode = _sink_mode(sk)
     if psum is None:
         seed = _S._cur.rng.seed_for(dev, d, dp)
-        check(L.npvp_frameln_act_bwd(_ptr(dout), _ptr(h), _ptr(mean), _ptr(rstd), _ptr(w), _ptr(b), _ptr(dh), _ptr(dw), _ptr(db),
-                                     frames, PF, d.p, d.salt, dp.p, dp.salt, T, _ptr(seed), mode, _ptr(slot), _ptr(ws), wsn,
-                                     _stream()), "npvp_frameln_act_bwd")
+        check(L.npvp_frameln_act_bwd_bits(_ptr(dout), _ptr(h), _ptr(mean), _ptr(rstd), _ptr(w), _ptr(b), _ptr(dh), _ptr(dw), _ptr(db),
+                                          frames, PF, d.p, d.salt, dp.p, dp.salt, T, _ptr(seed), mode, _ptr(slot), _ptr(ws), wsn,
+                                          _ptr(bits), _stream()), "npvp_frameln_act_bwd_bits")
     else:
         pe = HbmProbe.begin()
         check(L.npvp_frameln_act_bwd_apply_skip(_ptr(dout), _ptr(h), _ptr(mean), _ptr(rstd), _ptr(w), _ptr(b), _ptr(psum), nparts,
@@ -1245,16 +1245,16 @@
     return dh, dw, db
 
 
-def _fln_pgrad(dout, h, mean, rstd, w, b, frames, PF, d, sk):
+def _fln_pgrad(dout, h, mean, rstd, w, b, frames, PF, d, sk, bits=None):
     L = lib()
     dev = h.device
     psum = torch.empty(frames * (PF // 1024) * 2, dtype=torch.float32, device=dev)
     dw, db = (sk[0][0], sk[1][0]) if sk else (torch.empty_like(w), torch.empty_like(b))
     ws, wsn = _ws(L.npvp_frameln_act_bwd_workspace_bytes(frames, PF), dev)
     seed = _S._cur.rng.seed_for(dev, d)
-    check(L.npvp_frameln_act_bwd_pgrad(_ptr(dout), _ptr(h), mean, rstd, _ptr(w), _ptr(b), _ptr(psum), _ptr(dw), _ptr(db),
-                                       frames, PF, d.p, d.salt, 0.0, 0, 1, _ptr(seed), _sink_mode(sk), _ptr(ws), wsn, _stream()),
-          "npvp_frameln_act_bwd_pgrad")
+    check(L.npvp_frameln_act_bwd_pgrad_bits(_ptr(dout), _ptr(h), mean, rstd, _ptr(w), _ptr(b), _ptr(psum), _ptr(dw), _ptr(db),
+                                            frames, PF, d.p, d.salt, 0.0, 0, 1, _ptr(seed), _sink_mode(sk), _ptr(ws), wsn, _ptr(bits),
+                                            _stream()), "npvp_frameln_act_bwd_pgrad_bits")
     if sk:
         _reduce_partials(sk, ws, dw, db, L.npvp_frameln_act_bwd_reduce, L.npvp_frameln_act_bwd_reduce_job, "npvp_frameln_act_bwd_reduce",
                          (frames, PF, 1), True)
@@ -1384,9 +1384,14 @@
         DropRecorder.note(d2, "elem", R * hid)
         a2 = torch.empty(R, hid, dtype=f32, device=dev)
         a2_slot = _new_slot(dev)
-        check(L.npvp_frameln_act_fwd_parts_skip(_ptr(h2), _ptr(part2), hid // 512, 32768.0, 1e-5, _row(stats, 2), _row(stats, 3),
-                                                _ptr(n2w), _ptr(n2b), None, _ptr(a2), frames, PFh, d2.p, d2.salt, 0.0, 0, 1, _ptr(seed),
-                                                _ptr(a2_slot), *skip.frame, st), "npvp_frameln_act_fwd_parts_skip")
+        bits2 = bits3 = None
+        if DROP_BITS and d2.p > 0.0:
+            bits2 = torch.empty(R * hid // 8, dtype=torch.uint8, device=dev)
+            bits3 = torch.empty(R * Co // 8, dtype=torch.uint8, device=dev)
+        ctx.bits = (bits2, bits3)
+        check(L.npvp_frameln_act_fwd_parts_skip_bits(_ptr(h2), _ptr(part2), hid // 512, 32768.0, 1e-5, _row(stats, 2), _row(stats, 3),
+                                                     _ptr(n2w), _ptr(n2b), None, _ptr(a2), frames, PFh, d2.p, d2.salt, 0.0, 0, 1, _ptr(seed),
+                                                     _ptr(a2_slot), *skip.frame, _ptr(bits2), st), "npvp_frameln_act_fwd_parts_skip_bits")
         tag_amax(a2, a2_slot)
         h3 = torch.empty(R, Co, dtype=f32, device=dev)
         part3 = torch.empty(frames * (Co // 64) * 2, dtype=f32, device=dev)
@@ -1394,9 +1399,9 @@
         DropRecorder.note(d3, "elem", R * Co)
         DropRecorder.note(dp, "group", frames // max(1, T))
         out = torch.empty(R, Co, dtype=f32, device=dev)
-        check(L.npvp_frameln_act_fwd_parts_skip(_ptr(h3), _ptr(part3), Co // 64, 4096.0, 1e-5, _row(stats, 4), _row(stats, 5),
-                                                _ptr(n3w), _ptr(n3b), _ptr(res), _ptr(out), frames, PFo, d3.p, d3.salt, dp.p, dp.salt, T,
-                                                _ptr(seed), None, *skip.frame, st), "npvp_frameln_act_fwd_parts_skip")
+        check(L.npvp_frameln_act_fwd_parts_skip_bits(_ptr(h3), _ptr(part3), Co // 64, 4096.0, 1e-5, _row(stats, 4), _row(stats, 5),
+                                                     _ptr(n3w), _ptr(n3b), _ptr(res), _ptr(out), frames, PFo, d3.p, d3.salt, dp.p, dp.salt, T,
+                                                     _ptr(seed), None, *skip.frame, _ptr(bits3), st), "npvp_frameln_act_fwd_parts_skip_bits")
         ctx.save_for_backward(x, h1, h2, a2, h3, stats, wtb, w1, w2, n1w, n1b, n2w, n2b, n3w, n3b)
         ctx.cfg = (frames, T, d2, d3, dp, res is not None, b1 is not None, b2 is not None)
         ctx.sinks = (_wb_sink(w1, b1), _wb_sink(w2, b2), _ln_sink(n1w, n1b), _ln_sink(n2w, n2b), _ln_sink(n3w, n3b))
@@ -1414,14 +1419,15 @@
         Co = h3.shape[1]
         dev = x.device
         dout = _c(dout)
-        dh3, gn3w, gn3b = _fln_bwd(dout, h3, stats[4], stats[5], n3w, n3b, frames, 64 * Co, d3, dp, T, s_n3)
+        bits2, bits3 = ctx.bits
+        dh3, gn3w, gn3b = _fln_bwd(dout, h3, stats[4], stats[5], n3w, n3b, frames, 64 * Co, d3, dp, T, s_n3, bits=bits3)
         da2, gw2, gb2 = linear_bwd(dh3, a2, w2, True if has_b2 else None, s_fc2, skip=ctx.skip)
         fuse_n2 = MID_BWD_N2 and hid // 16 <= 256
         if fuse_n2:
-            psum2, gn2w, gn2b = _fln_pgrad(da2, h2, _row(stats, 2), _row(stats, 3), n2w, n2b, frames, 64 * hid, d2, s_n2)
+            psum2, gn2w, gn2b = _fln_pgrad(da2, h2, _row(stats, 2), _row(stats, 3), n2w, n2b, frames, 64 * hid, d2, s_n2, bits=bits2)
         else:
             dh2, gn2w, gn2b = _fln_bwd(da2, h2, stats[2], stats[3], n2w, n2b, frames, 64 * hid, d2, NO_DROP, 1, s_n2,
-                                          want_amax=False)
+                                          want_amax=False, bits=bits2)
             del da2
         da1 = torch.empty_like(h1)
         dwtb = torch.empty(10, hid, dtype=torch.float32, device=dev)
@@ -1433,11 +1439,11 @@
         if fuse_n2:
             seed = _S._cur.rng.seed_for(dev, d2)
             pe = HbmProbe.begin()
-            check(L.npvp_mlpdw_mid_bwd_n2(_ptr(da2), _ptr(h2), _row(stats, 2), _row(stats, 3), _ptr(n2w), _ptr(n2b), _ptr(psum2),
-                                          hid // 16, d2.p, d2.salt, _ptr(seed), _ptr(h1), _row(stats, 0), _row(stats, 1), _ptr(n1w),
-                                          _ptr(n1b), _ptr(wtb), _ptr(da1), _ptr(dwtb), _ptr(psum), frames, 8, 8, hid, wmode, _ptr(ws), wsn,
-                                          _stream()), "npvp_mlpdw_mid_bwd_n2")
-            HbmProbe.end(pe, "npvp::mlpdw_mid_bwd_kernel<1, true>", 4.0 * 4 * frames * 64 * hid)
+            check(L.npvp_mlpdw_mid_bwd_n2_bits(_ptr(da2), _ptr(h2), _row(stats, 2), _row(stats, 3), _ptr(n2w), _ptr(n2b), _ptr(psum2),
+                                               hid // 16, d2.p, d2.salt, _ptr(seed), _ptr(h1), _row(stats, 0), _row(stats, 1), _ptr(n1w),
+                                               _ptr(n1b), _ptr(wtb), _ptr(da1), _ptr(dwtb), _ptr(psum), frames, 8, 8, hid, wmode, _ptr(ws), wsn,
+                                               _ptr(bits2), _stream()), "npvp_mlpdw_mid_bwd_n2_bits")
+            HbmProbe.end(pe, "npvp::mlpdw_mid_bwd_kernel<1, true>", 4.0 * 4 * frames * 64 * hid + (frames * 64 * hid // 8 if bits2 is not None else 0))
             del da2, psum2
         else:
             check(L.npvp_mlpdw_mid_bwd(_ptr(dh2), _ptr(h1), _row(stats, 0), _row(stats, 1), _ptr(n1w), _ptr(n1b), _ptr(wtb), _ptr(da1),
@@ -1460,6 +1466,7 @@
 
 
 MID_BWD_N2 = True
+DROP_BITS = True
 DROP_PATH_SKIP = True
 WGRAD_ROW_SKIP = True
 
```

Result: no change. 8692, median of 6 (+0.4%).
